# mx-strk/InformationBottleneckDecodingLDPC

Hardware: AMD Instinct MI355X
Metric: decoded codewords/sec + achieved HBM GB/s, DVB-S2 N=64800 i_max=50 (higher is better)
Workload: dtype u4

## Files before the change

include/ibldpc.h:

```cpp
#ifndef IBLDPC_H
#define IBLDPC_H

#include <stdint.h>

#ifdef __cplusplus
extern "C" {
#endif

#define IBL_VERSION 3

enum { IBL_OK = 0, IBL_EINVAL = -1, IBL_EHIP = -2, IBL_ENOMEM = -3, IBL_EUNSUPPORTED = -4 };
enum { IBL_U8 = 1, IBL_I32 = 2, IBL_F32 = 3, IBL_F64 = 4, IBL_I8 = 5 };
enum { IBL_MINSUM = 0, IBL_BP = 1 };
enum { IBL_PATH_AUTO = 0, IBL_PATH_PASSES = 1, IBL_PATH_FUSED = 2 };
enum { IBL_FLAG_FORCE_GENERIC = 1 };

typedef struct ibl_graph ibl_graph;
typedef struct ibl_ib ibl_ib;
typedef struct ibl_float ibl_float;

int ibl_version(void);
const char* ibl_last_error(void);
int ibl_device_count(int32_t* n);

int ibl_map_node_connections(int32_t n_v, int32_t n_c, const int32_t* csr_indptr, const int32_t* csr_cols,
                             int32_t* cn_start, int32_t* cn_deg, int32_t* tgt_cn,
                             int32_t* vn_start, int32_t* vn_deg, int32_t* tgt_vn);

int ibl_graph_create(int32_t n_v, int32_t n_c, const int32_t* csr_indptr, const int32_t* csr_cols,
                     int32_t device, ibl_graph** out);
int ibl_graph_info(const ibl_graph* g, int32_t* n_v, int32_t* n_c, int64_t* n_e, int32_t* d_c_max,
                   int32_t* d_v_max);
void ibl_graph_destroy(ibl_graph* g);

int ibl_ib_create(const ibl_graph* g, int32_t T_ch, int32_t T_dec, int32_t imax,
                  const int32_t* cn_lut, int64_t cn_len, const int32_t* vn_lut, int64_t vn_len,
                  const int32_t* match_cn, int64_t mc_len, const int32_t* match_vn, int64_t mv_len,
                  int32_t match, int32_t max_batch, int32_t flags, ibl_ib** out);
int ibl_ib_path(const ibl_ib* h);
int ibl_ib_set_path(ibl_ib* h, int32_t path);
int ibl_ib_path_in_use(const ibl_ib* h, int32_t* fused);
int ibl_ib_set_small_batch(ibl_ib* h, int32_t max_b);
int ibl_ib_small_batch(const ibl_ib* h, int32_t* max_b);
int ibl_ib_folded(const ibl_ib* h, int32_t* n_folded);
int ibl_ib_set_fold(ibl_ib* h, int32_t on);
int ibl_ib_fused_ncw(const ibl_ib* h, int32_t B, int32_t* ncw);
int ibl_ib_decode(ibl_ib* h, const void* d_ch, int32_t ch_dtype, int32_t B, void* d_out, int32_t out_dtype,
                  int32_t early_stop, int32_t* d_iters, void* stream);
void ibl_ib_destroy(ibl_ib* h);
int ibl_ib_timing(ibl_ib* h, int32_t enable);
int ibl_ib_timing_read(ibl_ib* h, double* cn_ms, int32_t* cn_launches, double* vn_ms, int32_t* vn_launches);

int ibl_float_create(const ibl_graph* g, int32_t kind, int32_t imax, double llr_max, int32_t precision,
                     int32_t max_batch, ibl_float** out);
int ibl_float_decode(ibl_float* h, const void* d_llr, int32_t llr_dtype, int32_t B, void* d_out,
                     int32_t out_dtype, int32_t early_stop, int32_t* d_iters, void* stream);
void ibl_float_destroy(ibl_float* h);
int ibl_float_set_path(ibl_float* h, int32_t path);
int ibl_float_path_in_use(const ibl_float* h, int32_t* fused);
int ibl_float_fused_geometry(const ibl_float* h, int32_t B, int32_t* ngroups, int32_t* grid);
int ibl_float_folded(const ibl_float* h, int32_t* n_folded);
int ibl_float_is_wide(const ibl_float* h, int32_t* wide);
int ibl_float_set_small_batch(ibl_float* h, int32_t max_b);
int ibl_float_small_batch(const ibl_float* h, int32_t* max_b);
int ibl_float_input_check(ibl_float* h, int32_t* violations, void* stream);
int ibl_float_timing(ibl_float* h, int32_t enable);
int ibl_float_timing_read(ibl_float* h, double* cn_ms, int32_t* cn_launches, double* vn_ms, int32_t* vn_launches);
int ibl_float_create_corrected(const ibl_graph* g, double alpha, double beta, int32_t imax, double llr_max,
                               int32_t precision, int32_t max_batch, ibl_float** out);
int ibl_float_correction(const ibl_float* h, double* alpha, double* beta);
int ibl_ib_decode_each(ibl_ib* h, const void* d_ch, int32_t ch_dtype, int32_t B, void* d_out, int32_t out_dtype,
                       int32_t* d_iters, void* stream);
int ibl_float_decode_each(ibl_float* h, const void* d_llr, int32_t llr_dtype, int32_t B, void* d_out,
                          int32_t out_dtype, int32_t* d_iters, void* stream);

typedef struct ibl_layered ibl_layered;
int ibl_layers_validate(int32_t n_v, int32_t n_c, const int32_t* csr_indptr, const int32_t* csr_cols,
                        int32_t n_layers, const int32_t* layer_ptr, const int32_t* layer_checks);
int ibl_layered_create(const ibl_graph* g, int32_t n_layers, const int32_t* layer_ptr, const int32_t* layer_checks,
                       int32_t imax, float alpha, float beta, float llr_max, int32_t precision, int32_t max_batch,
                       ibl_layered** out);
int ibl_layered_create_path(const ibl_graph* g, int32_t n_layers, const int32_t* layer_ptr,
                            const int32_t* layer_checks, int32_t imax, float alpha, float beta, float llr_max,
                            int32_t precision, int32_t max_batch, int32_t path, ibl_layered** out);
int ibl_layered_path_in_use(const ibl_layered* h, int32_t* fused);
int ibl_layered_is_wide(const ibl_layered* h, int32_t* wide);
int ibl_layered_decode(ibl_layered* h, const void* d_llr, int32_t llr_dtype, int32_t B, void* d_out,
                       int32_t out_dtype, int32_t early_stop, int32_t* d_iters, void* stream);
int ibl_layered_geometry(const ibl_layered* h, int32_t B, int32_t* cw_per_group, int32_t* ngroups, int32_t* grid);
int ibl_layered_set_compaction(ibl_layered* h, int32_t every, int32_t min_free_pct);
int ibl_layered_compaction_stats(const ibl_layered* h, void* stream, int32_t* compactions, int32_t* extent);
void ibl_layered_destroy(ibl_layered* h);

int ibl_layered_create_fixed(const ibl_graph* g, int32_t n_layers, const int32_t* layer_ptr,
                             const int32_t* layer_checks, int32_t imax, int32_t alpha16, int32_t beta_q, int32_t q_max,
                             float scale, int32_t max_batch, int32_t path, ibl_layered** out);
int ibl_layered_create_fixed_fused(const ibl_graph* g, int32_t n_layers, const int32_t* layer_ptr,
                                   const int32_t* layer_checks, int32_t imax, int32_t alpha16, int32_t beta_q,
                                   int32_t q_max, float scale, int32_t max_batch, ibl_layered** out);
int ibl_layered_is_fixed(const ibl_layered* h, int32_t* fixed);

int ibl_count_below(const void* d_x, int32_t dtype, int64_t rows, int32_t B, int64_t ld, double threshold,
                    int64_t* d_count, void* stream);

int ibl_channel_sample(const double* cdf, int32_t T, const double* llr, uint64_t seed, uint64_t offset, int32_t n,
                       int32_t B, const uint8_t* d_bits, void* d_out, int32_t out_dtype, int64_t ld, void* stream);

typedef struct ibl_encoder ibl_encoder;
int ibl_encoder_create(int32_t n_v, int32_t n_c, const int32_t* indptr, const int32_t* cols, int32_t max_batch,
                       int32_t device, ibl_encoder** out);
const char* ibl_encoder_algorithm(const ibl_encoder* h);
int ibl_encode(ibl_encoder* h, const uint8_t* d_info, int32_t B, uint8_t* d_code, void* stream);
void ibl_encoder_destroy(ibl_encoder* h);

int ibl_random_bits(uint64_t seed, uint64_t offset, int32_t n, int32_t B, uint8_t* d_out, void* stream);

int ibl_count_errors(const void* d_x, int32_t dtype, int64_t rows, int32_t B, int64_t ld, double threshold,
                     const uint8_t* d_bits, int64_t bits_ld, int64_t* d_count, void* stream);

int ibl_shard_range(int64_t total, int32_t rank, int32_t world, int64_t* start, int64_t* count);
#define IBL_COMM_ID_BYTES 128
typedef struct ibl_comm ibl_comm;
int ibl_comm_unique_id(uint8_t* id);
int ibl_comm_create(const uint8_t* id, int32_t nranks, int32_t rank, int32_t device, ibl_comm** out);
int ibl_comm_broadcast(ibl_comm* c, void* d_buf, int64_t bytes, int32_t root, void* stream);
int ibl_comm_allreduce_sum_i64(ibl_comm* c, int64_t* d_buf, int64_t count, void* stream);
void ibl_comm_destroy(ibl_comm* c);

// ... 6 lines not shown
```

informationbottleneckdecodingldpc_amd/_lib.py:

```python
from __future__ import annotations

import ctypes
import os

import numpy as np

_HERE = os.path.dirname(os.path.abspath(__file__))
LIB_PATH = os.environ.get("IBLDPC_LIB") or os.path.join(_HERE, "libibldpc.so")

IBL_OK, IBL_EINVAL, IBL_EHIP, IBL_ENOMEM, IBL_EUNSUPPORTED = 0, -1, -2, -3, -4
IBL_U8, IBL_I32, IBL_F32, IBL_F64, IBL_I8 = 1, 2, 3, 4, 5
IBL_MINSUM, IBL_BP = 0, 1
IBL_FLAG_FORCE_GENERIC = 1
IBL_PATH_AUTO, IBL_PATH_PASSES, IBL_PATH_FUSED = 0, 1, 2

EXPORTS = [
    "ibl_version", "ibl_last_error", "ibl_device_count", "ibl_map_node_connections",
    "ibl_graph_create", "ibl_graph_info", "ibl_graph_destroy",
    "ibl_ib_create", "ibl_ib_path", "ibl_ib_set_path", "ibl_ib_path_in_use", "ibl_ib_fused_ncw", "ibl_ib_decode",
    "ibl_ib_set_small_batch", "ibl_ib_small_batch", "ibl_ib_folded", "ibl_ib_set_fold",
    "ibl_ib_destroy",
    "ibl_float_create", "ibl_float_decode", "ibl_float_destroy", "ibl_count_below",
    "ibl_float_set_path", "ibl_float_path_in_use", "ibl_float_fused_geometry", "ibl_float_folded",
    "ibl_float_input_check", "ibl_float_is_wide",
    "ibl_float_set_small_batch", "ibl_float_small_batch",
    "ibl_float_create_corrected", "ibl_float_correction", "ibl_float_decode_each", "ibl_ib_decode_each",
    "ibl_ib_timing", "ibl_ib_timing_read", "ibl_float_timing", "ibl_float_timing_read",
    "ibl_channel_sample",
    "ibl_encoder_create",
    "ibl_encoder_algorithm",
    "ibl_encode",
    "ibl_encoder_destroy",
    "ibl_random_bits",
    "ibl_count_errors",
    "ibl_shard_range", "ibl_comm_unique_id", "ibl_comm_create", "ibl_comm_broadcast", "ibl_comm_allreduce_sum_i64",
    "ibl_comm_destroy",
    "ibl_layers_validate", "ibl_layered_create", "ibl_layered_decode", "ibl_layered_geometry", "ibl_layered_destroy",
    "ibl_layered_create_path", "ibl_layered_path_in_use", "ibl_layered_create_fixed", "ibl_layered_is_fixed",
    "ibl_layered_set_compaction", "ibl_layered_compaction_stats", "ibl_layered_is_wide",
    "ibl_layered_create_fixed_fused",
]
IBL_COMM_ID_BYTES = 128


class IBLError(RuntimeError):
    pass


_lib = None
_i32p = np.ctypeslib.ndpointer(dtype=np.int32, flags="C_CONTIGUOUS")
_vp = ctypes.c_void_p
_i32, _i64 = ctypes.c_int32, ctypes.c_int64


def load():
    global _lib
    if _lib is not None:
        return _lib
    if not os.path.exists(LIB_PATH):
        raise ImportError(f"{LIB_PATH} not found: build it with "
                          "`python -c 'import __graft_entry__ as g; g.build()'` (hipcc, gfx950)")
    L = ctypes.CDLL(LIB_PATH)
    L.ibl_version.restype = ctypes.c_int
    L.ibl_last_error.restype = ctypes.c_char_p
    L.ibl_device_count.argtypes = [ctypes.POINTER(_i32)]
    L.ibl_map_node_connections.argtypes = [_i32, _i32, _i32p, _i32p, _i32p, _i32p, _i32p, _i32p, _i32p, _i32p]
    L.ibl_graph_create.argtypes = [_i32, _i32, _i32p, _i32p, _i32, ctypes.POINTER(_vp)]
    L.ibl_graph_info.argtypes = [_vp, ctypes.POINTER(_i32), ctypes.POINTER(_i32), ctypes.POINTER(_i64),
                                 ctypes.POINTER(_i32), ctypes.POINTER(_i32)]
    L.ibl_graph_destroy.argtypes = [_vp]
    L.ibl_graph_destroy.restype = None
    L.ibl_ib_create.argtypes = [_vp, _i32, _i32, _i32, _i32p, _i64, _i32p, _i64, _i32p, _i64, _i32p, _i64,
                                _i32, _i32, _i32, ctypes.POINTER(_vp)]
    L.ibl_ib_path.argtypes = [_vp]
    L.ibl_ib_set_path.argtypes = [_vp, _i32]
    L.ibl_ib_path_in_use.argtypes = [_vp, ctypes.POINTER(_i32)]
    L.ibl_ib_fused_ncw.argtypes = [_vp, _i32, ctypes.POINTER(_i32)]
    L.ibl_ib_set_small_batch.argtypes = [_vp, _i32]
    L.ibl_ib_small_batch.argtypes = [_vp, ctypes.POINTER(_i32)]
    L.ibl_ib_folded.argtypes = [_vp, ctypes.POINTER(_i32)]
    L.ibl_ib_set_fold.argtypes = [_vp, _i32]
    L.ibl_ib_decode.argtypes = [_vp, _vp, _i32, _i32, _vp, _i32, _i32, _vp, _vp]
    L.ibl_ib_decode_each.argtypes = [_vp, _vp, _i32, _i32, _vp, _i32, _vp, _vp]
    L.ibl_ib_destroy.argtypes = [_vp]
    L.ibl_ib_destroy.restype = None
    L.ibl_float_create.argtypes = [_vp, _i32, _i32, ctypes.c_double, _i32, _i32, ctypes.POINTER(_vp)]
    L.ibl_float_decode.argtypes = [_vp, _vp, _i32, _i32, _vp, _i32, _i32, _vp, _vp]
    L.ibl_float_decode_each.argtypes = [_vp, _vp, _i32, _i32, _vp, _i32, _vp, _vp]
    L.ibl_float_destroy.argtypes = [_vp]
    L.ibl_float_destroy.restype = None
    L.ibl_float_set_path.argtypes = [_vp, _i32]
    L.ibl_float_path_in_use.argtypes = [_vp, ctypes.POINTER(_i32)]
    L.ibl_float_fused_geometry.argtypes = [_vp, _i32, ctypes.POINTER(_i32), ctypes.POINTER(_i32)]
    L.ibl_float_folded.argtypes = [_vp, ctypes.POINTER(_i32)]
    L.ibl_float_is_wide.argtypes = [_vp, ctypes.POINTER(_i32)]
    L.ibl_float_set_small_batch.argtypes = [_vp, _i32]
    L.ibl_float_small_batch.argtypes = [_vp, ctypes.POINTER(_i32)]
    L.ibl_float_input_check.argtypes = [_vp, ctypes.POINTER(_i32), _vp]
    L.ibl_float_create_corrected.argtypes = [_vp, ctypes.c_double, ctypes.c_double, _i32, ctypes.c_double, _i32, _i32,
                                             ctypes.POINTER(_vp)]
    L.ibl_float_correction.argtypes = [_vp, ctypes.POINTER(ctypes.c_double), ctypes.POINTER(ctypes.c_double)]
    for nm in ("ibl_ib_timing", "ibl_float_timing"):
        getattr(L, nm).argtypes = [_vp, _i32]
    for nm in ("ibl_ib_timing_read", "ibl_float_timing_read"):
        getattr(L, nm).argtypes = [_vp, ctypes.POINTER(ctypes.c_double), ctypes.POINTER(_i32),
                                   ctypes.POINTER(ctypes.c_double), ctypes.POINTER(_i32)]
    L.ibl_count_below.argtypes = [_vp, _i32, _i64, _i32, _i64, ctypes.c_double, _vp, _vp]
    _dp = np.ctypeslib.ndpointer(np.float64, flags="C_CONTIGUOUS")
    L.ibl_channel_sample.argtypes = [_dp, _i32, _vp, ctypes.c_uint64, ctypes.c_uint64, _i32, _i32, _vp, _vp,
                                     _i32, _i64, _vp]
    L.ibl_encoder_create.argtypes = [_i32, _i32, _i32p, _i32p, _i32, _i32, ctypes.POINTER(_vp)]
    L.ibl_encoder_algorithm.argtypes = [_vp]
    L.ibl_encoder_algorithm.restype = ctypes.c_char_p
    L.ibl_encode.argtypes = [_vp, _vp, _i32, _vp, _vp]
    L.ibl_encoder_destroy.argtypes = [_vp]
    L.ibl_encoder_destroy.restype = None
    L.ibl_random_bits.argtypes = [ctypes.c_uint64, ctypes.c_uint64, _i32, _i32, _vp, _vp]
    L.ibl_count_errors.argtypes = [_vp, _i32, _i64, _i32, _i64, ctypes.c_double, _vp, _i64, _vp, _vp]
    L.ibl_shard_range.argtypes = [_i64, _i32, _i32, ctypes.POINTER(_i64), ctypes.POINTER(_i64)]
    L.ibl_comm_unique_id.argtypes = [_vp]
    L.ibl_comm_create.argtypes = [_vp, _i32, _i32, _i32, ctypes.POINTER(_vp)]
    L.ibl_comm_broadcast.argtypes = [_vp, _vp, _i64, _i32, _vp]
    L.ibl_comm_allreduce_sum_i64.argtypes = [_vp, _vp, _i64, _vp]
    L.ibl_comm_destroy.argtypes = [_vp]
    L.ibl_comm_destroy.restype = None
    L.ibl_layers_validate.argtypes = [_i32, _i32, _i32p, _i32p, _i32, _i32p, _i32p]
    _f32 = ctypes.c_float
    L.ibl_layered_create.argtypes = [_vp, _i32, _i32p, _i32p, _i32, _f32, _f32, _f32, _i32, _i32, ctypes.POINTER(_vp)]
    L.ibl_layered_create_path.argtypes = [_vp, _i32, _i32p, _i32p, _i32, _f32, _f32, _f32, _i32, _i32, _i32,
                                          ctypes.POINTER(_vp)]
    L.ibl_layered_path_in_use.argtypes = [_vp, ctypes.POINTER(_i32)]
    L.ibl_layered_create_fixed.argtypes = [_vp, _i32, _i32p, _i32p, _i32, _i32, _i32, _i32, _f32, _i32, _i32,
                                           ctypes.POINTER(_vp)]
    L.ibl_layered_create_fixed_fused.argtypes = [_vp, _i32, _i32p, _i32p, _i32, _i32, _i32, _i32, _f32, _i32,
                                                 ctypes.POINTER(_vp)]
    L.ibl_layered_is_fixed.argtypes = [_vp, ctypes.POINTER(_i32)]
    L.ibl_layered_is_wide.argtypes = [_vp, ctypes.POINTER(_i32)]
    L.ibl_layered_decode.argtypes =[_vp, _vp, _i32, _i32, _vp, _i32, _i32, _vp, _vp]
    L.ibl_layered_geometry.argtypes = [_vp, _i32, ctypes.POINTER(_i32), ctypes.POINTER(_i32), ctypes.POINTER(_i32)]
    L.ibl_layered_set_compaction.argtypes = [_vp, _i32, _i32]
    L.ibl_layered_compaction_stats.argtypes = [_vp, _vp, ctypes.POINTER(_i32), ctypes.POINTER(_i32)]
    L.ibl_layered_destroy.argtypes = [_vp]
    L.ibl_layered_destroy.restype = None
    for name in EXPORTS:
        getattr(L, name)
    _lib = L
    return L


def check(rc: int, what: str = "") -> None:
    if rc != IBL_OK:
        msg = load().ibl_last_error().decode(errors="replace")
        raise IBLError(f"{what} failed (rc={rc}): {msg}")


def device_count() -> int:
    n = _i32(0)
    load().ibl_device_count(ctypes.byref(n))
    return int(n.value)


def map_node_connections(n_v: int, n_c: int, indptr: np.ndarray, cols: np.ndarray):
    L = load()
    indptr = np.ascontiguousarray(indptr, dtype=np.int32)
# ... 33 lines not shown
```

informationbottleneckdecodingldpc_amd/csrc/capi_ib.hip:

```cpp
#include <cstring>
#include <functional>

#include "host.h"

using namespace ibl;

struct ibl_ib {
  const ibl_graph* g = nullptr;
  int32_t Tc = 0, T = 0, imax = 0, CM = 0, VM = 0, match = 0, max_batch = 0, ldb = 0;
  bool fast = false;
  DevBuf<uint8_t> cin, vin, ch8;
  DevBuf<int32_t> flags, dL;
  DevBuf<uint32_t> cn_img, vn_img, dec_img;
  int cn_nt = 0, vn_nt = 0, dec_nt = 0;
  int32_t cn_fslot[kMaxD + 1] = {0}, vn_fslot[kMaxD + 1] = {0};
  KCfg kcn, kvn, kdec;
  KTimer timer;
  int32_t n_folded = 0, fold_slot = -1, n_rest = 0, rest_heavy = 0;
  bool fold_on = true;
  std::vector<int32_t> fold_rec, fold_cn_info, fold_vn_info;
  DevBuf<uint8_t> cin2;
  DevBuf<int32_t> fold, cn_info_f, vn_info_r;
  int32_t path = IBL_PATH_AUTO;
  bool fused_ok = false, f_half_ok = false;
  bool f_each_ok = false;
  int32_t f_ncw_forced = 0;
  int32_t small_b = 0;
  bool s_ok = false;
  size_t s_lds_cn = 0, s_lds_vn = 0, s_lds_dec = 0;
  ChainGraphs s_graphs;
  FusedTaskBufs ft;
  int32_t f_nreg = 0, f_dbuf = 0, f_cn_uni = 0, f_vn_uni = 0;
  size_t f_lds = 0;
  int f_grid = 0, f_block = 0;
  DevBuf<int32_t> cn_lut, vn_lut, mc, mv;
  int64_t cn_len = 0, vn_len = 0, mc_len = 0, mv_len = 0;
};

namespace {

using Table = std::vector<uint8_t>;

struct IbLuts {
  const int32_t *cn, *vn, *mc, *mv;
  int64_t cn_len, vn_len, mc_len, mv_len;
};
struct IbSlots {
  std::vector<int> cdeg, vdeg;
  int cn_nraw = 0, vn_nraw = 0;
  int cn_nt = 0, vn_nt = 0;
};
struct IbImages {
  std::vector<uint32_t> cn_img, vn_img, dec_img;
};

Table make_table(int T, const std::function<int(int, int)>& f) {
  Table tb(256, 0);
  for (int t = 0; t < T; ++t)
    for (int m = 0; m < T; ++m) tb[t * kTP + m] = (uint8_t)f(t, m);
  return tb;
}

void append_pass(std::vector<uint32_t>& img, const std::vector<Table>& tbs, int nreg) {
  for (int R = 0; R < nreg; ++R)
    for (int r = 0; r < 256; ++r) {
      uint32_t w = 0;
      for (int j = 0; j < 4; ++j) {
        const size_t k = (size_t)4 * R + j;
        if (k < tbs.size()) w |= (uint32_t)tbs[k][r] << (8 * j);
      }
      img.push_back(w);
    }
}

std::vector<int> present(const std::vector<int32_t>& deg) {
  std::vector<int> d(deg.begin(), deg.end());
  std::sort(d.begin(), d.end());
  d.erase(std::unique(d.begin(), d.end()), d.end());
  return d;
}

size_t fast_lds(int nt) { return lds_of_quads(regions_of(nt)) + 64; }

int pick_cfg(int which, int maxd, int nt, int num_cus, KCfg* k) {
  k->lds = fast_lds(nt);
  int best_waves = 0;
  for (int block : {1024, 768, 640, 512, 384, 256}) {
    int bpc = 0;
    if (ib_fast_occupancy(which, maxd, block, k->lds, &bpc) != hipSuccess) continue;
    const int waves = bpc * block / 64;
    if (bpc > 0 && waves > best_waves) {
      best_waves = waves;
      k->block = block;
      k->grid = bpc * num_cus;
    }
  }
  return best_waves > 0 ? IBL_OK : fail(IBL_EHIP, "no occupancy for IB kernel (LDS too large?)");
}

int ib_validate(const ibl_graph* g, int32_t Tc, int32_t T, int32_t imax, const IbLuts& lu, int32_t match,
                int32_t max_batch) {
  if (Tc < 2 || T < 2 || Tc > 256 || T > 256) return fail(IBL_EUNSUPPORTED, "cardinalities must lie in [2, 256]");
  if (imax < 1) return fail(IBL_EINVAL, "imax must be >= 1");
  if (max_batch < 1) return fail(IBL_EINVAL, "max_batch must be >= 1");
  const int CM = g->dcm, VM = g->dvm;
  if (CM < 3) return fail(IBL_EUNSUPPORTED, "IB decoding needs a check-node degree >= 3");
  const int64_t need_cn = (int64_t)Tc * Tc + (int64_t)(CM - 3) * Tc * T + (int64_t)(imax - 1) * (CM - 2) * T * T;
  const int64_t need_vn = (int64_t)imax * ((int64_t)Tc * T + (int64_t)(VM - 1) * T * T);
  if (!lu.cn || lu.cn_len < need_cn) return fail(IBL_EINVAL, "CN LUT vector shorter than the reference layout");
  if (!lu.vn || lu.vn_len < need_vn) return fail(IBL_EINVAL, "VN LUT vector shorter than the reference layout");
  auto in_T = [T](const int32_t* p, int64_t n) { return std::all_of(p, p + n, [T](int32_t x) { return x >= 0 && x < T; }); };
  if (!in_T(lu.cn, lu.cn_len)) return fail(IBL_EINVAL, "CN LUT entries must lie in [0, T_dec)");
  if (!in_T(lu.vn, lu.vn_len)) return fail(IBL_EINVAL, "VN LUT entries must lie in [0, T_dec)");
  if (match) {
    if (!lu.mc || lu.mc_len < (int64_t)imax * CM * T || !lu.mv || lu.mv_len < (int64_t)imax * VM * T)
      return fail(IBL_EINVAL, "matching vectors shorter than (imax, d_max, T_dec)");
    if (!in_T(lu.mc, lu.mc_len) || !in_T(lu.mv, lu.mv_len))
      return fail(IBL_EINVAL, "matching entries must lie in [0, T_dec)");
  }
  return IBL_OK;
}

IbSlots ib_plan_slots(ibl_ib* h, int32_t flags) {
  const ibl_graph* g = h->g;
  const int CM = h->CM, VM = h->VM;
  IbSlots sl;
  sl.cdeg = present(g->h_cn_deg);
  sl.vdeg = present(g->h_vn_deg);
  const bool deg_ok = CM <= kMaxD && VM <= kMaxD;
  sl.cn_nt = sl.cn_nraw = h->match ? CM - 3 : CM - 2;
  sl.vn_nt = sl.vn_nraw = h->match ? std::max(VM - 2, 0) : VM - 1;
  if (h->match) {
    sl.cn_nt += (int)sl.cdeg.size();
    for (int d : sl.vdeg) sl.vn_nt += (d >= 2);
  }
  const int max_nt = (kLdsBytes / kSuper) * 8;
  int slot = sl.cn_nraw;
  for (int d : sl.cdeg) {
    const int fs = h->match ? slot++ : (d >= 3 ? d - 3 : 0);
    if (deg_ok) h->cn_fslot[d] = fs;
  }
  slot = sl.vn_nraw;
  for (int d : sl.vdeg) {
    if (d < 2) continue;
    const int fs = h->match ? slot++ : d - 2;
    if (deg_ok) h->vn_fslot[d] = fs;
  }
  const bool lds_ok = fast_lds(sl.cn_nt) <= (size_t)kLdsBytes && fast_lds(std::max(sl.vn_nt, 1)) <= (size_t)kLdsBytes;
  h->fast = !(flags & IBL_FLAG_FORCE_GENERIC) && h->Tc == h->T && h->T <= kTP && deg_ok && sl.cn_nt <= max_nt &&
            sl.vn_nt <= max_nt && VM <= max_nt && sl.cn_nt > 0 && lds_ok;
  if (h->fast && CM <= 8) {
    std::vector<int32_t> rec, rest;
    const int32_t n = plan_ib_fold(*g, &rec, &rest);
    if (n > 0 && sl.cn_nt + 1 <= max_nt && fast_lds(sl.cn_nt + 1) <= (size_t)kLdsBytes) {
      h->n_folded = n;
      h->fold_slot = sl.cn_nt++;
      std::vector<int32_t> cls((size_t)g->n_c), all((size_t)g->n_c);
      for (int32_t c = 0; c < g->n_c; ++c) {
        cls[c] = rec[(size_t)kIbFoldRec * c];
        all[c] = c;
      }
      int32_t heavy = 0;
      h->fold_cn_info = work_order_keyed(all, g->h_cn_start, g->h_cn_deg, &cls, &heavy);
      h->fold_vn_info = work_order_keyed(rest, g->h_vn_start, g->h_vn_deg, nullptr, &h->rest_heavy);
      h->n_rest = (int32_t)rest.size();
      h->fold_rec.swap(rec);
    }
  }
  return sl;
}

IbImages ib_build_images(ibl_ib* h, const IbLuts& lu, const IbSlots& sl) {
  const int Tc = h->Tc, T = h->T, imax = h->imax, CM = h->CM, VM = h->VM;
  IbImages im;
  const int64_t T2 = (int64_t)T * T;
  auto cn_raw = [&](int p, int l, int t, int m) -> int {
    int64_t idx;
    if (p == 0) idx = (l == 0) ? (int64_t)t * Tc + m : (int64_t)Tc * Tc + (int64_t)(l - 1) * Tc * T + (int64_t)t * T + m;
    else idx = (int64_t)Tc * Tc + (int64_t)(CM - 3) * Tc * T + (int64_t)(p - 1) * (CM - 2) * T2 + l * T2 + (int64_t)t * T + m;
    return lu.cn[idx];
  };
  auto vn_raw = [&](int k, int l, int t, int m) -> int {
    const int64_t off = (int64_t)k * ((int64_t)Tc * T + (int64_t)(VM - 1) * T2);
    const int64_t idx = off + (l == 0 ? (int64_t)t * T + m : (int64_t)Tc * T + (int64_t)(l - 1) * T2 + (int64_t)t * T + m);
    return lu.vn[idx];
  };
  for (int p = 0; p < imax; ++p) {
    std::vector<Table> tbs;
    for (int l = 0; l < sl.cn_nraw; ++l) tbs.push_back(make_table(T, [&](int t, int m) { return cn_raw(p, l, t, m); }));
    if (h->match)
      for (int d : sl.cdeg) {
        const int64_t mrow = (int64_t)p * T * CM + (int64_t)(d - 1) * T;
        if (d == 2) tbs.push_back(make_table(T, [&](int t, int) { return lu.mc[mrow + t]; }));
        else tbs.push_back(make_table(T, [&](int t, int m) { return lu.mc[mrow + cn_raw(p, d - 3, t, m)]; }));
      }
    if (h->fold_slot >= 0) {
      const int64_t mrow = (int64_t)p * T * VM + (int64_t)T;
      tbs.resize((size_t)h->fold_slot, Table(256, 0));
      tbs.push_back(make_table(T, [&](int t, int m) {
        const int r = vn_raw(p, 0, m, t);
        return h->match ? lu.mv[mrow + r] : r;
      }));
    }
    append_pass(im.cn_img, tbs, regions_of(sl.cn_nt));
  }
  h->cn_nt = regions_of(sl.cn_nt);
  for (int k = 0; k < std::max(imax - 1, 1); ++k) {
    std::vector<Table> tbs;
    for (int l = 0; l < sl.vn_nraw; ++l) tbs.push_back(make_table(T, [&](int t, int m) { return vn_raw(k, l, t, m); }));
    for (int d : sl.vdeg) {
      if (!h->match || d < 2) continue;
      const int64_t mrow = (int64_t)k * T * VM + (int64_t)(d - 1) * T;
      tbs.push_back(make_table(T, [&](int t, int m) { return lu.mv[mrow + vn_raw(k, d - 2, t, m)]; }));
    }
    append_pass(im.vn_img, tbs, regions_of(std::max(sl.vn_nt, 1)));
  }
  h->vn_nt = regions_of(std::max(sl.vn_nt, 1));
  for (int k = 0; k < imax; ++k) {
    std::vector<Table> tbs;
    for (int l = 0; l < VM; ++l) tbs.push_back(make_table(T, [&](int t, int m) { return vn_raw(k, l, t, m); }));
    append_pass(im.dec_img, tbs, regions_of(VM));
  }
  h->dec_nt = regions_of(VM);
  return im;
}

int ib_fused_setup(ibl_ib* h) {
  const ibl_graph* g = h->g;
  if (!h->fast || g->n_e == 0 || g->dc_min < 2) return IBL_OK;
  const int nreg = std::max(h->cn_nt, std::max(h->vn_nt, h->dec_nt));
  const size_t lds1 = lds_of_quads(nreg) + (size_t)nreg * 1024 + (size_t)g->n_e * 4 + 16;
  const size_t lds2 = lds_of_quads(2 * nreg) + (size_t)g->n_e * 4 + 16;
  const bool dbuf = nreg <= 2 && lds2 <= (size_t)kLdsBytes && env_on("IBL_FUSED_DBUF");
  const size_t lds = dbuf ? lds2 : lds1;
  if (lds > (size_t)kLdsBytes) return IBL_OK;
  int bpc = 0, block = 0;
  size_t priv = 0;
  if (ib_fused_occupancy(h->CM, h->VM, 8, lds, &bpc, &block, &priv) != hipSuccess || bpc < 1 || priv != 0) {
    (void)hipGetLastError();
    return IBL_OK;
  }
  {
    int bpc4 = 0, block4 = 0;
    size_t priv4 = 0;
    h->f_half_ok = ib_fused_occupancy(h->CM, h->VM, 4, lds, &bpc4, &block4, &priv4) == hipSuccess && bpc4 == bpc &&
                   block4 == block && priv4 == 0;
    (void)hipGetLastError();
  }
  {
    int bpe = 0, blocke = 0;
    size_t prive = 0;
    h->f_each_ok = ib_fused_occupancy(h->CM, h->VM, 8, lds, &bpe, &blocke, &prive, true) == hipSuccess && bpe == bpc &&
                   blocke == block && prive == 0;
    if (h->f_each_ok && h->f_half_ok)
      h->f_each_ok = ib_fused_occupancy(h->CM, h->VM, 4, lds, &bpe, &blocke, &prive, true) == hipSuccess &&
                     bpe == bpc && blocke == block && prive == 0;
    (void)hipGetLastError();
  }
  FusedTasks ft;
  build_fused_tasks(*g, &ft, env_on("IBL_FUSED_VORDER"), fused_vwin());
  if (int rc = h->ft.upload(ft)) return rc;
  if (env_on("IBL_FUSED_UNIFORM")) {
    auto uniform = [](const std::vector<int32_t>& task, int32_t n, bool vn) {
      if (task.empty()) return 0;
      const int32_t d = task[2];
      for (size_t t = 0; t < task.size() / 4; ++t) {
        const int32_t p = (int32_t)(64 * t), cnt = std::min<int32_t>(64, n - p);
        const int32_t* r = &task[4 * t];
        if (r[1] != cnt || r[2] != d || (vn ? (r[0] != p || r[3] != p * d) : r[0] != p * d)) return 0;
      }
      return (int)d;
    };
    h->f_cn_uni = uniform(ft.cn_task, g->n_c, false);
    h->f_vn_uni = uniform(ft.vn_task, g->n_v, true);
  }
  if (const char* ne = getenv("IBL_FUSED_NCW")) h->f_ncw_forced = atoi(ne);
  h->f_nreg = nreg;
  h->f_dbuf = dbuf ? 1 : 0;
  h->f_lds = lds;
  h->f_block = block;
  h->f_grid = bpc * g->num_cus;
  h->fused_ok = true;
  return IBL_OK;
}

int ib_configure_fast(ibl_ib* h, const IbImages& im) {
  const ibl_graph* g = h->g;
  const int CM = h->CM, VM = h->VM;
  int rc;
  if ((rc = h->cn_img.upload(im.cn_img)) || (rc = h->vn_img.upload(im.vn_img)) || (rc = h->dec_img.upload(im.dec_img)))
    return rc;
  if ((rc = pick_cfg(0, CM, 4 * h->cn_nt, g->num_cus, &h->kcn)) ||
      (rc = pick_cfg(1, VM, 4 * h->vn_nt, g->num_cus, &h->kvn)) ||
      (rc = pick_cfg(2, VM, 4 * h->dec_nt, g->num_cus, &h->kdec)))
    return rc;
  size_t priv = 0;
  const char* kname = "";
  HIPCHK(ib_fast_private_bytes(CM, VM, &priv, &kname));
#if IBL_DIAG
  const bool allow_scratch = getenv("IBL_ALLOW_SCRATCH") != nullptr;
#else
  const bool allow_scratch = false;
#endif
  if (!allow_scratch && (rc = refuse_private(priv, std::string("fast-path kernel ") + kname + " has a ",
                                             "-byte private segment (register spill / scratch item): rebuild required")))
    return rc;
  if ((rc = ib_fused_setup(h))) return rc;
  HIPCHK(ib_small_private_bytes(CM, VM, &priv, &kname));
  h->s_ok = priv == 0;
  small_batch_env(h->s_ok, kSmallBatchDefault, &h->small_b, &h->s_graphs);
  h->s_lds_cn = lds_of_quads(h->cn_nt);
  h->s_lds_vn = lds_of_quads(h->vn_nt);
  h->s_lds_dec = lds_of_quads(h->dec_nt);
  return IBL_OK;
}

int ib_upload_generic(ibl_ib* h, const IbLuts& lu) {
  int rc;
  h->cn_len = lu.cn_len; h->vn_len = lu.vn_len;
  if ((rc = h->cn_lut.upload(lu.cn, lu.cn_len)) || (rc = h->vn_lut.upload(lu.vn, lu.vn_len))) return rc;
  if (h->match) {
    h->mc_len = lu.mc_len; h->mv_len = lu.mv_len;
    if ((rc = h->mc.upload(lu.mc, lu.mc_len)) || (rc = h->mv.upload(lu.mv, lu.mv_len))) return rc;
  }
  return IBL_OK;
}

bool ib_fused_in_use(const ibl_ib* h) { return h->fused_ok && h->path != IBL_PATH_PASSES; }

int ib_fused_ncw(const ibl_ib* h, int B) {
  const int ngroups = (B + 7) / 8;
  const int forced = h->f_ncw_forced;
  if (!h->f_half_ok || forced == 8) return 8;
  return (forced == 4 || 2 * ngroups <= h->f_grid) ? 4 : 8;
}

int ib_fold_alloc(ibl_ib* h) {
  if (h->n_folded == 0 || h->cin2) return IBL_OK;
  DevBuf<uint8_t> c2;
  DevBuf<int32_t> fold, cf, vr;
  int rc;
  if ((rc = c2.alloc_zero((size_t)h->g->n_e * h->ldb)) || (rc = fold.upload(h->fold_rec)) ||
      (rc = cf.upload(h->fold_cn_info)) || (rc = vr.upload(h->fold_vn_info)))
    return rc;
  h->fold = std::move(fold);
  h->cn_info_f = std::move(cf);
  h->vn_info_r = std::move(vr);
  h->cin2 = std::move(c2);
  return IBL_OK;
}


void ib_pass_args(const ibl_ib* h, int B, int ldbb, IbFastArgs* cn, IbFastArgs* vn) {
  const ibl_graph* g = h->g;
  cn->ch8 = vn->ch8 = h->ch8;
  cn->info = g->cn_info; cn->tgt = g->tgt_cn; cn->out = h->vin;
  vn->info = g->vn_info; vn->tgt = g->tgt_vn; vn->out = h->cin; vn->in = h->vin;
  cn->n_nodes = g->n_c; vn->n_nodes = g->n_v;
  cn->ldb = vn->ldb = ldbb;
  cn->B = vn->B = B;
  cn->half = vn->half = h->T / 2;
  cn->match = vn->match = h->match;
  cn->nt = h->cn_nt; vn->nt = h->vn_nt;
  std::memcpy(cn->fslot, h->cn_fslot, sizeof(cn->fslot));
  std::memcpy(vn->fslot, h->vn_fslot, sizeof(vn->fslot));
}

IbFusedArgs ib_fused_args(const ibl_ib* h, uint32_t* chT, int32_t B, void* d_out, int32_t out_dtype, int* grid) {
  const ibl_graph* g = h->g;
  IbFusedArgs f{};
  f.cn_img = h->cn_img; f.vn_img = h->vn_img; f.dec_img = h->dec_img; f.chT = chT;
  f.cn_task = h->ft.cn_task; f.vn_task = h->ft.vn_task; f.vn_node = h->ft.vn_node; f.vn_slot = h->ft.vn_slot;
  f.out = d_out;
  std::memcpy(f.cn_fslot, h->cn_fslot, sizeof(f.cn_fslot));
  std::memcpy(f.vn_fslot, h->vn_fslot, sizeof(f.vn_fslot));
  f.cn_nt = h->cn_nt; f.vn_nt = h->vn_nt; f.dec_nt = h->dec_nt; f.nreg = h->f_nreg; f.dbuf = h->f_dbuf;
  f.n_cn_nodes = g->n_c; f.cn_uni = h->f_cn_uni; f.vn_uni = h->f_vn_uni;
  f.n_e = (int32_t)g->n_e; f.n_v = g->n_v; f.n_cn_tasks = h->ft.n_cn; f.n_vn_tasks = h->ft.n_vn;
// ... 60 lines not shown
    const int wpb = small_block(nwords) / 64;
    const int need = (ntask * nwords + wpb - 1) / wpb;
    return std::max(1, std::min(need, per_cu * g->num_cus));
  };
  IbFastArgs cn{}, vn{};
  ib_pass_args(h, B, ldbb, &cn, &vn);
  cn.task = g->cn_task; cn.n_tasks = g->n_cn_task;
  vn.task = g->vn_task; vn.n_tasks = g->n_vn_task;
  cn.nwords = vn.nwords = nwords;
  const int gcn = grid_of(g->n_cn_task, h->s_lds_cn), gvn = grid_of(g->n_vn_task, h->s_lds_vn);
  auto chain = [&](hipStream_t st) -> hipError_t {
    IbFastArgs c0 = cn, v = vn;
    c0.in = nullptr; c0.gather = g->csr_cols; c0.img = h->cn_img; c0.gate = nullptr; c0.unsat = nullptr;
    hipError_t e = h->timer.timed(0, st, [&] { return launch_ib_cn_small(c0, h->CM, gcn, h->s_lds_cn, st); });
    if (e != hipSuccess) return e;
    IbFastArgs c = c0;
    c.gather = nullptr;
    c.in = h->cin;
    for (int j = 1; j < I; ++j) {
      const int32_t* gate = flag_row(h->flags, early && j >= 2, j - 1);
      v.img = h->vn_img + (size_t)(j - 1) * h->vn_nt * 256;
      v.gate = gate;
      if ((e = h->timer.timed(1, st, [&] { return launch_ib_vn_small(v, h->VM, gvn, h->s_lds_vn, st); })) != hipSuccess)
        return e;
      c.img = h->cn_img + (size_t)j * h->cn_nt * 256;
      c.gate = gate;
      c.unsat = flag_row(h->flags, early, j);
      if ((e = h->timer.timed(0, st, [&] { return launch_ib_cn_small(c, h->CM, gcn, h->s_lds_cn, st); })) != hipSuccess)
        return e;
    }
    return hipSuccess;
  };
  if (h->s_graphs.on && !h->timer.on) HIPCHK(h->s_graphs.run(B, early ? 1 : 0, s, chain));
  else HIPCHK(chain(s));
  HIPCHK(launch_finalize(h->flags, I, early ? 1 : 0, h->dL, d_iters, s));
  IbDecArgs dc{};
  dc.vin = h->vin; dc.ch8 = h->ch8; dc.img = h->dec_img; dc.iters = h->dL; dc.out = d_out; dc.out_dtype = out_dtype;
  dc.nt = h->dec_nt; dc.n_nodes = g->n_v; dc.ldb = ldbb; dc.B = B;
  dc.info = g->vn_info; dc.task = g->vn_task; dc.n_tasks = g->n_vn_task; dc.nwords = nwords;
  dc.aligned = out_aligned(B, d_out, 4, out_dtype == kU8 ? 1 : 4);
  HIPCHK(launch_ib_dec_small(dc, grid_of(g->n_vn_task, h->s_lds_dec), h->s_lds_dec, s));
  return IBL_OK;
}

int ib_decode_fast(ibl_ib* h, const void* d_ch, int32_t ch_dtype, int32_t B, void* d_out, int32_t out_dtype,
                   bool early, int32_t* d_iters, hipStream_t s) {
  const ibl_graph* g = h->g;
  const int I = h->imax;
  const int ccn = ib_fast_chunk(h->CM), cvn = ib_fast_chunk(h->VM);
  const int ldbb = h->ldb / 2;
  HIPCHK(launch_ib_stage4(d_ch, ch_dtype, g->n_v, B, h->ch8, ldbb, s));
  IbFastArgs cn{}, vn{};
  ib_pass_args(h, B, ldbb, &cn, &vn);
  cn.n_heavy = g->cn_heavy; vn.n_heavy = g->vn_heavy;
  const bool fold = h->fold_on && h->n_folded > 0 && I > 1;
  int rc;
  if (fold) {
    if ((rc = ib_fold_alloc(h))) return rc;
    vn.info = h->vn_info_r; vn.n_nodes = h->n_rest; vn.n_heavy = h->rest_heavy;
    cn.fold = h->fold; cn.fold_slot = h->fold_slot;
  }
  uint8_t* cb[2] = {h->cin, fold ? h->cin2 : h->cin};
  auto cn_fold = [&](int j) {
    const bool f = fold && j < I - 1;
    cn.info = f ? h->cn_info_f.get() : g->cn_info.get();
    cn.fold_mode = f ? ((early && j >= 1) ? 2 : 1) : 0;
    cn.fout = f ? cb[(j + 1) & 1] : nullptr;
  };
#if IBL_DIAG
  if (const char* vp = getenv("IBL_VN_PART")) {
    if (vp[0] == 'h') {
      vn.n_nodes = g->vn_heavy;
    } else if (vp[0] == 'l') {
      vn.info = g->vn_info + 4 * (size_t)g->vn_heavy;
      vn.n_nodes = g->n_v - g->vn_heavy;
      vn.n_heavy = 0;
    }
  }
#endif
  cn.nchunks = (B + ccn - 1) / ccn;
  vn.nchunks = (B + cvn - 1) / cvn;
  cn.in = nullptr; cn.gather = g->csr_cols; cn.img = h->cn_img; cn.gate = nullptr; cn.unsat = nullptr;
  cn_fold(0);
  auto launch_cn = [&]() { return launch_ib_cn_fast(cn, h->CM, h->kcn.grid, h->kcn.block, h->kcn.lds, s); };
  HIPCHK(h->timer.timed(0, s, launch_cn));
  cn.gather = nullptr;
  uint64_t* trace = nullptr;
  size_t nwv = 0;
#if IBL_DIAG
  const char* trace_path = getenv("IBL_TRACE_WAVES");
  TraceBuf tr;
  nwv = (size_t)h->kvn.grid * (h->kvn.block / 64);
  const size_t nwc = (size_t)h->kcn.grid * (h->kcn.block / 64);
  if (trace_path && I > 1) {
    if ((rc = tr.open(3 * (nwv + nwc), s))) return rc;
    trace = tr.d;
  }
#endif
  for (int j = 1; j < I; ++j) {
    const int32_t* gate = flag_row(h->flags, early && j >= 2, j - 1);
    vn.img = h->vn_img + (size_t)(j - 1) * h->vn_nt * 256;
    vn.gate = gate;
    vn.trace = (trace && j == I / 2) ? trace : nullptr;
    vn.out = cb[j & 1];
    HIPCHK(h->timer.timed(1, s, [&] { return launch_ib_vn_fast(vn, h->VM, h->kvn.grid, h->kvn.block, h->kvn.lds, s); }));
    cn.img = h->cn_img + (size_t)j * h->cn_nt * 256;
    cn.gate = gate;
    cn.unsat = flag_row(h->flags, early, j);
    cn.trace = (trace && j == I / 2) ? trace + 3 * nwv : nullptr;
    cn.in = cb[j & 1];
    cn_fold(j);
    HIPCHK(h->timer.timed(0, s, launch_cn));
  }
#if IBL_DIAG
  if (trace && ((rc = tr.save(s, std::string(trace_path) + "_vn.bin", 0, 3 * nwv)) ||
                (rc = tr.save(s, std::string(trace_path) + "_cn.bin", 3 * nwv, 3 * nwc))))
    return rc;
#endif
  HIPCHK(launch_finalize(h->flags, I, early ? 1 : 0, h->dL, d_iters, s));
  IbDecArgs dc{};
  dc.vin = h->vin; dc.ch8 = h->ch8; dc.start = g->vn_start; dc.deg = g->vn_deg; dc.img = h->dec_img;
  dc.iters = h->dL; dc.out = d_out; dc.out_dtype = out_dtype; dc.nt = h->dec_nt; dc.n_nodes = g->n_v;
  dc.nchunks = (B + kChunkDec - 1) / kChunkDec; dc.ldb = ldbb; dc.B = B;
  dc.aligned = out_aligned(B, d_out, 4, out_dtype == kU8 ? 1 : 4);
  HIPCHK(launch_ib_dec_fast(dc, h->kdec.grid, h->kdec.block, h->kdec.lds, s));
  return IBL_OK;
}

int ib_decode_generic(ibl_ib* h, const void* d_ch, int32_t ch_dtype, int32_t B, void* d_out, int32_t out_dtype,
                      bool early, int32_t* d_iters, hipStream_t s) {
  const ibl_graph* g = h->g;
  const int I = h->imax;
  HIPCHK(launch_ib_stage(d_ch, ch_dtype, g->n_v, B, h->ch8, h->ldb, s));
  IbGenArgs cn{}, vn{};
  cn.ch8 = vn.ch8 = h->ch8;
  cn.start = g->cn_start; cn.deg = g->cn_deg; cn.tgt = g->tgt_cn; cn.out = h->vin; cn.lut = h->cn_lut;
  cn.lut_len = h->cn_len; cn.mt = h->mc; cn.mt_len = h->mc_len;
  vn.start = g->vn_start; vn.deg = g->vn_deg; vn.tgt = g->tgt_vn; vn.out = h->cin; vn.in = h->vin; vn.lut = h->vn_lut;
  vn.lut_len = h->vn_len; vn.mt = h->mv; vn.mt_len = h->mv_len;
  cn.Tc = vn.Tc = h->Tc; cn.T = vn.T = h->T; cn.CM = vn.CM = h->CM; cn.VM = vn.VM = h->VM;
  cn.match = vn.match = h->match;
  cn.n_nodes = g->n_c; vn.n_nodes = g->n_v;
  cn.ldb = vn.ldb = h->ldb; cn.B = vn.B = B; cn.half = vn.half = h->T / 2;
  cn.pass = 0; cn.in = nullptr; cn.gather = g->csr_cols;
  HIPCHK(h->timer.timed(0, s, [&] { return launch_ib_cn_gen(cn, s); }));
  cn.in = h->cin; cn.gather = nullptr;
  for (int j = 1; j < I; ++j) {
    const int32_t* gate = flag_row(h->flags, early && j >= 2, j - 1);
    vn.pass = j - 1; vn.gate = gate;
    HIPCHK(h->timer.timed(1, s, [&] { return launch_ib_vn_gen(vn, s); }));
    cn.pass = j; cn.gate = gate; cn.unsat = flag_row(h->flags, early, j);
    HIPCHK(h->timer.timed(0, s, [&] { return launch_ib_cn_gen(cn, s); }));
  }
  HIPCHK(launch_finalize(h->flags, I, early ? 1 : 0, h->dL, d_iters, s));
  IbGenDecArgs dc{};
  dc.vin = h->vin; dc.ch8 = h->ch8; dc.start = g->vn_start; dc.deg = g->vn_deg; dc.lut = h->vn_lut;
  dc.lut_len = h->vn_len; dc.iters = h->dL; dc.out = d_out; dc.out_dtype = out_dtype; dc.Tc = h->Tc; dc.T = h->T;
  dc.VM = h->VM; dc.n_nodes = g->n_v; dc.ldb = h->ldb; dc.B = B;
  HIPCHK(launch_ib_dec_gen(dc, s));
  return IBL_OK;
}
}

extern "C" {

int ibl_ib_create(const ibl_graph* g, int32_t Tc, int32_t T, int32_t imax, const int32_t* cn_lut, int64_t cn_len,
                  const int32_t* vn_lut, int64_t vn_len, const int32_t* match_cn, int64_t mc_len,
                  const int32_t* match_vn, int64_t mv_len, int32_t match, int32_t max_batch, int32_t flags,
                  ibl_ib** out) {
  if (!out) return fail(IBL_EINVAL, "out is NULL");
  *out = nullptr;
  if (!g) return fail(IBL_EINVAL, "graph is NULL");
  const IbLuts lu{cn_lut, vn_lut, match_cn, match_vn, cn_len, vn_len, mc_len, mv_len};
  int rc = ib_validate(g, Tc, T, imax, lu, match, max_batch);
  if (rc) return rc;
  HIPCHK(hipSetDevice(g->device));
  std::unique_ptr<ibl_ib> h(new ibl_ib());
  h->g = g;
  h->Tc = Tc; h->T = T; h->imax = imax; h->CM = g->dcm; h->VM = g->dvm; h->match = match ? 1 : 0;
  h->max_batch = max_batch;
  h->ldb = (max_batch + kRowPad - 1) / kRowPad * kRowPad;
  const size_t inbox = (size_t)g->n_e * h->ldb;
  if ((rc = h->cin.alloc_zero(inbox)) || (rc = h->vin.alloc_zero(inbox)) ||
      (rc = h->ch8.alloc_zero((size_t)g->n_v * h->ldb)) || (rc = h->flags.alloc_zero((size_t)imax * kShards)) ||
      (rc = h->dL.alloc(1)))
    return rc;
  const IbSlots sl = ib_plan_slots(h.get(), flags);
  if (h->fast) rc = ib_configure_fast(h.get(), ib_build_images(h.get(), lu, sl));
  else rc = ib_upload_generic(h.get(), lu);
  if (rc) return rc;
  *out = h.release();
  return IBL_OK;
}

int ibl_ib_path(const ibl_ib* h) { return h && h->fast ? 1 : 0; }

int ibl_ib_set_small_batch(ibl_ib* h, int32_t max_b) {
  if (!h) return fail(IBL_EINVAL, "decoder is NULL");
  if (max_b < 0) return fail(IBL_EINVAL, "max_b must be >= 0");
  if (max_b > 0 && !(h->fast && h->s_lds_cn > 0))
    return fail(IBL_EUNSUPPORTED, "the small-batch kernels need the fast path (T_ch = T_dec <= 16, degrees <= 16)");
  if (max_b > 0 && !h->s_ok)
    return fail(IBL_EUNSUPPORTED, "the small-batch kernels of this build have a private segment: rebuild required");
  h->small_b = max_b;
  return IBL_OK;
}

int ibl_ib_small_batch(const ibl_ib* h, int32_t* max_b) {
  if (!h || !max_b) return fail(IBL_EINVAL, "NULL argument");
  *max_b = h->small_b;
  return IBL_OK;
}

int ibl_ib_set_path(ibl_ib* h, int32_t path) {
  if (!h) return fail(IBL_EINVAL, "decoder is NULL");
  if (int rc = check_path(path)) return rc;
  if (path == IBL_PATH_FUSED && !h->fused_ok)
    return fail(IBL_EUNSUPPORTED, "code does not fit the fused IB kernel (fast path, E * 4 B of messages plus the "
                                  "largest pass's tables within 160 KiB, check degrees >= 2)");
  h->path = path;
  return IBL_OK;
}

int ibl_ib_fused_ncw(const ibl_ib* h, int32_t B, int32_t* ncw) {
  if (!h || !ncw) return fail(IBL_EINVAL, "NULL argument");
  if (B < 1 || B > h->max_batch) return fail(IBL_EINVAL, "B must lie in [1, max_batch]");
  *ncw = ib_fused_in_use(h) ? ib_fused_ncw(h, B) : 0;
  return IBL_OK;
}

int ibl_ib_path_in_use(const ibl_ib* h, int32_t* fused) {
  if (!h || !fused) return fail(IBL_EINVAL, "NULL argument");
  *fused = ib_fused_in_use(h) ? 1 : 0;
  return IBL_OK;
}

int ibl_ib_folded(const ibl_ib* h, int32_t* n_folded) {
  if (!h || !n_folded) return fail(IBL_EINVAL, "NULL argument");
  *n_folded = h->n_folded;
  return IBL_OK;
}

int ibl_ib_set_fold(ibl_ib* h, int32_t on) {
  if (!h) return fail(IBL_EINVAL, "decoder is NULL");
  h->fold_on = on != 0;
  return IBL_OK;
}

int ibl_ib_timing(ibl_ib* h, int32_t enable) { return timing_enable(h, enable); }
int ibl_ib_timing_read(ibl_ib* h, double* cn_ms, int32_t* cn_n, double* vn_ms, int32_t* vn_n) {
  return timing_read(h, cn_ms, cn_n, vn_ms, vn_n);
}

void ibl_ib_destroy(ibl_ib* h) {
  if (h) (void)hipSetDevice(h->g->device);
  delete h;
}

static int ib_decode_check(const ibl_ib* h, const void* d_ch, int32_t ch_dtype, int32_t B, const void* d_out,
                           int32_t out_dtype) {
  if (!h) return fail(IBL_EINVAL, "decoder is NULL");
  if (B < 1 || B > h->max_batch) return fail(IBL_EINVAL, "B must lie in [1, max_batch]");
  if (ch_dtype != kU8 && ch_dtype != kI32) return fail(IBL_EINVAL, "channel dtype must be IBL_U8 or IBL_I32");
  if (out_dtype != kU8 && out_dtype != kI32) return fail(IBL_EINVAL, "output dtype must be IBL_U8 or IBL_I32");
  if (!d_ch || !d_out) return fail(IBL_EINVAL, "NULL buffer");
  return IBL_OK;
}

int
ibl_ib_decode_each(ibl_ib* h, const void* d_ch, int32_t ch_dtype, int32_t B, void* d_out, int32_t out_dtype,
                   int32_t* d_iters, void* stream) {
  if (int rc = ib_decode_check(h, d_ch, ch_dtype, B, d_out, out_dtype)) return rc;
  if (!ib_fused_in_use(h))
    return fail(IBL_EUNSUPPORTED, "the per-codeword stop runs on the fused kernel only (path \"passes\", the generic "
                                  "path, or the code does not fit it)");
  if (!h->f_each_ok)
    return fail(IBL_EUNSUPPORTED, "the per-codeword-stop kernels of this build have a private segment or another "
                                  "occupancy than the fused kernel: rebuild required");
  HIPCHK(hipSetDevice(h->g->device));
  return ib_each_fused(h, d_ch, ch_dtype, B, d_out, out_dtype, d_iters, (hipStream_t)stream);
}

int ibl_ib_decode(ibl_ib* h, const void* d_ch, int32_t ch_dtype, int32_t B, void* d_out, int32_t out_dtype,
                  int32_t early_stop, int32_t* d_iters, void* stream) {
  if (int rc = ib_decode_check(h, d_ch, ch_dtype, B, d_out, out_dtype)) return rc;
  hipStream_t s = (hipStream_t)stream;
  HIPCHK(hipSetDevice(h->g->device));
  const bool early = early_stop != 0 && h->imax > 1;
  if (early) HIPCHK(hipMemsetAsync(h->flags, 0, sizeof(int32_t) * (size_t)h->imax * kShards, s));
  if (ib_fused_in_use(h)) return ib_decode_fused(h, d_ch, ch_dtype, B, d_out, out_dtype, early, d_iters, s);
  if (!h->fast) return ib_decode_generic(h, d_ch, ch_dtype, B, d_out, out_dtype, early, d_iters, s);
  if (B <= h->small_b) return ib_decode_small(h, d_ch, ch_dtype, B, d_out, out_dtype, early, d_iters, s);
  return ib_decode_fast(h, d_ch, ch_dtype, B, d_out, out_dtype, early, d_iters, s);
}

}
```

informationbottleneckdecodingldpc_amd/csrc/common.h:

```cpp
#pragma once
#include <hip/hip_runtime.h>
#pragma clang diagnostic ignored "-Wunused-result"
#include <stddef.h>
#include <stdint.h>

#include "plan.h"

namespace ibl {

constexpr int kWave = 64;
constexpr int kChunk = 256;
#ifndef IBL_W
#define IBL_W 2
#endif
constexpr int kW = IBL_W;
constexpr int kChunkIB = 512 * kW;
#ifndef IBL_LIGHT_W
#define IBL_LIGHT_W 4
#endif
constexpr int kRowPad = 512 * (IBL_LIGHT_W > IBL_W ? IBL_LIGHT_W : IBL_W);
constexpr int kChunkDec = 512;
constexpr int kTbl = 8192;
constexpr int kSuper = 65536;
constexpr int kRowSh = 12, kColSh = 8;
__host__ __device__ constexpr uint32_t quad_off(int q) { return (uint32_t)(q >> 1) * kSuper + (uint32_t)(q & 1) * 128u; }
__host__ __device__ constexpr uint32_t slot_off(int s) { return quad_off(s >> 2) + (uint32_t)(s & 3); }
constexpr int regions_of(int nt) { return (nt + 3) >> 2; }
__host__ __device__ constexpr size_t lds_of_quads(int nq) { return (size_t)((nq + 1) >> 1) * kSuper; }
constexpr int kTP = 16;
constexpr int kShards = 64;
constexpr int kLdsBytes = 160 * 1024;

enum Dtype : int32_t { kU8 = 1, kI32 = 2, kF32 = 3, kF64 = 4, kI8 = 5 };

int set_error(int code, const char* msg);

typedef __attribute__((address_space(4))) const int32_t cint32;
__device__ __forceinline__ int32_t sload(const int32_t* p, int i) { return ((cint32*)p)[i]; }

__device__ __forceinline__ int take_ticket(int* ctr, int lane) {
  int t = 0;
  if (lane == 0) t = __hip_atomic_fetch_add(ctr, 1, __ATOMIC_RELAXED, __HIP_MEMORY_SCOPE_WORKGROUP);
  return __builtin_amdgcn_readfirstlane(t);
}

struct IbFastArgs {
  const uint8_t* in;
  uint8_t* out;
  const uint8_t* ch8;
  const int32_t* info;
  const int32_t* tgt;
  const int32_t* gather;
  const uint32_t* img;
  const int32_t* gate;
  int32_t* unsat;
  int32_t fslot[kMaxD + 1];
  int32_t nt;
  int32_t n_nodes, nchunks, ldb, B, half, match;
  int32_t n_heavy;
  uint64_t* trace;
  const int32_t* task;
  int32_t n_tasks, nwords;
  const int32_t* fold;
  uint8_t* fout;
  int32_t fold_mode, fold_slot;
};

struct IbDecArgs {
  const uint8_t* vin;
  const uint8_t* ch8;
  const int32_t* start;
  const int32_t* deg;
  const uint32_t* img;
  const int32_t* iters;
  void* out;
  int32_t out_dtype, nt, n_nodes, nchunks, ldb, B, aligned;
  const int32_t* info;
  const int32_t* task;
  int32_t n_tasks, nwords;
};

struct IbFusedArgs {
  const uint32_t* cn_img;
  const uint32_t* vn_img;
  const uint32_t* dec_img;
  const uint32_t* chT;
  const int32_t* cn_task;
  const int32_t* vn_task;
  const int32_t* vn_node;
  const int32_t* vn_slot;
  void* out;
  int32_t* unsat;
  const int32_t* dL;
  int32_t cn_fslot[kMaxD + 1], vn_fslot[kMaxD + 1];
  int32_t cn_nt, vn_nt, dec_nt, nreg;
  int32_t dbuf;
  int32_t n_cn_nodes;
  int32_t cn_uni, vn_uni;
  int32_t n_e, n_v, n_cn_tasks, n_vn_tasks, B, imax, half, match, out_dtype, aligned, ngroups;
  int32_t ncw;
  uint64_t* trace;
  int32_t* iters;
};

struct IbGenArgs {
  const uint8_t* in;
  uint8_t* out;
  const uint8_t* ch8;
  const int32_t* start;
  const int32_t* deg;
  const int32_t* tgt;
  const int32_t* gather;
  const int32_t* lut;
  const int32_t* mt;
  const int32_t* gate;
  int32_t* unsat;
  int64_t lut_len, mt_len;
  int32_t pass, Tc, T, CM, VM, match, n_nodes, ldb, B, half;
};

struct IbGenDecArgs {
  const uint8_t* vin;
  const uint8_t* ch8;
  const int32_t* start;
  const int32_t* deg;
  const int32_t* lut;
  const int32_t* iters;
  void* out;
  int64_t lut_len;
  int32_t out_dtype, Tc, T, VM, n_nodes, ldb, B;
};

enum FlFamily : int { kFlPerPass = 0, kFlSmall = 1, kFlFused = 2 };
enum FlPass : int { kFlCheck = 0, kFlVariable = 1, kFlDecision = 2, kFlSend = 3 };
constexpr int kFlWideD = 32;
constexpr int fl_cw_per_lane(int prec) { return prec == kF32 ? 4 : 2; }
constexpr size_t fl_elem_size(int dtype) { return dtype == kF32 ? 4 : 8; }
constexpr int fl_vn_chunk(int prec) { return 64 * fl_cw_per_lane(prec); }
struct FlArgs {
  const void* in;
  void* out;
  const void* ch;
  const int32_t* start;
  const int32_t* deg;
  const int32_t* tgt;
  const int32_t* gate;
  int32_t* unsat;
  double llr_max;
  int32_t n_nodes, nchunks, ldb, B;
  const int32_t* fold;
  void* fout;
  int32_t fold_mode;
  const int32_t* nodes;
  const int32_t* info;
  const int32_t* task;
  int32_t n_tasks, nwords;
  double cor_a, cor_b;
};

constexpr int kFlTraceWords = 65;
struct FlFusedArgs {
  const void* ch;
  const int32_t* cn_task;
  const int32_t* vn_task;
  const int32_t* vn_node;
  const int32_t* vn_slot;
  void* out;
  int32_t* unsat;
  const int32_t* dL;
  double llr_max;
  int32_t n_e, n_v, n_cn_tasks, n_vn_tasks, ldb, B, imax, out_dtype, aligned, ngroups;
  int32_t n_vs;
  uint64_t* trace;
  double cor_a, cor_b;
  int32_t* iters;
};

struct FlDecArgs {
  const void* vin0;
  const void* vin1;
  const void* ch;
  const int32_t* start;
  const int32_t* deg;
  const int32_t* iters;
  void* out;
  int32_t out_dtype, n_nodes, nchunks, ldb, B, aligned;
  const int32_t* info;
  const int32_t* task;
  int32_t n_tasks, nwords;
};

hipError_t launch_ib_stage(const void* ch, int dtype, int n, int B, uint8_t* ch8, int ldb, hipStream_t s);
hipError_t launch_ib_stage4(const void* ch, int dtype, int n, int B, uint8_t* ch4, int ldb_bytes, hipStream_t s);
hipError_t launch_ib_cn_fast(const IbFastArgs& a, int maxd, int grid, int block, size_t lds, hipStream_t s);
hipError_t launch_ib_vn_fast(const IbFastArgs& a, int maxd, int grid, int block, size_t lds, hipStream_t s);
int ib_fast_chunk(int maxd);
hipError_t launch_ib_dec_fast(const IbDecArgs& a, int grid, int block, size_t lds, hipStream_t s);
constexpr int kSmallBlock = 1024;
__host__ __device__ constexpr int small_block(int nwords) { return nwords <= 1 ? 256 : (nwords <= 8 ? 512 : 1024); }
constexpr int kFlSmallBlock = 256;
constexpr int kSmallBatchDefault = 224;
constexpr int kFlSmallBatchDefault = 64;
hipError_t launch_ib_cn_small(const IbFastArgs& a, int maxd, int grid, size_t lds, hipStream_t s);
hipError_t launch_ib_vn_small(const IbFastArgs& a, int maxd, int grid, size_t lds, hipStream_t s);
hipError_t launch_ib_dec_small(const IbDecArgs& a, int grid, size_t lds, hipStream_t s);
hipError_t ib_small_private_bytes(int cn_maxd, int vn_maxd, size_t* bytes, const char** name);
hipError_t ib_fast_occupancy(int which, int maxd, int block, size_t lds, int* blocks_per_cu);
hipError_t ib_fast_private_bytes(int cn_maxd, int vn_maxd, size_t* bytes, const char** name);
hipError_t launch_ib_stage_t(const void* ch, int dtype, int n, int B, const int32_t* perm, uint32_t* chT,
                             hipStream_t s);
hipError_t launch_ib_fused(const IbFusedArgs& a, int cmax, int vmax, int grid, int block, size_t lds, hipStream_t s,
                           bool each = false);
hipError_t ib_fused_occupancy(int cmax, int vmax, int ncw, size_t lds, int* blocks_per_cu, int* block,
                              size_t* private_bytes, bool each = false);
hipError_t launch_ib_cn_gen(const IbGenArgs& a, hipStream_t s);
hipError_t launch_ib_vn_gen(const IbGenArgs& a, hipStream_t s);
hipError_t launch_ib_dec_gen(const IbGenDecArgs& a, hipStream_t s);
hipError_t launch_finalize(const int32_t* flags, int imax, int early, int32_t* dL, int32_t* user, hipStream_t s);
constexpr int kMaxT = 64;
constexpr int kChBinSh = 43, kChBins = 1 << (53 - kChBinSh);
struct ChArgs {
  uint64_t kthr[kMaxT + 1];
  double llr[kMaxT];
  uint64_t ctr[4];
  uint64_t key[2];
  const uint8_t* bits;
  void* out;
  int64_t total, ld;
  int32_t B, T, dtype;
  int32_t sorted;
  uint16_t bin[kChBins];
};
hipError_t launch_ch_sample(const ChArgs& a, hipStream_t s);

hipError_t launch_enc_pack(const uint8_t* in, int rows, int B, int Bw, uint32_t* out, hipStream_t s);
hipError_t launch_enc_ax(const uint32_t* x, const int32_t* indptr, const int32_t* cols, int M, int Bw, uint32_t* r,
                         hipStream_t s);
hipError_t launch_enc_subst(const uint32_t* in, uint32_t* out, const int32_t* indptr, const int32_t* cols, int M,
                            int Bw, int dir, hipStream_t s);
hipError_t launch_enc_scan(const uint32_t* r, uint32_t* tot, int M, int Bw, int dir, uint32_t* p, hipStream_t s);
int enc_scan_segments();
hipError_t launch_enc_gather(const uint32_t* in, const int32_t* order, int M, int Bw, uint32_t* out, hipStream_t s);
hipError_t launch_enc_unpack(const uint8_t* info, const uint32_t* p, int K, int M, int B, int Bw, uint8_t* code,
                             hipStream_t s);
hipError_t launch_random_bits(uint64_t seed, uint64_t offset, int64_t total, uint8_t* out, hipStream_t s);
hipError_t launch_count_errors(const void* x, int dtype, int64_t rows, int B, int64_t ld, double thr,
                               const uint8_t* bits, int64_t bits_ld, unsigned long long* cnt, hipStream_t s);

hipError_t launch_count_below(const void* x, int dtype, int64_t rows, int B, int64_t ld, double thr,
                              unsigned long long* cnt, hipStream_t s);

hipError_t launch_fl_send(const FlArgs& a, int prec, hipStream_t s);
hipError_t launch_fl_stage(const void* x, int in_dtype, int n, int B, void* dst, int prec, int ldb, int rule,
                           int32_t* bad, hipStream_t s);
hipError_t launch_fl_stage_t(const void* x, int in_dtype, int n, int B, const int32_t* perm, void* dst, int prec,
                             int rule, int32_t* bad, hipStream_t s);
hipError_t launch_fl_pass(FlFamily fam, FlPass pass, const FlArgs& a, int kind, int prec, int maxd, int grid,
                          hipStream_t s);
hipError_t launch_fl_dec(FlFamily fam, const FlDecArgs& a, int prec, int grid, hipStream_t s);
hipError_t launch_fl_fused(const FlFusedArgs& a, int kind, int prec, int cmax, int vmax, int grid, size_t lds,
                           hipStream_t s, bool each = false);
hipError_t fl_occupancy(FlFamily fam, FlPass pass, int kind, int prec, int cmax, int vmax, size_t lds,
                        int* blocks_per_cu, int* block, bool each = false);
hipError_t fl_private_bytes(FlFamily fam, int kind, int prec, int cn_maxd, int vn_maxd, bool fused, size_t* bytes,
                            const char** name);

struct LayeredArgs {
  float* buf;
  const int32_t* task;
  const int32_t* idx;
  int32_t* iters;
  float alpha, beta, llr_max;
  int32_t n_v, n_c, n_tasks, B, imax, early, ngroups, cw_per_group, cw_bytes;
  uint64_t* trace;
};
hipError_t lay_fused_occupancy(bool wide, int cw_per_group, size_t lds, int* blocks_per_cu, size_t* private_bytes);
hipError_t launch_lay_fused(const LayeredArgs& a, bool wide, int grid, size_t lds, hipStream_t s);
// ... 76 lines not shown
```

informationbottleneckdecodingldpc_amd/csrc/ib_kernels.hip:

```cpp
#include <algorithm>
#include <type_traits>

#include "common.h"

namespace ibl {


typedef __attribute__((address_space(3))) const uint8_t lds8_t;
__device__ __forceinline__ uint32_t lu(uint32_t x, uint32_t c) {
  asm("" : "+v"(x));
  return *(lds8_t*)(size_t)(x + c);
}
__device__ __forceinline__ uint32_t luc(uint32_t t, uint32_t q, uint32_t c) {
  uint32_t x;
  static_assert(kRowSh == 12, "luc's shift is the row shift of the table layout");
  asm("v_lshl_or_b32 %0, %1, 12, %2" : "=v"(x) : "v"(t), "v"(q));
  return *(lds8_t*)(size_t)(x + c);
}
__device__ __forceinline__ uint32_t lds_base(const uint8_t* p) { return (uint32_t)(size_t)(lds8_t*)p; }
__device__ __forceinline__ void lds_at_zero(const uint8_t* lds) {
  if (lds_base(lds) != 0u) __builtin_trap();
}

__device__ __forceinline__ uint32_t qidx(uint32_t m, uint32_t lane4) { return (m << kColSh) | lane4; }

__device__ __forceinline__ uint32_t valid_mask4(int remaining) {
  return remaining >= 4 ? 0xFu : (remaining <= 0 ? 0u : ((1u << remaining) - 1u));
}

__device__ __forceinline__ bool gate_open(const int32_t* gate, int lane) {
  if (!gate) return true;
  return __ballot(gate[lane] != 0) != 0ull;
}

constexpr int kStageR = 4;
__device__ __forceinline__ void stage_tables(uint8_t* lds, const uint32_t* img, int nreg) {
  const int nraw = nreg * 256, lane = threadIdx.x & 63;
  const int wv = threadIdx.x >> 6, nwv = blockDim.x >> 6, nchunk = (nraw + 63) >> 6;
  for (int c0 = 0; c0 < nchunk; c0 += kStageR * nwv) {
    uint32_t v[kStageR];
#pragma unroll
    for (int k = 0; k < kStageR; ++k) {
      const int r = (c0 + wv + k * nwv) * 64 + lane;
      v[k] = r < nraw ? img[r] : 0u;
    }
#pragma unroll
    for (int k = 0; k < kStageR; ++k) {
      const int c = c0 + wv + k * nwv;
      if (c >= nchunk) break;
#pragma unroll
      for (int p = 0; p < 8; ++p) {
        const int src = 8 * p + (lane >> 3), r = c * 64 + src;
        const uint32_t w = __shfl(v[k], src, 64);
        if (r < nraw)
          *reinterpret_cast<uint4*>(lds + quad_off(r >> 8) + (uint32_t)(r & 255) * 256u + 16u * (uint32_t)(lane & 7)) =
              make_uint4(w, w, w, w);
      }
    }
  }
}

__device__ __forceinline__ uint32_t nib(uint32_t w, int k) { return __builtin_amdgcn_ubfe(w, 4 * k, 4); }
__device__ __forceinline__ uint32_t colq(uint32_t w, int k, uint32_t lane4) {
  static_assert(kColSh == 8, "colq places the column in byte 1");
  const uint32_t src = (k & 1) ? ((w >> 4) & 0x0F0F0F0Fu) : (w & 0x0F0F0F0Fu);
  return __builtin_amdgcn_perm(src, lane4, 0x03020000u | ((4u + (uint32_t)(k >> 1)) << 8));
}

template <int P>
__device__ __forceinline__ uint32_t rowcol(uint32_t x, uint32_t y) {
  if constexpr (P == 0) return ((x << 4) & 0xF0F0F0F0u) | (y & 0x0F0F0F0Fu);
  else return (x & 0xF0F0F0F0u) | ((y >> 4) & 0x0F0F0F0Fu);
}
__device__ __forceinline__ uint32_t colb(uint32_t e, int k, uint32_t lane4) {
  return __builtin_amdgcn_perm(e, lane4, 0x03020000u | ((4u + (uint32_t)(k >> 1)) << 8));
}
template <int K>
__device__ __forceinline__ uint32_t pk(uint32_t acc, uint32_t t) {
  static_assert(K >= 0 && K < 8, "nibble of a dword");
  if constexpr (K == 0) {
    return t;
  } else {
    uint32_t r;
    asm("v_lshl_or_b32 %0, %1, %2, %3" : "=v"(r) : "v"(t), "n"(4 * K), "v"(acc));
    return r;
  }
}

__device__ __forceinline__ void step_fence() { __builtin_amdgcn_sched_barrier(0); }
#define IBL_E(e, x, y) const uint32_t e##_0 = rowcol<0>(x, y), e##_1 = rowcol<1>(x, y)
#define IBL_EP(e, s) ((ST == 2 ? (K0 & 1) : ((s) & 1)) ? e##_1 : e##_0)
#define IBL_X2(M, ...) M(0, __VA_ARGS__), M(1, __VA_ARGS__)
#define IBL_X4(M, ...) IBL_X2(M, __VA_ARGS__), M(2, __VA_ARGS__), M(3, __VA_ARGS__)
#define IBL_Q_(s, q, w, base) q##_##s = colq(w, K0 + ST * s, base)
#define IBL_QC_(s, q, on, w) q##_##s = (on) ? colq(w, K0 + ST * s, lane4c) : 0u
#define IBL_LUC_(s, n, p, q, c) n##_##s = luc(p##_##s, q##_##s, c)
#define IBL_LU1_(s, n, e, base, c) n##_##s = lu(colb(IBL_EP(e, s), K0 + ST * s, base), c)
#define IBL_LINK_(s, n, on, p, q) n##_##s = (on) ? luc(p##_##s, q##_##s, 0u) : p##_##s
#define IBL_PK_(s, o, v) o = pk<K0 + ST * s>(o, v##_##s)
#define IBL_Q2(...) const uint32_t IBL_X2(IBL_Q_, __VA_ARGS__)
#define IBL_Q4(...) const uint32_t IBL_X4(IBL_Q_, __VA_ARGS__)
#define IBL_QC2(...) const uint32_t IBL_X2(IBL_QC_, __VA_ARGS__)
#define IBL_QC4(...) const uint32_t IBL_X4(IBL_QC_, __VA_ARGS__)
#define IBL_LUC2(...) const uint32_t IBL_X2(IBL_LUC_, __VA_ARGS__)
#define IBL_LUC4(...) const uint32_t IBL_X4(IBL_LUC_, __VA_ARGS__)
#define IBL_LU12(...) const uint32_t IBL_X2(IBL_LU1_, __VA_ARGS__)
#define IBL_LU14(...) const uint32_t IBL_X4(IBL_LU1_, __VA_ARGS__)
#define IBL_LINK2(...) const uint32_t IBL_X2(IBL_LINK_, __VA_ARGS__)
#define IBL_LINK4(...) const uint32_t IBL_X4(IBL_LINK_, __VA_ARGS__)
#define IBL_PK2(...) IBL_X2(IBL_PK_, __VA_ARGS__)
#define IBL_PK4(...) IBL_X4(IBL_PK_, __VA_ARGS__)

__device__ __forceinline__ uint32_t valid_nib8(int remaining) {
  return remaining >= 8 ? 0xFFFFFFFFu : (remaining <= 0 ? 0u : ((1u << (4 * remaining)) - 1u));
}

template <int W> struct RowVec;
template <> struct RowVec<1> { typedef uint32_t T; };
template <> struct RowVec<2> { typedef uint2 T; };
template <> struct RowVec<4> { typedef uint4 T; };

#ifndef IBL_NT_CN
#define IBL_NT_CN 1
#endif
#ifndef IBL_NT
#define IBL_NT 1
#endif
typedef uint32_t u32x2_t __attribute__((ext_vector_type(2)));
typedef uint32_t u32x4_t __attribute__((ext_vector_type(4)));
template <int W> struct RowNV;
template <> struct RowNV<1> { typedef uint32_t T; };
template <> struct RowNV<2> { typedef u32x2_t T; };
template <> struct RowNV<4> { typedef u32x4_t T; };

template <int W, bool NT = false>
__device__ __forceinline__ void load_row(const uint8_t* p, uint32_t (&r)[W]) {
  if constexpr (NT) {
    using T = typename RowNV<W>::T;
    const T v = __builtin_nontemporal_load(reinterpret_cast<const T*>(p));
    if constexpr (W == 1) {
      r[0] = v;
    } else {
#pragma unroll
      for (int i = 0; i < W; ++i) r[i] = v[i];
    }
  } else {
    const auto v = *reinterpret_cast<const typename RowVec<W>::T*>(p);
    if constexpr (W == 1) {
      r[0] = v;
    } else if constexpr (W == 2) {
      r[0] = v.x; r[1] = v.y;
    } else {
      r[0] = v.x; r[1] = v.y; r[2] = v.z; r[3] = v.w;
    }
  }
}

template <int W, bool NT = false>
__device__ __forceinline__ void store_row(uint8_t* p, const uint32_t (&r)[W]) {
  if constexpr (NT) {
    using T = typename RowNV<W>::T;
    T v;
    if constexpr (W == 1) {
      v = r[0];
    } else {
#pragma unroll
      for (int i = 0; i < W; ++i) v[i] = r[i];
    }
    __builtin_nontemporal_store(v, reinterpret_cast<T*>(p));
  } else if constexpr (W == 1) {
    *reinterpret_cast<uint32_t*>(p) = r[0];
  } else if constexpr (W == 2) {
    *reinterpret_cast<uint2*>(p) = make_uint2(r[0], r[1]);
  } else {
    *reinterpret_cast<uint4*>(p) = make_uint4(r[0], r[1], r[2], r[3]);
  }
}


template <int MAXD>
constexpr int rowW() { return MAXD <= 8 ? kW : 1; }
template <int MAXD>
constexpr int chunkOf() { return 512 * rowW<MAXD>(); }
static_assert(kLightD <= 8, "light item buffers must fit the MAXD=8 bodies");

template <int MAXD, int W_ = rowW<MAXD>()>
struct ItemBuf {
  static constexpr int kMax = MAXD, W = W_;
  uint32_t row[MAXD][W];
  uint32_t tgv;
  uint32_t chw[W];
  int d, st, node;
  uint32_t off;
  int cwb;
  int fc, fv0, fv1, fd0, fd1;
};

struct PhaseItems {
  int first, pos0, nch;
};

template <class Buf, bool VN, bool GATHER, int FOLD = 0>
__device__ __forceinline__ void fetch_item(const IbFastArgs& a, int item, int lane, Buf& b, const PhaseItems& pi) {
  constexpr int W = Buf::W, MAXD = Buf::kMax;
  const int rel = item - pi.first;
  const int q = __builtin_amdgcn_readfirstlane(rel / pi.nch);
  const int chunk = __builtin_amdgcn_readfirstlane(rel - q * pi.nch);
  const int pos = pi.pos0 + q;
  const int node = sload(a.info, 4 * pos);
  b.node = node;
  b.st = sload(a.info, 4 * pos + 1);
  b.d = sload(a.info, 4 * pos + 2);
  if constexpr (FOLD != 0) {
    const int32_t* rec = a.fold + (size_t)kIbFoldRec * node;
    b.fc = sload(rec, 0);
    b.fv0 = sload(rec, 1);
    b.fv1 = sload(rec, 2);
    b.fd0 = sload(rec, 3);
    b.fd1 = sload(rec, 4);
  }
  b.off = (uint32_t)(chunk * (256 * W) + lane * 4 * W);
  b.cwb = chunk * (512 * W) + lane * 8 * W;
#pragma unroll
  for (int j = 0; j < MAXD; ++j) {
    const int e = b.st + min(j, b.d - 1);
    const uint8_t* row = GATHER ? a.ch8 + (size_t)sload(a.gather, e) * a.ldb : a.in + (size_t)e * a.ldb;
    load_row<W, VN ? (bool)IBL_NT : ((bool)IBL_NT_CN && !GATHER)>(row + b.off, b.row[j]);
  }
  if (VN) {
    load_row<W, IBL_NT>(a.ch8 + (size_t)node * a.ldb + b.off, b.chw);
  } else {
#pragma unroll
    for (int i = 0; i < W; ++i) b.chw[i] = 0;
  }
  b.tgv = (uint32_t)a.tgt[b.st + min(lane, b.d - 1)];
}

template <bool VN, class Buf>
__device__ __forceinline__ void settle(const Buf& b) {
  constexpr int W = Buf::W;
#pragma unroll
  for (int j = 0; j < Buf::kMax; ++j)
#pragma unroll
    for (int i = 0; i < W; ++i) asm volatile("" ::"v"(b.row[j][i]));
  if constexpr (VN) {
#pragma unroll
    for (int i = 0; i < W; ++i) asm volatile("" ::"v"(b.chw[i]));
  }
  asm volatile("" ::"v"(b.tgv));
}

__device__ __forceinline__ uint32_t pack4n(uint32_t acc, const uint32_t (&t)[4], int g) {
  return g == 0 ? pk<3>(pk<2>(pk<1>(pk<0>(acc, t[0]), t[1]), t[2]), t[3])
                : pk<7>(pk<6>(pk<5>(pk<4>(acc, t[0]), t[1]), t[2]), t[3]);
}

#ifndef IBL_SCHED_FILE
#define IBL_SCHED_FILE "ib_sched.inc"
#endif
#include IBL_SCHED_FILE
#ifndef IBL_UNROLLED_FILE
#define IBL_UNROLLED_FILE "ib_unrolled.inc"
#endif
template <int D, int MAXD = 8> constexpr bool kWordCT = D <= 8 && MAXD <= 8;
#include IBL_UNROLLED_FILE
template <int D, int K0, int ST>
__device__ __forceinline__ void cn_group_ct(uint32_t lane4, const uint32_t (&in)[D], uint32_t fbase, uint32_t (&o)[D]) {
  cn_group_fold_ct<D, 0, K0, ST>(lane4, in, fbase, 0u, 0u, 0u, o);
}

template <int NCW> constexpr int kWordST = NCW == 8 ? 2 : 1;
template <int S, int NCW>
__host__ __device__ constexpr int word_k0(int gi) {
  if (kWordST<NCW> == 1) return gi * S;
  const int npp = 4 / S;
  return gi / npp + (gi % npp) * 2 * S;
}
template <int D, int GI, int NCW>
__device__ __forceinline__ void cn_word_ct(uint32_t lane4, const uint32_t (&in)[D], uint32_t fbase,
                                           uint32_t (&outw)[D]) {
  constexpr int S = cn_sched_s(D);
  static_assert(S == 2 || S == 4, "parity groups of 2 or 4 codewords");
  cn_group_ct<D, word_k0<S, NCW>(GI), kWordST<NCW>>(lane4, in, fbase, outw);
  if constexpr ((GI + 1) * S < NCW) {
    __builtin_amdgcn_sched_barrier(0);
    cn_word_ct<D, GI + 1, NCW>(lane4, in, fbase, outw);
  }
}
template <int D, int NCW = 8, bool CT = false>
__device__ __forceinline__ void cn_word(uint32_t lane4, const uint32_t (&in)[D], uint32_t fbase,
                                        uint32_t (&outw)[D]) {
  if constexpr (CT) {
    cn_word_ct<D, 0, NCW>(lane4, in, fbase, outw);
  } else {
#pragma unroll 1
    for (int k0 = 0; k0 < NCW; k0 += cn_sched_s(D)) cn_group<D>(lane4, in, fbase, outw, k0);
  }
}

template <int D, int FC, int GI = 0>
__device__ __forceinline__ void cn_word_fold(uint32_t lane4, const uint32_t (&in)[D], uint32_t fbase,
                                             uint32_t lane4c, uint32_t ch0, uint32_t ch1, uint32_t (&outw)[D]) {
  constexpr int S = cn_sched_s(D);
  static_assert(S == 2 || S == 4, "parity groups of 2 or 4 codewords");
  cn_group_fold_ct<D, FC, word_k0<S, 8>(GI), kWordST<8>>(lane4, in, fbase, lane4c, ch0, ch1, outw);
  if constexpr ((GI + 1) * S < 8) {
    __builtin_amdgcn_sched_barrier(0);
    cn_word_fold<D, FC, GI + 1>(lane4, in, fbase, lane4c, ch0, ch1, outw);
  }
}
__device__ __forceinline__ uint32_t fold_word(uint32_t w, uint32_t ch, uint32_t lane4c) {
  uint32_t r = 0;
#pragma unroll
  for (int g = 0; g < 2; ++g) {
    uint32_t t[4];
#pragma unroll
    for (int s = 0; s < 4; ++s) t[s] = luc(nib(w, 4 * g + s), colq(ch, 4 * g + s, lane4c), 0u);
    r = pack4n(r, t, g);
  }
  return r;
}

template <int D, bool GATHER, class Buf, int FC = 0, bool KEEP = false>
__device__ __forceinline__ void cn_compute(const IbFastArgs& a, uint32_t lane4, const Buf& b,
                                           int fslot, bool do_par, bool& unsat, uint8_t* fout = nullptr) {
  constexpr int W = Buf::W;
  uint32_t outw[D][W], trow[D];
  uint32_t chf[2][W] = {};
  if constexpr (FC != 0 && !GATHER) {
    if constexpr ((FC & 1) != 0) load_row<W>(a.ch8 + (size_t)b.fv0 * (uint32_t)a.ldb + b.off, chf[0]);
    if constexpr ((FC & 2) != 0) load_row<W>(a.ch8 + (size_t)b.fv1 * (uint32_t)a.ldb + b.off, chf[1]);
  }
#pragma unroll
  for (int w = 0; w < D; ++w) trow[w] = __builtin_amdgcn_readlane(b.tgv, w);
  const uint32_t fbase = slot_off(fslot);
  if (do_par) {
    const uint32_t bias = (uint32_t)(8 - a.half) * 0x11111111u;
    uint32_t any = 0;
#pragma unroll
    for (int i = 0; i < W; ++i) {
      uint32_t x = (D & 1) ? 0x88888888u : 0u;
#pragma unroll
      for (int j = 0; j < D; ++j) x ^= b.row[j][i] + bias;
      any |= x & 0x88888888u & valid_nib8(a.B - b.cwb - 8 * i);
    }
    if (__ballot(any != 0) != 0ull) unsat = true;
  }
#pragma unroll
  for (int i = 0; i < W; ++i) {
    uint32_t in[D], o[D];
    if constexpr (kWordCT<D, Buf::kMax>) {
      if (i) __builtin_amdgcn_sched_barrier(0);
    }
#pragma unroll
    for (int j = 0; j < D; ++j) {
      in[j] = b.row[j][i];
      o[j] = 0;
    }
    if constexpr (D == 2) {
      if (a.match) {
#pragma unroll
        for (int g = 0; g < 2; ++g) {
          uint32_t t0[4], t1[4];
#pragma unroll
          for (int s = 0; s < 4; ++s) {
            t0[s] = lu((nib(in[1], 4 * g + s) << kRowSh) + lane4, fbase);
            t1[s] = lu((nib(in[0], 4 * g + s) << kRowSh) + lane4, fbase);
          }
          o[0] = pack4n(o[0], t0, g);
          o[1] = pack4n(o[1], t1, g);
        }
      } else {
        o[0] = in[1];
        o[1] = in[0];
      }
    } else if constexpr (FC != 0 && !KEEP) {
      const uint32_t c0 = GATHER ? in[D - 2] : chf[0][i], c1 = GATHER ? in[D - 1] : chf[1][i];
      cn_word_fold<D, FC>(lane4, in, fbase, lane4 + slot_off(a.fold_slot), c0, c1, o);
    } else {
      cn_word<D, 8, kWordCT<D, Buf::kMax>>(lane4, in, fbase, o);
    }
#pragma unroll
    for (int w = 0; w < D; ++w) outw[w][i] = o[w];
  }
  if constexpr (FC == 0 || KEEP) {
#pragma unroll
    for (int w = 0; w < D; ++w) store_row<W, (bool)IBL_NT_CN>(a.out + (size_t)trow[w] * (uint32_t)a.ldb + b.off, outw[w]);
  }
  if constexpr (FC != 0 && KEEP) {
    const uint32_t lane4c = lane4 + slot_off(a.fold_slot);
#pragma unroll
    for (int fa = 0; fa < 2; ++fa) {
      if (!((FC >> fa) & 1)) continue;
      uint32_t fw[W];
#pragma unroll
      for (int i = 0; i < W; ++i) fw[i] = fold_word(outw[D - 2 + fa][i], GATHER ? b.row[D - 2 + fa][i] : chf[fa][i], lane4c);
      store_row<W, (bool)IBL_NT_CN>(fout + (size_t)(uint32_t)(fa ? b.fd1 : b.fd0) * (uint32_t)a.ldb + b.off, fw);
    }
  } else if constexpr (FC != 0) {
#pragma unroll
    for (int w = 0; w < D - 2; ++w) store_row<W, (bool)IBL_NT_CN>(a.out + (size_t)trow[w] * (uint32_t)a.ldb + b.off, outw[w]);
    if constexpr ((FC & 1) != 0) {
      store_row<W, (bool)IBL_NT_CN>(fout + (size_t)(uint32_t)b.fd0 * (uint32_t)a.ldb + b.off, outw[D - 2]);
    } else {
      store_row<W, (bool)IBL_NT_CN>(a.out + (size_t)trow[D - 2] * (uint32_t)a.ldb + b.off, outw[D - 2]);
    }
    if constexpr ((FC & 2) != 0) {
      store_row<W, (bool)IBL_NT_CN>(fout + (size_t)(uint32_t)b.fd1 * (uint32_t)a.ldb + b.off, outw[D - 1]);
    } else {
      store_row<W, (bool)IBL_NT_CN>(a.out + (size_t)trow[D - 1] * (uint32_t)a.ldb + b.off, outw[D - 1]);
    }
  }
}

template <int D, bool GATHER, bool KEEP, class Buf>
__device__ __forceinline__ void cn_compute_fold(const IbFastArgs& a, uint32_t lane4, const Buf& b,
                                                int fslot, bool do_par, bool& unsat) {
  if constexpr (D >= 3 && D <= 8) {
    uint8_t* fout = a.fout;
    asm volatile("" : "+s"(fout));
    switch (b.fc) {
      case 1: cn_compute<D, GATHER, Buf, 1, KEEP>(a, lane4, b, fslot, do_par, unsat, fout); return;
      case 2: cn_compute<D, GATHER, Buf, 2, KEEP>(a, lane4, b, fslot, do_par, unsat, fout); return;
      case 3: cn_compute<D, GATHER, Buf, 3, KEEP>(a, lane4, b, fslot, do_par, unsat, fout); return;
      default: break;
    }
  }
  cn_compute<D, GATHER>(a, lane4, b, fslot, do_par, unsat);
}

template <int D, int GI, int NCW>
__device__ __forceinline__ void vn_word_ct(uint32_t lane4, const uint32_t (&in)[D], uint32_t chw,
                                           uint32_t fbase, uint32_t (&outw)[D]) {
  constexpr int S = vn_sched_s(D);
  static_assert(S == 2 || S == 4, "parity groups of 2 or 4 codewords");
  vn_group_ct<D, word_k0<S, NCW>(GI), kWordST<NCW>>(lane4, in, fbase, chw, outw);
  if constexpr ((GI + 1) * S < NCW) {
    __builtin_amdgcn_sched_barrier(0);
    vn_word_ct<D, GI + 1, NCW>(lane4, in, chw, fbase, outw);
  }
}
template <int D, int NCW = 8, bool CT = false>
__device__ __forceinline__ void vn_word(uint32_t lane4, const uint32_t (&in)[D], uint32_t chw,
                                        uint32_t fbase, uint32_t (&outw)[D]) {
  if constexpr (CT) {
    vn_word_ct<D, 0, NCW>(lane4, in, chw, fbase, outw);
  } else {
#pragma unroll 1
    for (int k0 = 0; k0 < NCW; k0 += vn_sched_s(D)) vn_group<D>(lane4, in, chw, fbase, outw, k0);
  }
}

template <int D, class Buf>
__device__ __forceinline__ void vn_compute(const IbFastArgs& a, uint32_t lane4, const Buf& b,
                                           int fslot) {
  constexpr int W = Buf::W;
  uint32_t outw[D][W], trow[D];
#pragma unroll
  for (int w = 0; w < D; ++w) trow[w] = __builtin_amdgcn_readlane(b.tgv, w);
  const uint32_t fbase = slot_off(fslot);
#pragma unroll
  for (int i = 0; i < W; ++i) {
    if constexpr (D == 1) {
      outw[0][i] = b.chw[i];
    } else {
      uint32_t in[D], o[D];
#pragma unroll
      for (int j = 0; j < D; ++j) {
        in[j] = b.row[j][i];
        o[j] = 0;
      }
      vn_word<D>(lane4, in, b.chw[i], fbase, o);
#pragma unroll
      for (int w = 0; w < D; ++w) outw[w][i] = o[w];
    }
  }
#pragma unroll
  for (int w = 0; w < D; ++w) store_row<W, IBL_NT>(a.out + (size_t)trow[w] * (uint32_t)a.ldb + b.off, outw[w]);
}

__device__ __forceinline__ void store4(void* out, int dtype, size_t row_off, int cw0, int B, bool aligned,
                                       uint32_t packed) {
  if (dtype == kU8) {
    uint8_t* p = reinterpret_cast<uint8_t*>(out) + row_off + cw0;
    if (aligned && cw0 + 4 <= B) {
      *reinterpret_cast<uint32_t*>(p) = packed;
    } else {
#pragma unroll
      for (int s = 0; s < 4; ++s)
        if (cw0 + s < B) p[s] = (uint8_t)(packed >> (8 * s));
    }
  } else {
    int32_t* p = reinterpret_cast<int32_t*>(out) + row_off + cw0;
    if (aligned && cw0 + 4 <= B) {
      int4 v = make_int4(packed & 0xff, (packed >> 8) & 0xff, (packed >> 16) & 0xff, packed >> 24);
      *reinterpret_cast<int4*>(p) = v;
    } else {
#pragma unroll
      for (int s = 0; s < 4; ++s)
        if (cw0 + s < B) p[s] = (int32_t)((packed >> (8 * s)) & 0xff);
    }
  }
}

template <int D>
__device__ __forceinline__ void dec_item(const IbDecArgs& a, uint32_t lane4, int node,
                                         int st, uint32_t off, int cwb) {
  uint32_t inw[D];
#pragma unroll
  for (int j = 0; j < D; ++j) inw[j] = *reinterpret_cast<const uint32_t*>(a.vin + (size_t)(st + j) * a.ldb + off);
  const uint32_t cw = *reinterpret_cast<const uint32_t*>(a.ch8 + (size_t)node * a.ldb + off);
#pragma unroll
  for (int g = 0; g < 2; ++g) {
    if (cwb + 4 * g >= a.B) break;
    uint32_t packed = 0;
#pragma unroll
    for (int s = 0; s < 4; ++s) {
      const int k = 4 * g + s;
      uint32_t Q = lu((nib(cw, k) << kRowSh) + qidx(nib(inw[0], k), lane4), 0);
#pragma unroll
      for (int l = 1; l < D; ++l) Q = luc(Q, qidx(nib(inw[l], k), lane4), slot_off(l));
      packed |= Q << (8 * s);
    }
    store4(a.out, a.out_dtype, (size_t)node * a.B, cwb + 4 * g, a.B, a.aligned != 0, packed);
  }
}

#define IBL_DEG_CASES(X) X(2) X(3) X(4) X(5) X(6) X(7) X(8) X(9) X(10) X(11) X(12) X(13) X(14) X(15) X(16)
#define IBL_DEG_CASES8(X) X(2) X(3) X(4) X(5) X(6) X(7) X(8)

__device__ __forceinline__ int* lds_counters(const uint8_t* lds, const IbFastArgs& a) {
  return reinterpret_cast<int*>(const_cast<uint8_t*>(lds) + lds_of_quads(a.nt));
}
__device__ __forceinline__ void stage_pass(uint8_t* lds, const IbFastArgs& a) {
  if (threadIdx.x < 2) lds_counters(lds, a)[threadIdx.x] = 0;
  stage_tables(lds, a.img, a.nt);
}

#ifndef IBL_LIGHT_DEPTH
#define IBL_LIGHT_DEPTH 2
#endif
template <class Buf, bool VN, bool GATHER, int DLO, int DEPTH = 2, int FOLD = 0>
__device__ __forceinline__ void ib_phase(const IbFastArgs& a, uint32_t lane4, int lane, int first,
                                         int end, int nw, int wpb, int* ctr, bool do_par, bool& unsat,
                                         uint64_t* trace_items, const PhaseItems pi) {
  auto compute = [&](const Buf& cur) __attribute__((always_inline)) {
    settle<VN>(cur);
    if constexpr (VN) {
      switch (cur.d) {
        case 1: if constexpr (DLO < 1) vn_compute<1>(a, lane4, cur, 0); break;
#define X(D) case D: if constexpr (D > DLO && D <= Buf::kMax) vn_compute<D>(a, lane4, cur, a.fslot[D]); break;
        IBL_DEG_CASES(X)
#undef X
        default: break;
      }
    } else {
      switch (cur.d) {
#define X(D) case D: if constexpr (D > DLO && D <= Buf::kMax) { \
          if constexpr (FOLD != 0) cn_compute_fold<D, GATHER, FOLD == 2>(a, lane4, cur, a.fslot[D], do_par, unsat); \
          else cn_compute<D, GATHER>(a, lane4, cur, a.fslot[D], do_par, unsat); } break;
        IBL_DEG_CASES(X)
#undef X
        default: break;
      }
    }
  };
  const int base = first + (int)blockIdx.x * wpb;
  auto item_of = [&](int k) { return base + (k % wpb) + nw * (k / wpb); };
  int done = 0;
  if constexpr (DEPTH == 3) {
    Buf A, Bb, Cc;
    int ia = item_of(take_ticket(ctr, lane));
    if (ia >= end) return;
    fetch_item<Buf, VN, GATHER, FOLD>(a, ia, lane, A, pi);
    int ib = item_of(take_ticket(ctr, lane));
    fetch_item<Buf, VN, GATHER, FOLD>(a, min(ib, end - 1), lane, Bb, pi);
    int kn = take_ticket(ctr, lane);
    for (;;) {
      int ic = item_of(kn);
      fetch_item<Buf, VN, GATHER, FOLD>(a, min(ic, end - 1), lane, Cc, pi);
      kn = take_ticket(ctr, lane);
      compute(A);
      ++done;
      if (ib >= end) break;
      ia = item_of(kn);
      fetch_item<Buf, VN, GATHER, FOLD>(a, min(ia, end - 1), lane, A, pi);
      kn = take_ticket(ctr, lane);
      compute(Bb);
      ++done;
      if (ic >= end) break;
      ib = item_of(kn);
      fetch_item<Buf, VN, GATHER, FOLD>(a, min(ib, end - 1), lane, Bb, pi);
      kn = take_ticket(ctr, lane);
      compute(Cc);
      ++done;
      if (ia >= end) break;
    }
  } else {
    Buf A, Bb;
    int item = item_of(take_ticket(ctr, lane));
    if (item >= end) return;
    fetch_item<Buf, VN, GATHER, FOLD>(a, item, lane, A, pi);
    int kn = take_ticket(ctr, lane);
    for (;;) {
      int next = item_of(kn);
      fetch_item<Buf, VN, GATHER, FOLD>(a, min(next, end - 1), lane, Bb, pi);
      kn = take_ticket(ctr, lane);
      compute(A);
      ++done;
      if (next >= end) break;
      item = next;
      next = item_of(kn);
      fetch_item<Buf, VN, GATHER, FOLD>(a, min(next, end - 1), lane, A, pi);
      kn = take_ticket(ctr, lane);
      compute(Bb);
      ++done;
      if (next >= end) break;
      item = next;
    }
  }
  if (trace_items && lane == 0) *trace_items += (uint64_t)done;
}

template <int MAXD, bool VN, bool GATHER, int FOLD = 0>
__device__ __forceinline__ void ib_pass(const IbFastArgs& a, const uint8_t* lds) {
  const int lane = threadIdx.x & 63;
  const uint32_t lane4 = (uint32_t)(lane & 31) << 2;
  const int wpb = blockDim.x >> 6;
  const int gw = __builtin_amdgcn_readfirstlane(blockIdx.x * wpb + (threadIdx.x >> 6)), nw = gridDim.x * wpb;
  constexpr int W = rowW<MAXD>();
  constexpr int LW = (VN && MAXD <= 8) ? IBL_LIGHT_W : W;
  const int nch_l = LW == W ? a.nchunks : (a.B + 512 * LW - 1) / (512 * LW);
  const int heavy_end = a.n_heavy * a.nchunks, nitems = heavy_end + (a.n_nodes - a.n_heavy) * nch_l;
  const bool do_par = !VN && !GATHER && a.unsat != nullptr;
  bool unsat = false;
  uint64_t* trace_items = a.trace ? a.trace + 3 * gw + 2 : nullptr;
  if (a.trace && lane == 0) {
    a.trace[3 * gw] = __builtin_readcyclecounter();
    *trace_items = (uint64_t)__smid() << 32;
  }
  int* ctr = lds_counters(lds, a);
#ifndef IBL_MIX16
#define IBL_MIX16 6
#endif
  const bool light_first = VN && (int)(threadIdx.x >> 6) * 16 < wpb * IBL_MIX16;
#pragma unroll 1
  for (int r = 0; r < 2; ++r) {
    if ((r == 0) != light_first)
      ib_phase<ItemBuf<MAXD, W>, VN, GATHER, kLightD, 2, FOLD>(a, lane4, lane, 0, heavy_end, nw, wpb, ctr, do_par, unsat,
                                                      trace_items, PhaseItems{0, 0, a.nchunks});
    else
      ib_phase<ItemBuf<kLightD, LW>, VN, GATHER, 0, (VN ? IBL_LIGHT_DEPTH : 2), FOLD>(a, lane4, lane, heavy_end, nitems, nw, wpb, ctr + 1, do_par,
                                                   unsat, trace_items, PhaseItems{heavy_end, a.n_heavy, nch_l});
  }
  if (a.trace && lane == 0) {
    a.trace[3 * gw + 1] = __builtin_readcyclecounter();
  }
  if (do_par && unsat && lane == 0) atomicOr(&a.unsat[gw & (kShards - 1)], 1);
}

#ifndef IBL_LB8
#define IBL_LB8 1024
#endif
#ifndef IBL_LB16
#define IBL_LB16 512
#endif
#ifndef IBL_WPE8
#define IBL_WPE8 1
#endif
#ifndef IBL_LB8C
#define IBL_LB8C IBL_LB8
#endif
#ifndef IBL_WPE8C
#define IBL_WPE8C IBL_WPE8
#endif
template <int MAXD, bool GATHER, int FOLD = 0>
__global__ __launch_bounds__(MAXD <= 8 ? IBL_LB8C : IBL_LB16, MAXD <= 8 ? IBL_WPE8C : 1) void ib_cn_fast(IbFastArgs a) {
  static_assert(FOLD == 0 || MAXD <= 8, "the max-degree-16 bodies do not fold");
  extern __shared__ __attribute__((aligned(16))) uint8_t lds[];
  if (!gate_open(a.gate, threadIdx.x & 63)) return;
  lds_at_zero(lds);
  stage_pass(lds, a);
  __syncthreads();
  ib_pass<MAXD, false, GATHER, FOLD>(a, lds);
}

template <int MAXD>
__global__ __launch_bounds__(MAXD <= 8 ? IBL_LB8 : IBL_LB16, MAXD <= 8 ? IBL_WPE8 : 1) void ib_vn_fast(IbFastArgs a) {
  extern __shared__ __attribute__((aligned(16))) uint8_t lds[];
  if (!gate_open(a.gate, threadIdx.x & 63)) return;
  lds_at_zero(lds);
  stage_pass(lds, a);
  __syncthreads();
  ib_pass<MAXD, true, false>(a, lds);
}

__global__ __launch_bounds__(1024) void ib_dec_fast(IbDecArgs a) {
  extern __shared__ __attribute__((aligned(16))) uint8_t lds[];
  const int lane = threadIdx.x & 63;
  const int L = __builtin_amdgcn_readfirstlane(*a.iters);
  lds_at_zero(lds);
  stage_tables(lds, a.img + (size_t)L * a.nt * 256, a.nt);
  __syncthreads();
  const uint32_t lane4 = (uint32_t)(lane & 31) << 2;
  const int wpb = blockDim.x >> 6;
  const int gw = blockIdx.x * wpb + (threadIdx.x >> 6), nw = gridDim.x * wpb;
  const int nitems = a.n_nodes * a.nchunks;
  for (int item = gw; item < nitems; item += nw) {
    const int node = __builtin_amdgcn_readfirstlane(item / a.nchunks);
    const int chunk = __builtin_amdgcn_readfirstlane(item - node * a.nchunks);
    const int d = a.deg[node], st = a.start[node];
    const uint32_t off = (uint32_t)(chunk * (kChunkDec / 2) + lane * 4);
    const int cwb = chunk * kChunkDec + lane * 8;
    if (cwb >= a.B) continue;
    switch (d) {
      case 1: dec_item<1>(a, lane4, node, st, off, cwb); break;
#define X(D) case D: dec_item<D>(a, lane4, node, st, off, cwb); break;
      IBL_DEG_CASES(X)
#undef X
      default: break;
    }
  }
}

template <int D, bool GATHER>
__device__ __forceinline__ void cn_small_item(const IbFastArgs& a, uint32_t lane4, int st, int c, bool do_par,
                                              bool& unsat) {
  uint32_t in[D], o[D];
  int tg[D];
  const uint32_t off = 4u * (uint32_t)c;
#pragma unroll
  for (int j = 0; j < D; ++j) {
    const int e = st + j;
    const uint8_t* row = GATHER ? a.ch8 + (size_t)a.gather[e] * a.ldb : a.in + (size_t)e * a.ldb;
    in[j] = *reinterpret_cast<const uint32_t*>(row + off);
    tg[j] = a.tgt[e];
    o[j] = 0;
  }
  if (do_par) {
    const uint32_t bias = (uint32_t)(8 - a.half) * 0x11111111u;
    uint32_t x = (D & 1) ? 0x88888888u : 0u;
#pragma unroll
    for (int j = 0; j < D; ++j) x ^= in[j] + bias;
    if (x & 0x88888888u & valid_nib8(a.B - 8 * c)) unsat = true;
  }
  const uint32_t fbase = slot_off(a.fslot[D]);
  if constexpr (D == 2) {
    if (a.match) {
#pragma unroll
      for (int g = 0; g < 2; ++g) {
        uint32_t t0[4], t1[4];
#pragma unroll
        for (int s = 0; s < 4; ++s) {
          t0[s] = lu((nib(in[1], 4 * g + s) << kRowSh) + lane4, fbase);
          t1[s] = lu((nib(in[0], 4 * g + s) << kRowSh) + lane4, fbase);
        }
        o[0] = pack4n(o[0], t0, g);
        o[1] = pack4n(o[1], t1, g);
      }
    } else {
      o[0] = in[1];
      o[1] = in[0];
    }
  } else {
    if (a.B - 8 * c <= 4) cn_word<D, 4>(lane4, in, fbase, o);
    else cn_word<D>(lane4, in, fbase, o);
  }
// ... 797 lines not shown
    if (d == 1) {
      a.out[(size_t)a.tgt[st] * a.ldb + b] = (uint8_t)c;
      continue;
    }
    for (int w = 0; w < d; ++w) {
      auto other = [&](int pos) -> int64_t { return a.in[(size_t)(st + (pos < w ? pos : pos + 1)) * a.ldb + b]; };
      int64_t x = lut_at(a.lut, a.lut_len, off + c * T + other(0));
      for (int l = 1; l <= d - 2; ++l)
        x = lut_at(a.lut, a.lut_len, off + x * T + other(l) + Tc * T + (int64_t)(l - 1) * T * T);
      if (a.match) x = lut_at(a.mt, a.mt_len, (int64_t)a.pass * T * a.VM + (int64_t)(d - 1) * T + x);
      a.out[(size_t)a.tgt[st + w] * a.ldb + b] = (uint8_t)x;
    }
  }
}

__global__ void ib_dec_gen(IbGenDecArgs a) {
  const int nb = (a.B + blockDim.x - 1) / blockDim.x;
  const int L = *a.iters;
  const int64_t T = a.T, Tc = a.Tc;
  const int64_t off = (int64_t)L * (Tc * T + (int64_t)(a.VM - 1) * T * T);
  for (int it = blockIdx.x; it < a.n_nodes * nb; it += gridDim.x) {
    const int n = it / nb;
    const int b = (it - n * nb) * blockDim.x + threadIdx.x;
    if (b >= a.B) continue;
    const int d = a.deg[n], st = a.start[n];
    const int64_t c = a.ch8[(size_t)n * a.ldb + b];
    int64_t x = lut_at(a.lut, a.lut_len, off + c * T + a.vin[(size_t)st * a.ldb + b]);
    for (int l = 1; l < d; ++l)
      x = lut_at(a.lut, a.lut_len, off + x * T + a.vin[(size_t)(st + l) * a.ldb + b] + Tc * T + (int64_t)(l - 1) * T * T);
    if (a.out_dtype == kU8) reinterpret_cast<uint8_t*>(a.out)[(size_t)n * a.B + b] = (uint8_t)x;
    else reinterpret_cast<int32_t*>(a.out)[(size_t)n * a.B + b] = (int32_t)x;
  }
}

__global__ void finalize_iters(const int32_t* flags, int imax, int early, int32_t* dL, int32_t* user) {
  const int lane = threadIdx.x & 63;
  int L = imax - 1;
  if (early) {
    for (int j = 1; j <= imax - 1; ++j) {
      if (__ballot(flags[(size_t)j * kShards + lane] != 0) == 0ull) {
        L = j;
        break;
      }
    }
  }
  if (lane == 0) {
    *dL = L;
    if (user) *user = L;
  }
}

hipError_t launch_ib_stage(const void* ch, int dtype, int n, int B, uint8_t* ch8, int ldb, hipStream_t s) {
  const size_t total = (size_t)n * (ldb / 4);
  const int grid = (int)std::min<size_t>((total + 255) / 256, 8192);
  hipLaunchKernelGGL(ib_stage, dim3(grid), dim3(256), 0, s, ch, dtype, n, B, ch8, ldb);
  return hipGetLastError();
}
hipError_t launch_ib_stage4(const void* ch, int dtype, int n, int B, uint8_t* ch4, int ldb_bytes, hipStream_t s) {
  const int words = std::min(ldb_bytes / 4, (B + 7) / 8);
  if (words <= 32 && (int64_t)n * words < (1ll << 31)) {
    const int grid = (int)std::max<int64_t>(1, std::min<int64_t>(((int64_t)n * words + 255) / 256, 8192));
    if (dtype == kU8)
      hipLaunchKernelGGL(ib_stage4_words<kU8>, dim3(grid), dim3(256), 0, s, ch, n, B, ch4, ldb_bytes, words);
    else
      hipLaunchKernelGGL(ib_stage4_words<kI32>, dim3(grid), dim3(256), 0, s, ch, n, B, ch4, ldb_bytes, words);
    return hipGetLastError();
  }
  const int64_t nseg = (words + 1023) / 1024, items = (int64_t)n * nseg;
  const int grid = (int)std::max<int64_t>(1, std::min<int64_t>(items, 8192));
  const size_t align = dtype == kU8 ? 8 : 16;
  int vec = (B % 8) == 0 && (reinterpret_cast<uintptr_t>(ch) % align) == 0;
  if (vec && dtype == kU8 && (B % 16) == 0 && (reinterpret_cast<uintptr_t>(ch) % 16) == 0 && (ldb_bytes % 16) == 0)
    vec = 2;
  if (dtype == kU8)
    hipLaunchKernelGGL(ib_stage4<kU8>, dim3(grid), dim3(256), 0, s, ch, n, B, ch4, ldb_bytes, words, nseg, vec);
  else
    hipLaunchKernelGGL(ib_stage4<kI32>, dim3(grid), dim3(256), 0, s, ch, n, B, ch4, ldb_bytes, words, nseg, vec);
  return hipGetLastError();
}
static bool ib_fold_args_ok(const IbFastArgs& a, int maxd) {
  return maxd <= 8 && a.fold && a.fout && a.fold_slot >= 0 && a.fold_slot < 8 * (int)(kLdsBytes / kSuper) &&
         !(a.gather && a.fold_mode == 2);
}
hipError_t launch_ib_cn_fast(const IbFastArgs& a, int maxd, int grid, int block, size_t lds, hipStream_t s) {
  if (a.fold_mode != 0) {
    if (!ib_fold_args_ok(a, maxd)) return hipErrorInvalidValue;
    if (a.gather) hipLaunchKernelGGL((ib_cn_fast<8, true, 1>), dim3(grid), dim3(block), lds, s, a);
    else if (a.fold_mode == 2) hipLaunchKernelGGL((ib_cn_fast<8, false, 2>), dim3(grid), dim3(block), lds, s, a);
    else hipLaunchKernelGGL((ib_cn_fast<8, false, 1>), dim3(grid), dim3(block), lds, s, a);
    return hipGetLastError();
  }
  if (a.gather) {
    if (maxd <= 8) hipLaunchKernelGGL((ib_cn_fast<8, true>), dim3(grid), dim3(block), lds, s, a);
    else hipLaunchKernelGGL((ib_cn_fast<16, true>), dim3(grid), dim3(block), lds, s, a);
  } else {
    if (maxd <= 8) hipLaunchKernelGGL((ib_cn_fast<8, false>), dim3(grid), dim3(block), lds, s, a);
    else hipLaunchKernelGGL((ib_cn_fast<16, false>), dim3(grid), dim3(block), lds, s, a);
  }
  return hipGetLastError();
}
hipError_t launch_ib_vn_fast(const IbFastArgs& a, int maxd, int grid, int block, size_t lds, hipStream_t s) {
  if (maxd <= 8) hipLaunchKernelGGL(ib_vn_fast<8>, dim3(grid), dim3(block), lds, s, a);
  else hipLaunchKernelGGL(ib_vn_fast<16>, dim3(grid), dim3(block), lds, s, a);
  return hipGetLastError();
}
int ib_fast_chunk(int maxd) { return maxd <= 8 ? chunkOf<8>() : chunkOf<16>(); }
static bool ib_small_args_ok(const IbFastArgs& a, bool vn) {
  return a.task && a.info && a.tgt && a.out && a.img && a.ch8 && (a.in || (!vn && a.gather)) && a.n_tasks >= 0 &&
         a.nwords >= 1 && 4 * a.nwords <= a.ldb;
}
hipError_t launch_ib_cn_small(const IbFastArgs& a, int maxd, int grid, size_t lds, hipStream_t s) {
  if (!ib_small_args_ok(a, false)) return hipErrorInvalidValue;
  if (a.gather) {
    if (maxd <= 8) hipLaunchKernelGGL((ib_cn_small<8, true>), dim3(grid), dim3(small_block(a.nwords)), lds, s, a);
    else hipLaunchKernelGGL((ib_cn_small<16, true>), dim3(grid), dim3(small_block(a.nwords)), lds, s, a);
  } else {
    if (maxd <= 8) hipLaunchKernelGGL((ib_cn_small<8, false>), dim3(grid), dim3(small_block(a.nwords)), lds, s, a);
    else hipLaunchKernelGGL((ib_cn_small<16, false>), dim3(grid), dim3(small_block(a.nwords)), lds, s, a);
  }
  return hipGetLastError();
}
hipError_t launch_ib_vn_small(const IbFastArgs& a, int maxd, int grid, size_t lds, hipStream_t s) {
  if (!ib_small_args_ok(a, true)) return hipErrorInvalidValue;
  if (maxd <= 8) hipLaunchKernelGGL(ib_vn_small<8>, dim3(grid), dim3(small_block(a.nwords)), lds, s, a);
  else hipLaunchKernelGGL(ib_vn_small<16>, dim3(grid), dim3(small_block(a.nwords)), lds, s, a);
  return hipGetLastError();
}
hipError_t launch_ib_dec_small(const IbDecArgs& a, int grid, size_t lds, hipStream_t s) {
  if (!a.task || !a.info || !a.vin || !a.img || !a.out || a.nwords < 1 || 4 * a.nwords > a.ldb)
    return hipErrorInvalidValue;
  hipLaunchKernelGGL(ib_dec_small, dim3(grid), dim3(small_block(a.nwords)), lds, s, a);
  return hipGetLastError();
}
hipError_t ib_small_private_bytes(int cn_maxd, int vn_maxd, size_t* bytes, const char** name) {
  const bool c8 = cn_maxd <= 8, v8 = vn_maxd <= 8;
  const struct { const void* f; const char* n; } ks[] = {
      {c8 ? (const void*)ib_cn_small<8, true> : (const void*)ib_cn_small<16, true>, "ib_cn_small<gather>"},
      {c8 ? (const void*)ib_cn_small<8, false> : (const void*)ib_cn_small<16, false>, "ib_cn_small"},
      {v8 ? (const void*)ib_vn_small<8> : (const void*)ib_vn_small<16>, "ib_vn_small"},
      {(const void*)ib_dec_small, "ib_dec_small"}};
  *bytes = 0;
  *name = "";
  for (const auto& k : ks) {
    hipError_t e = hipFuncSetAttribute(k.f, hipFuncAttributeMaxDynamicSharedMemorySize, kLdsBytes);
    if (e != hipSuccess) return e;
    hipFuncAttributes fa;
    e = hipFuncGetAttributes(&fa, k.f);
    if (e != hipSuccess) return e;
    if (fa.localSizeBytes > *bytes) {
      *bytes = fa.localSizeBytes;
      *name = k.n;
    }
  }
  return hipSuccess;
}
hipError_t launch_ib_dec_fast(const IbDecArgs& a, int grid, int block, size_t lds, hipStream_t s) {
  hipLaunchKernelGGL(ib_dec_fast, dim3(grid), dim3(block), lds, s, a);
  return hipGetLastError();
}
hipError_t ib_fast_occupancy(int which, int maxd, int block, size_t lds, int* blocks_per_cu) {
  if (which == 0) {
    for (const void* g : {(const void*)ib_cn_fast<8, true>, (const void*)ib_cn_fast<16, true>,
                          (const void*)ib_cn_fast<8, true, 1>, (const void*)ib_cn_fast<8, false, 1>,
                          (const void*)ib_cn_fast<8, false, 2>}) {
      hipError_t e = hipFuncSetAttribute(g, hipFuncAttributeMaxDynamicSharedMemorySize, kLdsBytes);
      if (e != hipSuccess) return e;
    }
  }
  const void* f = which == 0 ? (maxd <= 8 ? (const void*)ib_cn_fast<8, false> : (const void*)ib_cn_fast<16, false>)
                : which == 1 ? (maxd <= 8 ? (const void*)ib_vn_fast<8> : (const void*)ib_vn_fast<16>)
                             : (const void*)ib_dec_fast;
  hipError_t e = hipFuncSetAttribute(f, hipFuncAttributeMaxDynamicSharedMemorySize, kLdsBytes);
  if (e != hipSuccess) return e;
  hipFuncAttributes fa;
  e = hipFuncGetAttributes(&fa, f);
  if (e != hipSuccess) return e;
  if (block > fa.maxThreadsPerBlock) return hipErrorInvalidValue;
  return hipOccupancyMaxActiveBlocksPerMultiprocessor(blocks_per_cu, f, block, lds);
}
hipError_t ib_fast_private_bytes(int cn_maxd, int vn_maxd, size_t* bytes, const char** name) {
// ... 89 lines not shown
```

informationbottleneckdecodingldpc_amd/csrc/ib_unrolled.inc:

```
static_assert(cn_sched_s(8) == 4 && vn_sched_s(8) == 2,
              "the unrolled bodies were generated for another schedule (IBL_UNROLLED_FILE)");
template <int D, int FC, int K0, int ST> __device__ __forceinline__ void cn_group_fold_ct(uint32_t lane4, const uint32_t (&in)[D], uint32_t fbase, uint32_t lane4c, uint32_t ch0, uint32_t ch1,
    uint32_t (&o)[D]) {
  static_assert(D >= 3 && D <= 8 && K0 >= 0 && (ST == 1 || ST == 2), "unrolled bodies: degrees 3..8");
  if constexpr (D == 3) {
    const uint32_t lane4f = lane4 + fbase;
    IBL_E(E0_1, in[0], in[1]);
    IBL_E(E0_2, in[0], in[2]);
    IBL_E(E1_2, in[1], in[2]);
    IBL_LU14(v_P_0, E0_1, lane4f, 0u);
    IBL_LU14(v_o0_0, E1_2, lane4f, 0u);
    step_fence();
    IBL_QC4(qc1, FC & 2, ch1);
    IBL_LINK4(f_P, FC & 2, v_P_0, qc1);
    IBL_LU14(v_c1_0, E0_2, lane4f, 0u);
    IBL_PK4(o[0], v_o0_0);
    step_fence();
    IBL_QC4(qc0, FC & 1, ch0);
    IBL_LINK4(f_c1, FC & 1, v_c1_0, qc0);
    IBL_PK4(o[2], f_P);
    step_fence();
    IBL_PK4(o[1], f_c1);
    step_fence();
  }
// ... 170 lines not shown
    step_fence();
    IBL_QC4(qc0, FC & 1, ch0);
    IBL_LINK4(f_c5, FC & 1, v_c5_0, qc0);
    step_fence();
    IBL_PK4(o[5], f_c5);
    step_fence();
  }
  if constexpr (D == 8) {
    const uint32_t lane4f = lane4 + fbase;
    IBL_E(E0_1, in[0], in[1]);
    IBL_E(E0_2, in[0], in[2]);
    IBL_E(E1_2, in[1], in[2]);
    IBL_LU14(v_P_0, E0_1, lane4, 0u);
    IBL_LU14(v_o0_0, E1_2, lane4, 0u);
    step_fence();
    IBL_Q4(q2, in[2], lane4);
    IBL_Q4(q3, in[3], lane4);
    IBL_LUC4(v_P_1, v_P_0, q2, 1u);
    IBL_LUC4(v_o0_1, v_o0_0, q3, 1u);
    step_fence();
    IBL_Q4(q4, in[4], lane4);
    IBL_LUC4(v_P_2, v_P_1, q3, 2u);
    IBL_LUC4(v_o0_2, v_o0_1, q4, 2u);
    step_fence();
    IBL_Q4(q5, in[5], lane4);
    IBL_LUC4(v_P_3, v_P_2, q4, 3u);
    IBL_LUC4(v_o0_3, v_o0_2, q5, 3u);
    step_fence();
    IBL_Q4(q6, in[6], lane4);
    IBL_LUC4(v_P_4, v_P_3, q5, 128u);
    IBL_LUC4(v_o0_4, v_o0_3, q6, 128u);
    step_fence();
    IBL_Q4(q7, in[7], lane4f);
    IBL_LUC4(v_P_5, v_P_4, q6, fbase);
    IBL_LUC4(v_o0_5, v_o0_4, q7, 0u);
    step_fence();
    IBL_QC4(qc1, FC & 2, ch1);
    IBL_LINK4(f_P, FC & 2, v_P_5, qc1);
    IBL_LU14(v_c1_0, E0_2, lane4, 0u);
    IBL_LUC4(v_c2_0, v_P_0, q3, 1u);
    IBL_PK4(o[0], v_o0_5);
    step_fence();
    IBL_LUC4(v_c1_1, v_c1_0, q3, 1u);
    IBL_LUC4(v_c2_1, v_c2_0, q4, 2u);
    IBL_PK4(o[7], f_P);
    step_fence();
    IBL_LUC4(v_c1_2, v_c1_1, q4, 2u);
    IBL_LUC4(v_c2_2, v_c2_1, q5, 3u);
    step_fence();
    IBL_LUC4(v_c1_3, v_c1_2, q5, 3u);
    IBL_LUC4(v_c2_3, v_c2_2, q6, 128u);
    step_fence();
    IBL_LUC4(v_c1_4, v_c1_3, q6, 128u);
    IBL_LUC4(v_c2_4, v_c2_3, q7, 0u);
    step_fence();
    IBL_LUC4(v_c1_5, v_c1_4, q7, 0u);
    IBL_LUC4(v_c3_0, v_P_1, q4, 2u);
    IBL_PK4(o[2], v_c2_4);
    step_fence();
    IBL_LUC4(v_c3_1, v_c3_0, q5, 3u);
    IBL_LUC4(v_c4_0, v_P_2, q5, 3u);
    IBL_PK4(o[1], v_c1_5);
    step_fence();
    IBL_LUC4(v_c3_2, v_c3_1, q6, 128u);
    IBL_LUC4(v_c4_1, v_c4_0, q6, 128u);
    step_fence();
    IBL_LUC4(v_c3_3, v_c3_2, q7, 0u);
    IBL_LUC4(v_c4_2, v_c4_1, q7, 0u);
    step_fence();
    IBL_LUC4(v_c5_0, v_P_3, q6, 128u);
    IBL_LUC4(v_c6_0, v_P_4, q7, 0u);
    IBL_PK4(o[3], v_c3_3);
    IBL_PK4(o[4], v_c4_2);
    step_fence();
    IBL_QC4(qc0, FC & 1, ch0);
    IBL_LINK4(f_c6, FC & 1, v_c6_0, qc0);
    IBL_LUC4(v_c5_1, v_c5_0, q7, 0u);
    step_fence();
    IBL_PK4(o[6], f_c6);
    IBL_PK4(o[5], v_c5_1);
    step_fence();
  }
}
template <int D, int K0, int ST> __device__ __forceinline__ void vn_group_ct(uint32_t lane4, const uint32_t (&in)[D], uint32_t fbase, uint32_t chw,
    uint32_t (&o)[D]) {
  static_assert(D >= 2 && D <= 4 && K0 >= 0 && (ST == 1 || ST == 2), "unrolled bodies: degrees 2..4");
  if constexpr (D == 2) {
    const uint32_t lane4f = lane4 + fbase;
    IBL_E(Ec_0, chw, in[0]);
    IBL_E(Ec_1, chw, in[1]);
    IBL_LU12(v_Q_0, Ec_0, lane4f, 0u);
    IBL_LU12(v_o0_0, Ec_1, lane4f, 0u);
    step_fence();
    IBL_PK2(o[1], v_Q_0);
    IBL_PK2(o[0], v_o0_0);
    step_fence();
  }
  if constexpr (D == 3) {
    const uint32_t lane4f = lane4 + fbase;
    IBL_E(Ec_0, chw, in[0]);
    IBL_E(Ec_1, chw, in[1]);
    IBL_LU12(v_Q_0, Ec_0, lane4, 0u);
    IBL_LU12(v_o0_0, Ec_1, lane4, 0u);
    step_fence();
    IBL_Q2(q1, in[1], lane4f);
    IBL_Q2(q2, in[2], lane4f);
    IBL_LUC2(v_Q_1, v_Q_0, q1, 0u);
    IBL_LUC2(v_o0_1, v_o0_0, q2, 0u);
    IBL_LUC2(v_c1_0, v_Q_0, q2, 0u);
    step_fence();
    IBL_PK2(o[2], v_Q_1);
    IBL_PK2(o[0], v_o0_1);
    IBL_PK2(o[1], v_c1_0);
    step_fence();
  }
  if constexpr (D == 4) {
    const uint32_t lane4f = lane4 + fbase;
    IBL_E(Ec_0, chw, in[0]);
    IBL_E(Ec_1, chw, in[1]);
    IBL_LU12(v_Q_0, Ec_0, lane4, 0u);
    IBL_LU12(v_o0_0, Ec_1, lane4, 0u);
    step_fence();
    IBL_Q2(q1, in[1], lane4);
    IBL_Q2(q2, in[2], lane4);
    IBL_LUC2(v_Q_1, v_Q_0, q1, 1u);
    IBL_LUC2(v_o0_1, v_o0_0, q2, 1u);
    IBL_LUC2(v_c1_0, v_Q_0, q2, 1u);
    step_fence();
    IBL_Q2(q3, in[3], lane4f);
    IBL_LUC2(v_Q_2, v_Q_1, q2, fbase);
    IBL_LUC2(v_o0_2, v_o0_1, q3, 0u);
    IBL_LUC2(v_c1_1, v_c1_0, q3, 0u);
    IBL_LUC2(v_c2_0, v_Q_1, q3, 0u);
    step_fence();
    IBL_PK2(o[3], v_Q_2);
    IBL_PK2(o[0], v_o0_2);
    IBL_PK2(o[1], v_c1_1);
    IBL_PK2(o[2], v_c2_0);
    step_fence();
  }
}
```

informationbottleneckdecodingldpc_amd/csrc/plan.h:

```cpp
#pragma once
#include <stddef.h>
#include <stdint.h>

#include <algorithm>
#include <string>
#include <vector>

namespace ibl {

constexpr int kMaxD = 16;
constexpr int kLightD = 4;
constexpr int kFoldRec = 8;

struct HostGraph {
  int32_t n_v = 0, n_c = 0;
  int64_t n_e = 0;
  std::vector<int32_t> h_cn_deg, h_vn_deg;
  std::vector<int32_t> h_cn_start, h_cols, h_vn_start, h_tgt_vn;
};

inline bool map_node_connections(int32_t n_v, int32_t n_c, const int32_t* indptr, const int32_t* cols,
                                 int32_t* cn_start, int32_t* cn_deg, int32_t* tgt_cn, int32_t* vn_start,
                                 int32_t* vn_deg, int32_t* tgt_vn, std::string* err) {
  if (n_v <= 0 || n_c <= 0 || !indptr || !cols) return *err = "empty graph", false;
// ... 76 lines not shown
    const int32_t e1 = g.h_tgt_vn[(size_t)g.h_vn_start[v]], e2 = g.h_tgt_vn[(size_t)g.h_vn_start[v] + 1];
    const int32_t c1 = chk_of[(size_t)e1], c2 = chk_of[(size_t)e2];
    if (used[c1] >= 2 || used[c2] >= 2) continue;
    auto put = [&](int32_t c, int32_t e, int32_t other) {
      int32_t* r = &(*rec)[(size_t)kFoldRec * c];
      const int k = used[c]++;
      r[k] = e - g.h_cn_start[c];
      r[2 + k] = other;
      r[4 + k] = v;
    };
    put(c1, e1, e2);
    put(c2, e2, e1);
    folded[v] = 1;
    ++n;
  }
  rest->clear();
  for (int32_t v = 0; v < nv; ++v)
    if (!folded[v]) rest->push_back(v);
  return n;
}

constexpr int kIbFoldRec = 8;
inline int32_t plan_ib_fold(const HostGraph& g, std::vector<int32_t>* rec, std::vector<int32_t>* rest) {
  const int32_t nc = g.n_c, nv = g.n_v;
  rec->assign((size_t)nc * kIbFoldRec, 0);
  std::vector<int32_t> chk_of(g.h_cols.size());
  for (int32_t c = 0; c < nc; ++c) {
    int32_t* r = &(*rec)[(size_t)kIbFoldRec * c];
    const int32_t d = g.h_cn_deg[c], st = g.h_cn_start[c];
    for (int32_t k = 0; k < d; ++k) chk_of[(size_t)st + k] = c;
    for (int a = 0; a < 2; ++a) {
      r[1 + a] = d >= 2 ? g.h_cols[(size_t)st + d - 2 + a] : 0;
      r[3 + a] = -1;
    }
  }
  auto tail_pos = [&](int32_t e) {
    const int32_t c = chk_of[(size_t)e], d = g.h_cn_deg[c], k = e - g.h_cn_start[c];
    return d >= 3 && k >= d - 2 ? k - (d - 2) : -1;
  };
  rest->clear();
  int32_t n = 0;
  for (int32_t v = 0; v < nv; ++v) {
    int32_t a1 = -1, a2 = -1, e1 = 0, e2 = 0;
    if (g.h_vn_deg[v] == 2) {
      e1 = g.h_tgt_vn[(size_t)g.h_vn_start[v]];
      e2 = g.h_tgt_vn[(size_t)g.h_vn_start[v] + 1];
      a1 = tail_pos(e1);
      a2 = tail_pos(e2);
    }
    if (a1 < 0 || a2 < 0) {
      rest->push_back(v);
      continue;
    }
    int32_t* r1 = &(*rec)[(size_t)kIbFoldRec * chk_of[(size_t)e1]];
    int32_t* r2 = &(*rec)[(size_t)kIbFoldRec * chk_of[(size_t)e2]];
    r1[0] |= 1 << a1;
    r1[3 + a1] = e2;
    r2[0] |= 1 << a2;
    r2[3 + a2] = e1;
    ++n;
  }
  return n;
}

inline std::vector<int32_t> work_order_keyed(const std::vector<int32_t>& nodes, const std::vector<int32_t>& start,
                                             const std::vector<int32_t>& deg, const std::vector<int32_t>* key,
                                             int32_t* heavy) {
  std::vector<int32_t> idx(nodes);
  auto kof = [&](int32_t x) { return key ? (*key)[(size_t)x] : 0; };
  std::stable_sort(idx.begin(), idx.end(), [&](int32_t x, int32_t y) {
    return deg[x] != deg[y] ? deg[x] > deg[y] : kof(x) < kof(y);
  });
  std::vector<int32_t> info(idx.size() * 4);
  *heavy = 0;
  for (size_t p = 0; p < idx.size(); ++p) {
    const int32_t v = idx[p];
    info[4 * p] = v;
    info[4 * p + 1] = start[v];
    info[4 * p + 2] = deg[v];
    info[4 * p + 3] = kof(v);
    if (deg[v] > kLightD) ++*heavy;
  }
  return info;
}

struct FusedTasks {
  std::vector<int32_t> cn_task, vn_task, vn_node, vn_slot;
};

inline void build_fused_tasks(const HostGraph& g, FusedTasks* ft, bool bank_order, size_t vwin) {
  const int64_t E = g.n_e;
  vwin = std::max<size_t>(1, vwin);
  const std::vector<int32_t>& tgt_vn = g.h_tgt_vn;
  auto starts = [](const std::vector<int32_t>& deg) {
    std::vector<int64_t> st(deg.size() + 1, 0);
    for (size_t i = 0; i < deg.size(); ++i) st[i + 1] = st[i] + deg[i];
    return st;
  };
  auto sorted = [](const std::vector<int32_t>& deg) {
    std::vector<int32_t> idx(deg.size());
    for (size_t i = 0; i < idx.size(); ++i) idx[i] = (int32_t)i;
    std::stable_sort(idx.begin(), idx.end(), [&](int32_t x, int32_t y) { return deg[x] > deg[y]; });
    return idx;
  };
  const std::vector<int64_t> cst = starts(g.h_cn_deg), vst = starts(g.h_vn_deg);
  std::vector<int32_t> slot_of((size_t)E);
  {
    const std::vector<int32_t> ord = sorted(g.h_cn_deg);
    int32_t slot = 0;
    for (size_t i = 0; i < ord.size();) {
      const int32_t d = g.h_cn_deg[ord[i]];
      int32_t cnt = 0;
      while (i + cnt < ord.size() && cnt < 64 && g.h_cn_deg[ord[i + cnt]] == d) ++cnt;
      ft->cn_task.insert(ft->cn_task.end(), {slot, cnt, d, 0});
      for (int32_t l = 0; l < cnt; ++l)
        for (int32_t k = 0; k < d; ++k) slot_of[(size_t)cst[ord[i + l]] + k] = slot + k * cnt + l;
      slot += cnt * d;
      i += cnt;
    }
  }
  {
    std::vector<int32_t> ord = sorted(g.h_vn_deg);
    for (size_t i0 = 0; bank_order && i0 < ord.size();) {
      const int32_t d = g.h_vn_deg[ord[i0]];
      size_t i1 = i0;
      while (i1 < ord.size() && g.h_vn_deg[ord[i1]] == d) ++i1;
      std::vector<int32_t> pool(ord.begin() + (long)i0, ord.begin() + (long)i1), res;
      res.reserve(pool.size());
      auto bank = [&](int32_t v, int k) { return (uint32_t)slot_of[(size_t)tgt_vn[(size_t)vst[v] + k]] & 31u; };
      while (!pool.empty()) {
        uint32_t used[kMaxD + 1] = {0};
        for (int lane = 0; lane < 32 && !pool.empty(); ++lane) {
          size_t best = 0;
          int bestc = 1 << 30;
          const size_t win = std::min<size_t>(pool.size(), vwin);
          for (size_t c = 0; c < win && bestc > 0; ++c) {
            int col = 0;
            for (int k = 0; k < d && k <= kMaxD; ++k) col += (used[k] >> bank(pool[c], k)) & 1u;
            if (col < bestc) { bestc = col; best = c; }
          }
          const int32_t v = pool[best];
          for (int k = 0; k < d && k <= kMaxD; ++k) used[k] |= 1u << bank(v, k);
          res.push_back(v);
          pool.erase(pool.begin() + (long)best);
        }
      }
      std::copy(res.begin(), res.end(), ord.begin() + (long)i0);
      i0 = i1;
    }
    int32_t sidx = 0;
    for (size_t i = 0; i < ord.size();) {
      const int32_t d = g.h_vn_deg[ord[i]];
      int32_t cnt = 0;
      while (i + cnt < ord.size() && cnt < 64 && g.h_vn_deg[ord[i + cnt]] == d) ++cnt;
      ft->vn_task.insert(ft->vn_task.end(), {(int32_t)i, cnt, d, sidx});
      ft->vn_slot.resize((size_t)sidx + (size_t)cnt * d);
      for (int32_t l = 0; l < cnt; ++l) {
        const int32_t v = ord[i + l];
        ft->vn_node.push_back(v);
        for (int32_t k = 0; k < d; ++k) ft->vn_slot[(size_t)sidx + k * cnt + l] = slot_of[(size_t)tgt_vn[(size_t)vst[v] + k]];
      }
      sidx += cnt * d;
      i += cnt;
    }
  }
}
// ... 135 lines not shown
```

informationbottleneckdecodingldpc_amd/engine.py:

```python
from __future__ import annotations

import ctypes
from typing import Optional

import numpy as np
import torch

from . import _lib
from .graph import EdgeGraph, build_graph
from .tables import IBTables

_DT_IB = {torch.uint8: _lib.IBL_U8, torch.int32: _lib.IBL_I32}
_DT_FL = {torch.float32: _lib.IBL_F32, torch.float64: _lib.IBL_F64}
_DT_ANY = {torch.uint8: _lib.IBL_U8, torch.int32: _lib.IBL_I32, torch.float32: _lib.IBL_F32,
           torch.float64: _lib.IBL_F64}


def _require_gpu(device) -> torch.device:
    if not torch.cuda.is_available():
        raise RuntimeError("no HIP device visible: the LDPC decoders run only on the GPU (no CPU fallback)")
    dev = torch.device("cuda", torch.cuda.current_device()) if device is None else torch.device(device)
    if dev.type != "cuda":
        raise ValueError(f"decoder device must be a HIP (cuda) device, got {dev}")
    if dev.index is None:
        dev = torch.device("cuda", torch.cuda.current_device())
    return dev


def _stream_ptr(dev: torch.device) -> int:
    return torch.cuda.current_stream(dev).cuda_stream


def _check_tensor(t: torch.Tensor, dev: torch.device, n_rows: int, name: str) -> None:
    if not isinstance(t, torch.Tensor) or t.device != dev:
        raise ValueError(f"{name} must be a tensor on {dev}")
    if t.dim() != 2 or t.shape[0] != n_rows or not t.is_contiguous():
        raise ValueError(f"{name} must be a contiguous [{n_rows}][B] tensor, got {tuple(t.shape)}")


class Graph:

    def __init__(self, H_or_graph, device=None):
        self.device = _require_gpu(device)
        self.edges: EdgeGraph = H_or_graph if isinstance(H_or_graph, EdgeGraph) else build_graph(H_or_graph)
        g = self.edges
        L = _lib.load()
        h = ctypes.c_void_p()
        _lib.check(L.ibl_graph_create(g.n_v, g.n_c, np.ascontiguousarray(g.csr_indptr, np.int32),
                                      np.ascontiguousarray(g.csr_cols, np.int32), self.device.index,
                                      ctypes.byref(h)), "ibl_graph_create")
        self._h = h

    @property
    def handle(self):
        return self._h

    def __del__(self):
        h = getattr(self, "_h", None)
        if h is not None and h.value:
            try:
                _lib.load().ibl_graph_destroy(h)
            except Exception:
                pass
            self._h = None


class IBDecoder:

    _PATHS = {"auto": _lib.IBL_PATH_AUTO, "passes": _lib.IBL_PATH_PASSES, "fused": _lib.IBL_PATH_FUSED}

    def __init__(self, graph: Graph, tables: IBTables, match: bool, max_batch: int, force_generic: bool = False,
                 path: str = "auto", fold: bool = True):
        self.graph = graph
        self.tables = tables
        self.match = bool(match)
        self.max_batch = int(max_batch)
        self.device = graph.device
        tb = tables
        cn = np.ascontiguousarray(tb.cn, np.int32)
        vn = np.ascontiguousarray(tb.vn, np.int32)
        mc = np.ascontiguousarray(tb.match_cn if tb.match_cn is not None else np.zeros(1), np.int32)
        mv = np.ascontiguousarray(tb.match_vn if tb.match_vn is not None else np.zeros(1), np.int32)
        h = ctypes.c_void_p()
        L = _lib.load()
        _lib.check(L.ibl_ib_create(graph.handle, tb.Tc, tb.T, tb.imax, cn, cn.size, vn, vn.size, mc, mc.size,
                                   mv, mv.size, int(self.match), self.max_batch,
                                   _lib.IBL_FLAG_FORCE_GENERIC if force_generic else 0, ctypes.byref(h)),
                   "ibl_ib_create")
        self._h = h
        self.fast_path = bool(L.ibl_ib_path(h))
        if path not in self._PATHS:
            raise ValueError(f"path must be one of {sorted(self._PATHS)}")
        _lib.check(L.ibl_ib_set_path(h, self._PATHS[path]), "ibl_ib_set_path")
        if not fold:
            self.fold = False

    @property
    def fused(self) -> bool:
        f = ctypes.c_int32()
        _lib.check(_lib.load().ibl_ib_path_in_use(self._h, ctypes.byref(f)), "ibl_ib_path_in_use")
        return bool(f.value)

    @property
    def small_batch(self) -> int:
        n = ctypes.c_int32()
        _lib.check(_lib.load().ibl_ib_small_batch(self._h, ctypes.byref(n)), "ibl_ib_small_batch")
        return int(n.value)

    @small_batch.setter
    def small_batch(self, max_b: int) -> None:
        _lib.check(_lib.load().ibl_ib_set_small_batch(self._h, int(max_b)), "ibl_ib_set_small_batch")

    @property
    def folded(self) -> int:
        f = ctypes.c_int32()
        _lib.check(_lib.load().ibl_ib_folded(self._h, ctypes.byref(f)), "ibl_ib_folded")
        return int(f.value)

    @property
    def fold(self) -> bool:
        return getattr(self, "_fold", True)

    @fold.setter
    def fold(self, on: bool) -> None:
        _lib.check(_lib.load().ibl_ib_set_fold(self._h, int(bool(on))), "ibl_ib_set_fold")
        self._fold = bool(on)

    def fused_ncw(self, B: int) -> int:
        n = ctypes.c_int32()
        _lib.check(_lib.load().ibl_ib_fused_ncw(self._h, int(B), ctypes.byref(n)), "ibl_ib_fused_ncw")
        return int(n.value)

    def decode(self, ch: torch.Tensor, out: Optional[torch.Tensor] = None, out_dtype=torch.int32,
               early_stop=True, iters: Optional[torch.Tensor] = None) -> torch.Tensor:
        each = isinstance(early_stop, str)
        if each and early_stop != "codeword":
            raise ValueError('early_stop must be True, False or "codeword"')
        n = self.graph.edges.n_v
        _check_tensor(ch, self.device, n, "channel values")
        if ch.dtype not in _DT_IB:
            raise ValueError("channel values must be uint8 or int32")
        B = ch.shape[1]
        if out is None:
            out = torch.empty((n, B), dtype=out_dtype, device=self.device)
        _check_tensor(out, self.device, n, "output")
        if out.dtype not in _DT_IB or out.shape[1] != B:
            raise ValueError("output must be uint8/int32 [N][B]")
        it_ptr = None
        if iters is not None:
            if iters.dtype != torch.int32 or iters.device != self.device or iters.numel() < 1:
                raise ValueError("iters must be an int32 device tensor")
            if each and (iters.numel() < B or not iters.is_contiguous()):
                raise ValueError("iters must be a contiguous int32 device tensor of at least B entries")
            it_ptr = iters.data_ptr()
        if each:
            _lib.check(_lib.load().ibl_ib_decode_each(self._h, ch.data_ptr(), _DT_IB[ch.dtype], B, out.data_ptr(),
                                                      _DT_IB[out.dtype], it_ptr, _stream_ptr(self.device)),
                       "ibl_ib_decode_each")
            return out
        _lib.check(_lib.load().ibl_ib_decode(self._h, ch.data_ptr(), _DT_IB[ch.dtype], B, out.data_ptr(),
                                             _DT_IB[out.dtype], int(bool(early_stop)), it_ptr,
                                             _stream_ptr(self.device)), "ibl_ib_decode")
        return out

    def __del__(self):
        h = getattr(self, "_h", None)
        if h is not None and h.value:
            try:
                _lib.load().ibl_ib_destroy(h)
            except Exception:
                pass
            self._h = None


class FloatDecoder:

    _PATHS = {"auto": _lib.IBL_PATH_AUTO, "passes": _lib.IBL_PATH_PASSES, "fused": _lib.IBL_PATH_FUSED}

    def __init__(self, graph: Graph, kind: int, imax: int, max_batch: int, precision=torch.float32,
                 llr_max: float = 150.0, path: str = "auto", alpha: float = 1.0, beta: float = 0.0):
        self.graph = graph
        self.kind = int(kind)
        self.imax = int(imax)
        self.max_batch = int(max_batch)
        self.precision = precision
        self.device = graph.device
        corrected = not (float(alpha) == 1.0 and float(beta) == 0.0)
        if corrected and self.kind != _lib.IBL_MINSUM:
            raise ValueError("alpha / beta correct min-sum (kind=0) only")
        h = ctypes.c_void_p()
        if corrected:
            _lib.check(_lib.load().ibl_float_create_corrected(graph.handle, float(alpha), float(beta), self.imax,
                                                              float(llr_max), _DT_FL[precision], self.max_batch,
                                                              ctypes.byref(h)), "ibl_float_create_corrected")
        else:
            _lib.check(_lib.load().ibl_float_create(graph.handle, self.kind, self.imax, float(llr_max),
                                                    _DT_FL[precision], self.max_batch, ctypes.byref(h)),
                       "ibl_float_create")
        self._h = h
        if path not in self._PATHS:
            raise ValueError(f"path must be one of {sorted(self._PATHS)}")
        _lib.check(_lib.load().ibl_float_set_path(h, self._PATHS[path]), "ibl_float_set_path")

    @property
    def correction(self):
        a, b = ctypes.c_double(), ctypes.c_double()
        _lib.check(_lib.load().ibl_float_correction(self._h, ctypes.byref(a), ctypes.byref(b)), "ibl_float_correction")
        return float(a.value), float(b.value)

# ... 366 lines not shown
```

Baseline: 201,500.

## Add composite two-step CN lookup table for dominant check degree

Precomputes, per iteration, a composite table that folds the last two CN lookup steps into one 32-bit LDS word indexed by two input nibbles. The unrolled check-node bodies for degrees 5 to 8 then do one word lookup plus a nibble extract where they previously chained two byte lookups. This shortens the serial LDS dependency chain in the CN pass. In exchange it costs an extra 64 KiB of LDS per block, and it is enabled only when that LDS budget leaves the block and grid configuration unchanged.

```diff
diff --git a/include/ibldpc.h b/include/ibldpc.h
--- a/include/ibldpc.h
+++ b/include/ibldpc.h
@@ -44,6 +44,8 @@
 int ibl_ib_small_batch(const ibl_ib* h, int32_t* max_b);
 int ibl_ib_folded(const ibl_ib* h, int32_t* n_folded);
 int ibl_ib_set_fold(ibl_ib* h, int32_t on);
+int ibl_ib_composite(const ibl_ib* h, int32_t* degree);
+int ibl_ib_set_composite(ibl_ib* h, int32_t on);
 int ibl_ib_fused_ncw(const ibl_ib* h, int32_t B, int32_t* ncw);
 int ibl_ib_decode(ibl_ib* h, const void* d_ch, int32_t ch_dtype, int32_t B, void* d_out, int32_t out_dtype,
                   int32_t early_stop, int32_t* d_iters, void* stream);
diff --git a/informationbottleneckdecodingldpc_amd/_lib.py b/informationbottleneckdecodingldpc_amd/_lib.py
--- a/informationbottleneckdecodingldpc_amd/_lib.py
+++ b/informationbottleneckdecodingldpc_amd/_lib.py
@@ -19,6 +19,7 @@
     "ibl_graph_create", "ibl_graph_info", "ibl_graph_destroy",
     "ibl_ib_create", "ibl_ib_path", "ibl_ib_set_path", "ibl_ib_path_in_use", "ibl_ib_fused_ncw", "ibl_ib_decode",
     "ibl_ib_set_small_batch", "ibl_ib_small_batch", "ibl_ib_folded", "ibl_ib_set_fold",
+    "ibl_ib_composite", "ibl_ib_set_composite",
     "ibl_ib_destroy",
     "ibl_float_create", "ibl_float_decode", "ibl_float_destroy", "ibl_count_below",
     "ibl_float_set_path", "ibl_float_path_in_use", "ibl_float_fused_geometry", "ibl_float_folded",
@@ -80,6 +81,8 @@
     L.ibl_ib_small_batch.argtypes = [_vp, ctypes.POINTER(_i32)]
     L.ibl_ib_folded.argtypes = [_vp, ctypes.POINTER(_i32)]
     L.ibl_ib_set_fold.argtypes = [_vp, _i32]
+    L.ibl_ib_composite.argtypes = [_vp, ctypes.POINTER(_i32)]
+    L.ibl_ib_set_composite.argtypes = [_vp, _i32]
     L.ibl_ib_decode.argtypes = [_vp, _vp, _i32, _i32, _vp, _i32, _i32, _vp, _vp]
     L.ibl_ib_decode_each.argtypes = [_vp, _vp, _i32, _i32, _vp, _i32, _vp, _vp]
     L.ibl_ib_destroy.argtypes = [_vp]
diff --git a/informationbottleneckdecodingldpc_amd/csrc/capi_ib.hip b/informationbottleneckdecodingldpc_amd/csrc/capi_ib.hip
--- a/informationbottleneckdecodingldpc_amd/csrc/capi_ib.hip
+++ b/informationbottleneckdecodingldpc_amd/csrc/capi_ib.hip
@@ -21,6 +21,9 @@
   std::vector<int32_t> fold_rec, fold_cn_info, fold_vn_info;
   DevBuf<uint8_t> cin2;
   DevBuf<int32_t> fold, cn_info_f, vn_info_r;
+  int32_t comp_deg = 0;
+  bool comp_on = true;
+  DevBuf<uint32_t> cn_comp;
   int32_t path = IBL_PATH_AUTO;
   bool fused_ok = false, f_half_ok = false;
   bool f_each_ok = false;
@@ -51,7 +54,7 @@
   int cn_nt = 0, vn_nt = 0;
 };
 struct IbImages {
-  std::vector<uint32_t> cn_img, vn_img, dec_img;
+  std::vector<uint32_t> cn_img, vn_img, dec_img, cn_comp;
 };
 
 Table make_table(int T, const std::function<int(int, int)>& f) {
@@ -82,8 +85,8 @@
 
 size_t fast_lds(int nt) { return lds_of_quads(regions_of(nt)) + 64; }
 
-int pick_cfg(int which, int maxd, int nt, int num_cus, KCfg* k) {
-  k->lds = fast_lds(nt);
+int pick_cfg(int which, int maxd, int nt, int num_cus, KCfg* k, size_t extra = 0) {
+  k->lds = fast_lds(nt) + extra;
   int best_waves = 0;
   for (int block : {1024, 768, 640, 512, 384, 256}) {
     int bpc = 0;
@@ -167,6 +170,7 @@
       h->fold_rec.swap(rec);
     }
   }
+  if (h->fast) h->comp_deg = ib_composite_degree(g->h_cn_deg, CM, sl.cn_nt);
   return sl;
 }
 
@@ -174,12 +178,7 @@
   const int Tc = h->Tc, T = h->T, imax = h->imax, CM = h->CM, VM = h->VM;
   IbImages im;
   const int64_t T2 = (int64_t)T * T;
-  auto cn_raw = [&](int p, int l, int t, int m) -> int {
-    int64_t idx;
-    if (p == 0) idx = (l == 0) ? (int64_t)t * Tc + m : (int64_t)Tc * Tc + (int64_t)(l - 1) * Tc * T + (int64_t)t * T + m;
-    else idx = (int64_t)Tc * Tc + (int64_t)(CM - 3) * Tc * T + (int64_t)(p - 1) * (CM - 2) * T2 + l * T2 + (int64_t)t * T + m;
-    return lu.cn[idx];
-  };
+  auto cn_raw = [&](int p, int l, int t, int m) -> int { return lu.cn[ib_cn_raw_index(Tc, T, CM, p, l, t, m)]; };
   auto vn_raw = [&](int k, int l, int t, int m) -> int {
     const int64_t off = (int64_t)k * ((int64_t)Tc * T + (int64_t)(VM - 1) * T2);
     const int64_t idx = off + (l == 0 ? (int64_t)t * T + m : (int64_t)Tc * T + (int64_t)(l - 1) * T2 + (int64_t)t * T + m);
@@ -203,6 +202,10 @@
       }));
     }
     append_pass(im.cn_img, tbs, regions_of(sl.cn_nt));
+    if (h->comp_deg) {
+      im.cn_comp.resize((size_t)(p + 1) * 512);
+      ib_composite_pass(lu.cn, lu.mc, h->match != 0, T, CM, p, h->comp_deg, &im.cn_comp[(size_t)p * 512]);
+    }
   }
   h->cn_nt = regions_of(sl.cn_nt);
   for (int k = 0; k < std::max(imax - 1, 1); ++k) {
@@ -294,6 +297,14 @@
       (rc = pick_cfg(1, VM, 4 * h->vn_nt, g->num_cus, &h->kvn)) ||
       (rc = pick_cfg(2, VM, 4 * h->dec_nt, g->num_cus, &h->kdec)))
     return rc;
+  if (h->comp_deg) {
+    KCfg kc;
+    if (pick_cfg(0, CM, 4 * h->cn_nt, g->num_cus, &kc, kIbCompBytes) != IBL_OK || kc.block != h->kcn.block ||
+        kc.grid != h->kcn.grid)
+      h->comp_deg = 0;
+    else if ((rc = h->cn_comp.upload(im.cn_comp)))
+      return rc;
+  }
   size_t priv = 0;
   const char* kname = "";
   HIPCHK(ib_fast_private_bytes(CM, VM, &priv, &kname));
@@ -520,7 +531,11 @@
   vn.nchunks = (B + cvn - 1) / cvn;
   cn.in = nullptr; cn.gather = g->csr_cols; cn.img = h->cn_img; cn.gate = nullptr; cn.unsat = nullptr;
   cn_fold(0);
-  auto launch_cn = [&]() { return launch_ib_cn_fast(cn, h->CM, h->kcn.grid, h->kcn.block, h->kcn.lds, s); };
+  const int comp = h->comp_on ? h->comp_deg : 0;
+  const uint32_t* cimg = comp ? h->cn_comp.get() : nullptr;
+  auto launch_cn = [&]() {
+    return launch_ib_cn_fast(cn, h->CM, h->kcn.grid, h->kcn.block, h->kcn.lds + (comp ? kIbCompBytes : 0), s, cimg, comp);
+  };
   HIPCHK(h->timer.timed(0, s, launch_cn));
   cn.gather = nullptr;
   uint64_t* trace = nullptr;
@@ -543,6 +558,7 @@
     vn.out = cb[j & 1];
     HIPCHK(h->timer.timed(1, s, [&] { return launch_ib_vn_fast(vn, h->VM, h->kvn.grid, h->kvn.block, h->kvn.lds, s); }));
     cn.img = h->cn_img + (size_t)j * h->cn_nt * 256;
+    if (comp) cimg = h->cn_comp + (size_t)j * 512;
     cn.gate = gate;
     cn.unsat = flag_row(h->flags, early, j);
     cn.trace = (trace && j == I / 2) ? trace + 3 * nwv : nullptr;
@@ -685,6 +701,18 @@
   return IBL_OK;
 }
 
+int ibl_ib_composite(const ibl_ib* h, int32_t* degree) {
+  if (!h || !degree) return fail(IBL_EINVAL, "NULL argument");
+  *degree = h->comp_on ? h->comp_deg : 0;
+  return IBL_OK;
+}
+
+int ibl_ib_set_composite(ibl_ib* h, int32_t on) {
+  if (!h) return fail(IBL_EINVAL, "decoder is NULL");
+  h->comp_on = on != 0;
+  return IBL_OK;
+}
+
 int ibl_ib_timing(ibl_ib* h, int32_t enable) { return timing_enable(h, enable); }
 int ibl_ib_timing_read(ibl_ib* h, double* cn_ms, int32_t* cn_n, double* vn_ms, int32_t* vn_n) {
   return timing_read(h, cn_ms, cn_n, vn_ms, vn_n);
diff --git a/informationbottleneckdecodingldpc_amd/csrc/common.h b/informationbottleneckdecodingldpc_amd/csrc/common.h
--- a/informationbottleneckdecodingldpc_amd/csrc/common.h
+++ b/informationbottleneckdecodingldpc_amd/csrc/common.h
@@ -22,6 +22,7 @@
 constexpr int kChunkDec = 512;
 constexpr int kTbl = 8192;
 constexpr int kSuper = 65536;
+static_assert(kIbCompBytes == (size_t)kSuper, "the composite table is one super-region of the quad layout");
 constexpr int kRowSh = 12, kColSh = 8;
 __host__ __device__ constexpr uint32_t quad_off(int q) { return (uint32_t)(q >> 1) * kSuper + (uint32_t)(q & 1) * 128u; }
 __host__ __device__ constexpr uint32_t slot_off(int s) { return quad_off(s >> 2) + (uint32_t)(s & 3); }
@@ -30,6 +31,10 @@
 constexpr int kTP = 16;
 constexpr int kShards = 64;
 constexpr int kLdsBytes = 160 * 1024;
+static_assert(kIbLdsBytes == (size_t)kLdsBytes && ib_table_lds(1) == lds_of_quads(regions_of(1)) &&
+                  ib_table_lds(7) == lds_of_quads(regions_of(7)) && ib_table_lds(9) == lds_of_quads(regions_of(9)) &&
+                  ib_table_lds(16) == lds_of_quads(regions_of(16)),
+              "plan.h restates the table layout's LDS size for ib_composite_degree");
 
 enum Dtype : int32_t { kU8 = 1, kI32 = 2, kF32 = 3, kF64 = 4, kI8 = 5 };
 
@@ -192,7 +197,8 @@
 
 hipError_t launch_ib_stage(const void* ch, int dtype, int n, int B, uint8_t* ch8, int ldb, hipStream_t s);
 hipError_t launch_ib_stage4(const void* ch, int dtype, int n, int B, uint8_t* ch4, int ldb_bytes, hipStream_t s);
-hipError_t launch_ib_cn_fast(const IbFastArgs& a, int maxd, int grid, int block, size_t lds, hipStream_t s);
+hipError_t launch_ib_cn_fast(const IbFastArgs& a, int maxd, int grid, int block, size_t lds, hipStream_t s,
+                             const uint32_t* cimg = nullptr, int comp = 0);
 hipError_t launch_ib_vn_fast(const IbFastArgs& a, int maxd, int grid, int block, size_t lds, hipStream_t s);
 int ib_fast_chunk(int maxd);
 hipError_t launch_ib_dec_fast(const IbDecArgs& a, int grid, int block, size_t lds, hipStream_t s);
diff --git a/informationbottleneckdecodingldpc_amd/csrc/ib_kernels.hip b/informationbottleneckdecodingldpc_amd/csrc/ib_kernels.hip
--- a/informationbottleneckdecodingldpc_amd/csrc/ib_kernels.hip
+++ b/informationbottleneckdecodingldpc_amd/csrc/ib_kernels.hip
@@ -16,6 +16,17 @@
   static_assert(kRowSh == 12, "luc's shift is the row shift of the table layout");
   asm("v_lshl_or_b32 %0, %1, 12, %2" : "=v"(x) : "v"(t), "v"(q));
   return *(lds8_t*)(size_t)(x + c);
+}
+typedef __attribute__((address_space(3))) const uint32_t lds32_t;
+__device__ __forceinline__ uint32_t lucw(uint32_t t, uint32_t q) {
+  uint32_t x;
+  asm("v_lshl_or_b32 %0, %1, 12, %2" : "=v"(x) : "v"(t), "v"(q));
+  return *(lds32_t*)(size_t)x;
+}
+__device__ __forceinline__ uint32_t cnib(uint32_t w, uint32_t sh) {
+  uint32_t r;
+  asm("v_bfe_u32 %0, %1, %2, 4" : "=v"(r) : "v"(w), "v"(sh));
+  return r;
 }
 __device__ __forceinline__ uint32_t lds_base(const uint8_t* p) { return (uint32_t)(size_t)(lds8_t*)p; }
 __device__ __forceinline__ void lds_at_zero(const uint8_t* lds) {
@@ -74,6 +85,16 @@
 }
 __device__ __forceinline__ uint32_t colb(uint32_t e, int k, uint32_t lane4) {
   return __builtin_amdgcn_perm(e, lane4, 0x03020000u | ((4u + (uint32_t)(k >> 1)) << 8));
+}
+__device__ __forceinline__ uint32_t colk(uint32_t w, uint32_t y, int k, uint32_t lane4k) {
+  const uint32_t src = (k & 1) ? ((w >> 4) & 0x0F0F0F0Fu) : (w & 0x0F0F0F0Fu);
+  const uint32_t hy = (k & 1) ? (y & 0x80808080u) : ((y << 4) & 0x80808080u);
+  const uint32_t b = (uint32_t)(k >> 1);
+  return __builtin_amdgcn_perm(src, hy, 0x0C0C0000u | ((4u + b) << 8) | b) | lane4k;
+}
+__device__ __forceinline__ uint32_t shk(uint32_t y, int k) {
+  const uint32_t s = (k & 1) ? ((y >> 2) & 0x1C1C1C1Cu) : ((y << 2) & 0x1C1C1C1Cu);
+  return s >> (8 * (k >> 1));
 }
 template <int K>
 __device__ __forceinline__ uint32_t pk(uint32_t acc, uint32_t t) {
@@ -98,6 +119,10 @@
 #define IBL_LU1_(s, n, e, base, c) n##_##s = lu(colb(IBL_EP(e, s), K0 + ST * s, base), c)
 #define IBL_LINK_(s, n, on, p, q) n##_##s = (on) ? luc(p##_##s, q##_##s, 0u) : p##_##s
 #define IBL_PK_(s, o, v) o = pk<K0 + ST * s>(o, v##_##s)
+#define IBL_QK_(s, q, w, y, base) q##_##s = colk(w, y, K0 + ST * s, base)
+#define IBL_SH_(s, h, y) h##_##s = shk(y, LS ? ((K0 + ST * s) & 1) : K0 + ST * s)
+#define IBL_LUK_(s, n, p, q) n##_##s = lucw(p##_##s, q##_##s)
+#define IBL_PKK_(s, o, v, h) o = pk<K0 + ST * s>(o, cnib(v##_##s, LS ? h##_##s >> (8 * ((K0 + ST * s) >> 1)) : h##_##s))
 #define IBL_Q2(...) const uint32_t IBL_X2(IBL_Q_, __VA_ARGS__)
 #define IBL_Q4(...) const uint32_t IBL_X4(IBL_Q_, __VA_ARGS__)
 #define IBL_QC2(...) const uint32_t IBL_X2(IBL_QC_, __VA_ARGS__)
@@ -110,6 +135,14 @@
 #define IBL_LINK4(...) const uint32_t IBL_X4(IBL_LINK_, __VA_ARGS__)
 #define IBL_PK2(...) IBL_X2(IBL_PK_, __VA_ARGS__)
 #define IBL_PK4(...) IBL_X4(IBL_PK_, __VA_ARGS__)
+#define IBL_QK2(...) const uint32_t IBL_X2(IBL_QK_, __VA_ARGS__)
+#define IBL_QK4(...) const uint32_t IBL_X4(IBL_QK_, __VA_ARGS__)
+#define IBL_SH2(...) const uint32_t IBL_X2(IBL_SH_, __VA_ARGS__)
+#define IBL_SH4(...) const uint32_t IBL_X4(IBL_SH_, __VA_ARGS__)
+#define IBL_LUK2(...) const uint32_t IBL_X2(IBL_LUK_, __VA_ARGS__)
+#define IBL_LUK4(...) const uint32_t IBL_X4(IBL_LUK_, __VA_ARGS__)
+#define IBL_PKK2(...) IBL_X2(IBL_PKK_, __VA_ARGS__)
+#define IBL_PKK4(...) IBL_X4(IBL_PKK_, __VA_ARGS__)
 
 __device__ __forceinline__ uint32_t valid_nib8(int remaining) {
   return remaining >= 8 ? 0xFFFFFFFFu : (remaining <= 0 ? 0u : ((1u << (4 * remaining)) - 1u));
@@ -263,6 +296,7 @@
 #define IBL_UNROLLED_FILE "ib_unrolled.inc"
 #endif
 template <int D, int MAXD = 8> constexpr bool kWordCT = D <= 8 && MAXD <= 8;
+template <int D, int MAXD> constexpr bool kCompD = D >= 5 && D <= 8 && MAXD <= 8;
 #include IBL_UNROLLED_FILE
 template <int D, int K0, int ST>
 __device__ __forceinline__ void cn_group_ct(uint32_t lane4, const uint32_t (&in)[D], uint32_t fbase, uint32_t (&o)[D]) {
@@ -298,15 +332,16 @@
   }
 }
 
-template <int D, int FC, int GI = 0>
+template <int D, int FC, int GI = 0, bool CP = false, bool LS = false>
 __device__ __forceinline__ void cn_word_fold(uint32_t lane4, const uint32_t (&in)[D], uint32_t fbase,
                                              uint32_t lane4c, uint32_t ch0, uint32_t ch1, uint32_t (&outw)[D]) {
   constexpr int S = cn_sched_s(D);
   static_assert(S == 2 || S == 4, "parity groups of 2 or 4 codewords");
-  cn_group_fold_ct<D, FC, word_k0<S, 8>(GI), kWordST<8>>(lane4, in, fbase, lane4c, ch0, ch1, outw);
+  if constexpr (CP) cn_group_fold_cp<D, FC, word_k0<S, 8>(GI), kWordST<8>, LS>(lane4, in, fbase, lane4c, ch0, ch1, outw);
+  else cn_group_fold_ct<D, FC, word_k0<S, 8>(GI), kWordST<8>>(lane4, in, fbase, lane4c, ch0, ch1, outw);
   if constexpr ((GI + 1) * S < 8) {
     __builtin_amdgcn_sched_barrier(0);
-    cn_word_fold<D, FC, GI + 1>(lane4, in, fbase, lane4c, ch0, ch1, outw);
+    cn_word_fold<D, FC, GI + 1, CP, LS>(lane4, in, fbase, lane4c, ch0, ch1, outw);
   }
 }
 __device__ __forceinline__ uint32_t fold_word(uint32_t w, uint32_t ch, uint32_t lane4c) {
@@ -321,9 +356,10 @@
   return r;
 }
 
-template <int D, bool GATHER, class Buf, int FC = 0, bool KEEP = false>
+template <int D, bool GATHER, class Buf, int FC = 0, bool KEEP = false, bool CP = false>
 __device__ __forceinline__ void cn_compute(const IbFastArgs& a, uint32_t lane4, const Buf& b,
                                            int fslot, bool do_par, bool& unsat, uint8_t* fout = nullptr) {
+  static_assert(!CP || kCompD<D, Buf::kMax>, "composite bodies: degrees 5..8 of the degree <= 8 kernels");
   constexpr int W = Buf::W;
   uint32_t outw[D][W], trow[D];
   uint32_t chf[2][W] = {};
@@ -376,9 +412,10 @@
       }
     } else if constexpr (FC != 0 && !KEEP) {
       const uint32_t c0 = GATHER ? in[D - 2] : chf[0][i], c1 = GATHER ? in[D - 1] : chf[1][i];
-      cn_word_fold<D, FC>(lane4, in, fbase, lane4 + slot_off(a.fold_slot), c0, c1, o);
+      cn_word_fold<D, FC, 0, CP, GATHER>(lane4, in, fbase, lane4 + slot_off(a.fold_slot), c0, c1, o);
     } else {
-      cn_word<D, 8, kWordCT<D, Buf::kMax>>(lane4, in, fbase, o);
+      if constexpr (CP) cn_word_fold<D, 0, 0, true, GATHER>(lane4, in, fbase, 0u, 0u, 0u, o);
+      else cn_word<D, 8, kWordCT<D, Buf::kMax>>(lane4, in, fbase, o);
     }
 #pragma unroll
     for (int w = 0; w < D; ++w) outw[w][i] = o[w];
@@ -413,20 +450,25 @@
   }
 }
 
-template <int D, bool GATHER, bool KEEP, class Buf>
+template <int D, bool GATHER, bool KEEP, bool CP, class Buf>
 __device__ __forceinline__ void cn_compute_fold(const IbFastArgs& a, uint32_t lane4, const Buf& b,
                                                 int fslot, bool do_par, bool& unsat) {
   if constexpr (D >= 3 && D <= 8) {
     uint8_t* fout = a.fout;
     asm volatile("" : "+s"(fout));
     switch (b.fc) {
-      case 1: cn_compute<D, GATHER, Buf, 1, KEEP>(a, lane4, b, fslot, do_par, unsat, fout); return;
-      case 2: cn_compute<D, GATHER, Buf, 2, KEEP>(a, lane4, b, fslot, do_par, unsat, fout); return;
-      case 3: cn_compute<D, GATHER, Buf, 3, KEEP>(a, lane4, b, fslot, do_par, unsat, fout); return;
+      case 1: cn_compute<D, GATHER, Buf, 1, KEEP, CP>(a, lane4, b, fslot, do_par, unsat, fout); return;
+      case 2: cn_compute<D, GATHER, Buf, 2, KEEP, CP>(a, lane4, b, fslot, do_par, unsat, fout); return;
+      case 3: cn_compute<D, GATHER, Buf, 3, KEEP, CP>(a, lane4, b, fslot, do_par, unsat, fout); return;
       default: break;
     }
   }
-  cn_compute<D, GATHER>(a, lane4, b, fslot, do_par, unsat);
+  cn_compute<D, GATHER, Buf, 0, false, CP>(a, lane4, b, fslot, do_par, unsat);
+}
+template <int D, bool GATHER, int FOLD, bool CP, class Buf>
+__device__ __forceinline__ void cn_item(const IbFastArgs& a, uint32_t lane4, const Buf& b, bool do_par, bool& unsat) {
+  if constexpr (FOLD != 0) cn_compute_fold<D, GATHER, FOLD == 2, CP>(a, lane4, b, a.fslot[D], do_par, unsat);
+  else cn_compute<D, GATHER, Buf, 0, false, CP>(a, lane4, b, a.fslot[D], do_par, unsat);
 }
 
 template <int D, int GI, int NCW>
@@ -529,12 +571,38 @@
 #define IBL_DEG_CASES(X) X(2) X(3) X(4) X(5) X(6) X(7) X(8) X(9) X(10) X(11) X(12) X(13) X(14) X(15) X(16)
 #define IBL_DEG_CASES8(X) X(2) X(3) X(4) X(5) X(6) X(7) X(8)
 
-__device__ __forceinline__ int* lds_counters(const uint8_t* lds, const IbFastArgs& a) {
-  return reinterpret_cast<int*>(const_cast<uint8_t*>(lds) + lds_of_quads(a.nt));
+__device__ __forceinline__ int* lds_counters(const uint8_t* lds, const IbFastArgs& a, bool comp = false) {
+  return reinterpret_cast<int*>(const_cast<uint8_t*>(lds) + lds_of_quads(a.nt) + (comp ? (size_t)kSuper : 0));
 }
 __device__ __forceinline__ void stage_pass(uint8_t* lds, const IbFastArgs& a) {
   if (threadIdx.x < 2) lds_counters(lds, a)[threadIdx.x] = 0;
   stage_tables(lds, a.img, a.nt);
+}
+__device__ __forceinline__ void stage_pass_comp(uint8_t* lds, const IbFastArgs& a, const uint32_t* cimg) {
+  if (threadIdx.x < 2) lds_counters(lds, a, true)[threadIdx.x] = 0;
+  const int nraw = a.nt * 256, nall = nraw + 512, qc = 2 * ((a.nt + 1) >> 1), lane = threadIdx.x & 63;
+  const int wv = threadIdx.x >> 6, nwv = blockDim.x >> 6, nchunk = nall >> 6;
+  for (int c0 = 0; c0 < nchunk; c0 += kStageR * nwv) {
+    uint32_t v[kStageR];
+#pragma unroll
+    for (int k = 0; k < kStageR; ++k) {
+      const int r = (c0 + wv + k * nwv) * 64 + lane;
+      v[k] = r < nraw ? a.img[r] : (r < nall ? cimg[r - nraw] : 0u);
+    }
+#pragma unroll
+    for (int k = 0; k < kStageR; ++k) {
+      const int c = c0 + wv + k * nwv;
+      if (c >= nchunk) break;
+#pragma unroll
+      for (int p = 0; p < 8; ++p) {
+        const int src = 8 * p + (lane >> 3), r = c * 64 + src;
+        const uint32_t w = __shfl(v[k], src, 64);
+        const int q = r < nraw ? r >> 8 : qc + ((r - nraw) >> 8);
+        *reinterpret_cast<uint4*>(lds + quad_off(q) + (uint32_t)(r & 255) * 256u + 16u * (uint32_t)(lane & 7)) =
+            make_uint4(w, w, w, w);
+      }
+    }
+  }
 }
 
 #ifndef IBL_LIGHT_DEPTH
@@ -543,7 +611,7 @@
 template <class Buf, bool VN, bool GATHER, int DLO, int DEPTH = 2, int FOLD = 0>
 __device__ __forceinline__ void ib_phase(const IbFastArgs& a, uint32_t lane4, int lane, int first,
                                          int end, int nw, int wpb, int* ctr, bool do_par, bool& unsat,
-                                         uint64_t* trace_items, const PhaseItems pi) {
+                                         uint64_t* trace_items, const PhaseItems pi, int comp = 0) {
   auto compute = [&](const Buf& cur) __attribute__((always_inline)) {
     settle<VN>(cur);
     if constexpr (VN) {
@@ -557,8 +625,14 @@
     } else {
       switch (cur.d) {
 #define X(D) case D: if constexpr (D > DLO && D <= Buf::kMax) { \
-          if constexpr (FOLD != 0) cn_compute_fold<D, GATHER, FOLD == 2>(a, lane4, cur, a.fslot[D], do_par, unsat); \
-          else cn_compute<D, GATHER>(a, lane4, cur, a.fslot[D], do_par, unsat); } break;
+          if constexpr (kCompD<D, Buf::kMax>) { \
+            if (comp == D) { \
+              asm volatile("; composite item");    \
+              cn_item<D, GATHER, FOLD, true>(a, lane4, cur, do_par, unsat); \
+              break; \
+            } \
+          } \
+          cn_item<D, GATHER, FOLD, false>(a, lane4, cur, do_par, unsat); } break;
         IBL_DEG_CASES(X)
 #undef X
         default: break;
@@ -623,7 +697,7 @@
 }
 
 template <int MAXD, bool VN, bool GATHER, int FOLD = 0>
-__device__ __forceinline__ void ib_pass(const IbFastArgs& a, const uint8_t* lds) {
+__device__ __forceinline__ void ib_pass(const IbFastArgs& a, const uint8_t* lds, int comp = 0) {
   const int lane = threadIdx.x & 63;
   const uint32_t lane4 = (uint32_t)(lane & 31) << 2;
   const int wpb = blockDim.x >> 6;
@@ -639,7 +713,7 @@
     a.trace[3 * gw] = __builtin_readcyclecounter();
     *trace_items = (uint64_t)__smid() << 32;
   }
-  int* ctr = lds_counters(lds, a);
+  int* ctr = lds_counters(lds, a, comp != 0);
 #ifndef IBL_MIX16
 #define IBL_MIX16 6
 #endif
@@ -648,10 +722,10 @@
   for (int r = 0; r < 2; ++r) {
     if ((r == 0) != light_first)
       ib_phase<ItemBuf<MAXD, W>, VN, GATHER, kLightD, 2, FOLD>(a, lane4, lane, 0, heavy_end, nw, wpb, ctr, do_par, unsat,
-                                                      trace_items, PhaseItems{0, 0, a.nchunks});
+                                                      trace_items, PhaseItems{0, 0, a.nchunks}, comp);
     else
       ib_phase<ItemBuf<kLightD, LW>, VN, GATHER, 0, (VN ? IBL_LIGHT_DEPTH : 2), FOLD>(a, lane4, lane, heavy_end, nitems, nw, wpb, ctr + 1, do_par,
-                                                   unsat, trace_items, PhaseItems{heavy_end, a.n_heavy, nch_l});
+                                                   unsat, trace_items, PhaseItems{heavy_end, a.n_heavy, nch_l}, comp);
   }
   if (a.trace && lane == 0) {
     a.trace[3 * gw + 1] = __builtin_readcyclecounter();
@@ -675,14 +749,22 @@
 #define IBL_WPE8C IBL_WPE8
 #endif
 template <int MAXD, bool GATHER, int FOLD = 0>
-__global__ __launch_bounds__(MAXD <= 8 ? IBL_LB8C : IBL_LB16, MAXD <= 8 ? IBL_WPE8C : 1) void ib_cn_fast(IbFastArgs a) {
+__global__ __launch_bounds__(MAXD <= 8 ? IBL_LB8C : IBL_LB16, MAXD <= 8 ? IBL_WPE8C : 1) void ib_cn_fast(IbFastArgs a,
+    const uint32_t* cimg, int comp) {
   static_assert(FOLD == 0 || MAXD <= 8, "the max-degree-16 bodies do not fold");
   extern __shared__ __attribute__((aligned(16))) uint8_t lds[];
   if (!gate_open(a.gate, threadIdx.x & 63)) return;
   lds_at_zero(lds);
-  stage_pass(lds, a);
-  __syncthreads();
-  ib_pass<MAXD, false, GATHER, FOLD>(a, lds);
+  if constexpr (MAXD <= 8) {
+    if (comp != 0) stage_pass_comp(lds, a, cimg);
+    else stage_pass(lds, a);
+    __syncthreads();
+    ib_pass<MAXD, false, GATHER, FOLD>(a, lds, comp);
+  } else {
+    stage_pass(lds, a);
+    __syncthreads();
+    ib_pass<MAXD, false, GATHER, FOLD>(a, lds);
+  }
 }
 
 template <int MAXD>
@@ -1646,20 +1728,24 @@
   return maxd <= 8 && a.fold && a.fout && a.fold_slot >= 0 && a.fold_slot < 8 * (int)(kLdsBytes / kSuper) &&
          !(a.gather && a.fold_mode == 2);
 }
-hipError_t launch_ib_cn_fast(const IbFastArgs& a, int maxd, int grid, int block, size_t lds, hipStream_t s) {
+hipError_t launch_ib_cn_fast(const IbFastArgs& a, int maxd, int grid, int block, size_t lds, hipStream_t s,
+                             const uint32_t* cimg, int comp) {
+  if (comp != 0 && !(maxd <= 8 && comp >= 5 && comp <= 8 && cimg && lds_of_quads(a.nt) == (size_t)kSuper &&
+                     lds >= 2 * (size_t)kSuper + 8))
+    return hipErrorInvalidValue;
   if (a.fold_mode != 0) {
     if (!ib_fold_args_ok(a, maxd)) return hipErrorInvalidValue;
-    if (a.gather) hipLaunchKernelGGL((ib_cn_fast<8, true, 1>), dim3(grid), dim3(block), lds, s, a);
-    else if (a.fold_mode == 2) hipLaunchKernelGGL((ib_cn_fast<8, false, 2>), dim3(grid), dim3(block), lds, s, a);
-    else hipLaunchKernelGGL((ib_cn_fast<8, false, 1>), dim3(grid), dim3(block), lds, s, a);
+    if (a.gather) hipLaunchKernelGGL((ib_cn_fast<8, true, 1>), dim3(grid), dim3(block), lds, s, a, cimg, comp);
+    else if (a.fold_mode == 2) hipLaunchKernelGGL((ib_cn_fast<8, false, 2>), dim3(grid), dim3(block), lds, s, a, cimg, comp);
+    else hipLaunchKernelGGL((ib_cn_fast<8, false, 1>), dim3(grid), dim3(block), lds, s, a, cimg, comp);
     return hipGetLastError();
   }
   if (a.gather) {
-    if (maxd <= 8) hipLaunchKernelGGL((ib_cn_fast<8, true>), dim3(grid), dim3(block), lds, s, a);
-    else hipLaunchKernelGGL((ib_cn_fast<16, true>), dim3(grid), dim3(block), lds, s, a);
+    if (maxd <= 8) hipLaunchKernelGGL((ib_cn_fast<8, true>), dim3(grid), dim3(block), lds, s, a, cimg, comp);
+    else hipLaunchKernelGGL((ib_cn_fast<16, true>), dim3(grid), dim3(block), lds, s, a, cimg, comp);
   } else {
-    if (maxd <= 8) hipLaunchKernelGGL((ib_cn_fast<8, false>), dim3(grid), dim3(block), lds, s, a);
-    else hipLaunchKernelGGL((ib_cn_fast<16, false>), dim3(grid), dim3(block), lds, s, a);
+    if (maxd <= 8) hipLaunchKernelGGL((ib_cn_fast<8, false>), dim3(grid), dim3(block), lds, s, a, cimg, comp);
+    else hipLaunchKernelGGL((ib_cn_fast<16, false>), dim3(grid), dim3(block), lds, s, a, cimg, comp);
   }
   return hipGetLastError();
 }
diff --git a/informationbottleneckdecodingldpc_amd/csrc/ib_unrolled.inc b/informationbottleneckdecodingldpc_amd/csrc/ib_unrolled.inc
--- a/informationbottleneckdecodingldpc_amd/csrc/ib_unrolled.inc
+++ b/informationbottleneckdecodingldpc_amd/csrc/ib_unrolled.inc
@@ -276,6 +276,220 @@
     step_fence();
   }
 }
+template <int D, int FC, int K0, int ST, bool LS> __device__ __forceinline__ void cn_group_fold_cp(uint32_t lane4, const uint32_t (&in)[D], uint32_t fbase, uint32_t lane4c, uint32_t ch0, uint32_t ch1,
+    uint32_t (&o)[D]) {
+  static_assert(D >= 5 && D <= 8 && K0 >= 0 && (ST == 1 || ST == 2), "unrolled bodies: degrees 5..8");
+  if constexpr (D == 5) {
+    const uint32_t lane4f = lane4 + fbase;
+    const uint32_t lane4k = lane4 + kSuper;
+    IBL_E(E0_1, in[0], in[1]);
+    IBL_E(E0_2, in[0], in[2]);
+    IBL_E(E1_2, in[1], in[2]);
+    IBL_LU14(v_P_0, E0_1, lane4, 0u);
+    IBL_LU14(v_o0_0, E1_2, lane4, 0u);
+    step_fence();
+    IBL_Q4(q2, in[2], lane4);
+    IBL_QK4(qk, in[3], in[4], lane4k);
+    IBL_SH4(sh, in[4]);
+    IBL_LUC4(v_P_1, v_P_0, q2, 1u);
+    IBL_LUK4(v_o0_1, v_o0_0, qk);
+    step_fence();
+    IBL_Q4(q3, in[3], lane4f);
+    IBL_LUC4(v_P_2, v_P_1, q3, 0u);
+    IBL_LU14(v_c1_0, E0_2, lane4, 0u);
+    IBL_PKK4(o[0], v_o0_1, sh);
+    step_fence();
+    IBL_QC4(qc1, FC & 2, ch1);
+    IBL_LINK4(f_P, FC & 2, v_P_2, qc1);
+    IBL_LUK4(v_c1_1, v_c1_0, qk);
+    IBL_LUK4(v_c2_0, v_P_0, qk);
+    step_fence();
+    IBL_Q4(q4, in[4], lane4f);
+    IBL_LUC4(v_c3_0, v_P_1, q4, 0u);
+    IBL_PK4(o[4], f_P);
+    IBL_PKK4(o[1], v_c1_1, sh);
+    IBL_PKK4(o[2], v_c2_0, sh);
+    step_fence();
+    IBL_QC4(qc0, FC & 1, ch0);
+    IBL_LINK4(f_c3, FC & 1, v_c3_0, qc0);
+    step_fence();
+    IBL_PK4(o[3], f_c3);
+    step_fence();
+  }
+  if constexpr (D == 6) {
+    const uint32_t lane4f = lane4 + fbase;
+    const uint32_t lane4k = lane4 + kSuper;
+    IBL_E(E0_1, in[0], in[1]);
+    IBL_E(E0_2, in[0], in[2]);
+    IBL_E(E1_2, in[1], in[2]);
+    IBL_LU14(v_P_0, E0_1, lane4, 0u);
+    IBL_LU14(v_o0_0, E1_2, lane4, 0u);
+    step_fence();
+    IBL_Q4(q2, in[2], lane4);
+    IBL_Q4(q3, in[3], lane4);
+    IBL_LUC4(v_P_1, v_P_0, q2, 1u);
+    IBL_LUC4(v_o0_1, v_o0_0, q3, 1u);
+    step_fence();
+    IBL_QK4(qk, in[4], in[5], lane4k);
+    IBL_SH4(sh, in[5]);
+    IBL_LUC4(v_P_2, v_P_1, q3, 2u);
+    IBL_LUK4(v_o0_2, v_o0_1, qk);
+    step_fence();
+    IBL_Q4(q4, in[4], lane4f);
+    IBL_LUC4(v_P_3, v_P_2, q4, 0u);
+    IBL_LU14(v_c1_0, E0_2, lane4, 0u);
+    IBL_PKK4(o[0], v_o0_2, sh);
+    step_fence();
+    IBL_QC4(qc1, FC & 2, ch1);
+    IBL_LINK4(f_P, FC & 2, v_P_3, qc1);
+    IBL_LUC4(v_c1_1, v_c1_0, q3, 1u);
+    IBL_LUC4(v_c2_0, v_P_0, q3, 1u);
+    step_fence();
+    IBL_LUK4(v_c1_2, v_c1_1, qk);
+    IBL_LUK4(v_c2_1, v_c2_0, qk);
+    IBL_PK4(o[5], f_P);
+    step_fence();
+    IBL_Q4(q5, in[5], lane4f);
+    IBL_LUK4(v_c3_0, v_P_1, qk);
+    IBL_LUC4(v_c4_0, v_P_2, q5, 0u);
+    IBL_PKK4(o[1], v_c1_2, sh);
+    IBL_PKK4(o[2], v_c2_1, sh);
+    step_fence();
+    IBL_QC4(qc0, FC & 1, ch0);
+    IBL_LINK4(f_c4, FC & 1, v_c4_0, qc0);
+    IBL_PKK4(o[3], v_c3_0, sh);
+    step_fence();
+    IBL_PK4(o[4], f_c4);
+    step_fence();
+  }
+  if constexpr (D == 7) {
+    const uint32_t lane4f = lane4 + fbase;
+    const uint32_t lane4k = lane4 + kSuper;
+    IBL_E(E0_1, in[0], in[1]);
+    IBL_E(E0_2, in[0], in[2]);
+    IBL_E(E1_2, in[1], in[2]);
+    IBL_LU14(v_P_0, E0_1, lane4, 0u);
+    IBL_LU14(v_o0_0, E1_2, lane4, 0u);
+    step_fence();
+    IBL_Q4(q2, in[2], lane4);
+    IBL_Q4(q3, in[3], lane4);
+    IBL_LUC4(v_P_1, v_P_0, q2, 1u);
+    IBL_LUC4(v_o0_1, v_o0_0, q3, 1u);
+    step_fence();
+    IBL_Q4(q4, in[4], lane4);
+    IBL_LUC4(v_P_2, v_P_1, q3, 2u);
+    IBL_LUC4(v_o0_2, v_o0_1, q4, 2u);
+    step_fence();
+    IBL_QK4(qk, in[5], in[6], lane4k);
+    IBL_SH4(sh, in[6]);
+    IBL_LUC4(v_P_3, v_P_2, q4, 3u);
+    IBL_LUK4(v_o0_3, v_o0_2, qk);
+    step_fence();
+    IBL_Q4(q5, in[5], lane4f);
+    IBL_LUC4(v_P_4, v_P_3, q5, 0u);
+    IBL_LU14(v_c1_0, E0_2, lane4, 0u);
+    IBL_PKK4(o[0], v_o0_3, sh);
+    step_fence();
+    IBL_QC4(qc1, FC & 2, ch1);
+    IBL_LINK4(f_P, FC & 2, v_P_4, qc1);
+    IBL_LUC4(v_c1_1, v_c1_0, q3, 1u);
+    IBL_LUC4(v_c2_0, v_P_0, q3, 1u);
+    step_fence();
+    IBL_LUC4(v_c1_2, v_c1_1, q4, 2u);
+    IBL_LUC4(v_c2_1, v_c2_0, q4, 2u);
+    IBL_PK4(o[6], f_P);
+    step_fence();
+    IBL_LUK4(v_c1_3, v_c1_2, qk);
+    IBL_LUK4(v_c2_2, v_c2_1, qk);
+    step_fence();
+    IBL_LUC4(v_c3_0, v_P_1, q4, 2u);
+    IBL_LUK4(v_c4_0, v_P_2, qk);
+    IBL_PKK4(o[1], v_c1_3, sh);
+    IBL_PKK4(o[2], v_c2_2, sh);
+    step_fence();
+    IBL_Q4(q6, in[6], lane4f);
+    IBL_LUK4(v_c3_1, v_c3_0, qk);
+    IBL_LUC4(v_c5_0, v_P_3, q6, 0u);
+    IBL_PKK4(o[4], v_c4_0, sh);
+    step_fence();
+    IBL_QC4(qc0, FC & 1, ch0);
+    IBL_LINK4(f_c5, FC & 1, v_c5_0, qc0);
+    IBL_PKK4(o[3], v_c3_1, sh);
+    step_fence();
+    IBL_PK4(o[5], f_c5);
+    step_fence();
+  }
+  if constexpr (D == 8) {
+    const uint32_t lane4f = lane4 + fbase;
+    const uint32_t lane4k = lane4 + kSuper;
+    IBL_E(E0_1, in[0], in[1]);
+    IBL_E(E0_2, in[0], in[2]);
+    IBL_E(E1_2, in[1], in[2]);
+    IBL_LU14(v_P_0, E0_1, lane4, 0u);
+    IBL_LU14(v_o0_0, E1_2, lane4, 0u);
+    step_fence();
+    IBL_Q4(q2, in[2], lane4);
+    IBL_Q4(q3, in[3], lane4);
+    IBL_LUC4(v_P_1, v_P_0, q2, 1u);
+    IBL_LUC4(v_o0_1, v_o0_0, q3, 1u);
+    step_fence();
+    IBL_Q4(q4, in[4], lane4);
+    IBL_LUC4(v_P_2, v_P_1, q3, 2u);
+    IBL_LUC4(v_o0_2, v_o0_1, q4, 2u);
+    step_fence();
+    IBL_Q4(q5, in[5], lane4);
+    IBL_LUC4(v_P_3, v_P_2, q4, 3u);
+    IBL_LUC4(v_o0_3, v_o0_2, q5, 3u);
+    step_fence();
+    IBL_QK4(qk, in[6], in[7], lane4k);
+    IBL_SH4(sh, in[7]);
+    IBL_LUC4(v_P_4, v_P_3, q5, 128u);
+    IBL_LUK4(v_o0_4, v_o0_3, qk);
+    step_fence();
+    IBL_Q4(q6, in[6], lane4f);
+    IBL_LUC4(v_P_5, v_P_4, q6, 0u);
+    IBL_LU14(v_c1_0, E0_2, lane4, 0u);
+    IBL_PKK4(o[0], v_o0_4, sh);
+    step_fence();
+    IBL_QC4(qc1, FC & 2, ch1);
+    IBL_LINK4(f_P, FC & 2, v_P_5, qc1);
+    IBL_LUC4(v_c1_1, v_c1_0, q3, 1u);
+    IBL_LUC4(v_c2_0, v_P_0, q3, 1u);
+    step_fence();
+    IBL_LUC4(v_c1_2, v_c1_1, q4, 2u);
+    IBL_LUC4(v_c2_1, v_c2_0, q4, 2u);
+    IBL_PK4(o[7], f_P);
+    step_fence();
+    IBL_LUC4(v_c1_3, v_c1_2, q5, 3u);
+    IBL_LUC4(v_c2_2, v_c2_1, q5, 3u);
+    step_fence();
+    IBL_LUK4(v_c1_4, v_c1_3, qk);
+    IBL_LUK4(v_c2_3, v_c2_2, qk);
+    step_fence();
+    IBL_LUC4(v_c3_0, v_P_1, q4, 2u);
+    IBL_LUC4(v_c4_0, v_P_2, q5, 3u);
+    IBL_PKK4(o[1], v_c1_4, sh);
+    IBL_PKK4(o[2], v_c2_3, sh);
+    step_fence();
+    IBL_LUC4(v_c3_1, v_c3_0, q5, 3u);
+    IBL_LUK4(v_c4_1, v_c4_0, qk);
+    step_fence();
+    IBL_LUK4(v_c3_2, v_c3_1, qk);
+    IBL_LUK4(v_c5_0, v_P_3, qk);
+    IBL_PKK4(o[4], v_c4_1, sh);
+    step_fence();
+    IBL_Q4(q7, in[7], lane4f);
+    IBL_LUC4(v_c6_0, v_P_4, q7, 0u);
+    IBL_PKK4(o[3], v_c3_2, sh);
+    IBL_PKK4(o[5], v_c5_0, sh);
+    step_fence();
+    IBL_QC4(qc0, FC & 1, ch0);
+    IBL_LINK4(f_c6, FC & 1, v_c6_0, qc0);
+    step_fence();
+    IBL_PK4(o[6], f_c6);
+    step_fence();
+  }
+}
 template <int D, int K0, int ST> __device__ __forceinline__ void vn_group_ct(uint32_t lane4, const uint32_t (&in)[D], uint32_t fbase, uint32_t chw,
     uint32_t (&o)[D]) {
   static_assert(D >= 2 && D <= 4 && K0 >= 0 && (ST == 1 || ST == 2), "unrolled bodies: degrees 2..4");
diff --git a/informationbottleneckdecodingldpc_amd/csrc/plan.h b/informationbottleneckdecodingldpc_amd/csrc/plan.h
--- a/informationbottleneckdecodingldpc_amd/csrc/plan.h
+++ b/informationbottleneckdecodingldpc_amd/csrc/plan.h
@@ -182,6 +182,46 @@
     if (deg[v] > kLightD) ++*heavy;
   }
   return info;
+}
+
+constexpr size_t kIbCompBytes = 65536;
+constexpr size_t kIbLdsBytes = 160 * 1024;
+constexpr size_t ib_table_lds(int nt) { return (size_t)((((nt + 3) >> 2) + 1) >> 1) * 65536; }
+inline int32_t ib_composite_degree(const std::vector<int32_t>& cn_deg, int cm, int cn_tables) {
+  if (cm > 8 || ib_table_lds(cn_tables) + kIbCompBytes + 64 > kIbLdsBytes) return 0;
+  int64_t cnt[9] = {0};
+  for (int32_t d : cn_deg)
+    if (d >= 5 && d <= 8) ++cnt[d];
+  int32_t best = 0;
+  for (int32_t d = 5; d <= 8; ++d)
+    if (cnt[d] > 0 && (best == 0 || cnt[d] >= cnt[best])) best = d;
+  return best;
+}
+inline void ib_composite_image(const uint8_t* L, const uint8_t* F, uint32_t* img) {
+  for (int e = 0; e < 256; ++e)
+    for (int h = 0; h < 2; ++h) {
+      uint32_t w = 0;
+      for (int y = 0; y < 8; ++y) w |= (uint32_t)(F[16 * (L[e] & 15) + 8 * h + y] & 15) << (4 * y);
+      img[256 * h + e] = w;
+    }
+}
+
+inline int64_t ib_cn_raw_index(int Tc, int T, int CM, int p, int l, int t, int m) {
+  const int64_t T2 = (int64_t)T * T;
+  if (p == 0) return l == 0 ? (int64_t)t * Tc + m : (int64_t)Tc * Tc + (int64_t)(l - 1) * Tc * T + (int64_t)t * T + m;
+  return (int64_t)Tc * Tc + (int64_t)(CM - 3) * Tc * T + (int64_t)(p - 1) * (CM - 2) * T2 + l * T2 + (int64_t)t * T + m;
+}
+inline void ib_composite_pass(const int32_t* cn, const int32_t* mc, bool match, int T, int CM, int p, int D,
+                              uint32_t* img) {
+  uint8_t L[256] = {0}, F[256] = {0};
+  const int64_t mrow = (int64_t)p * T * CM + (int64_t)(D - 1) * T;
+  for (int t = 0; t < T; ++t)
+    for (int m = 0; m < T; ++m) {
+      const int32_t r = cn[ib_cn_raw_index(T, T, CM, p, D - 3, t, m)];
+      L[16 * t + m] = (uint8_t)cn[ib_cn_raw_index(T, T, CM, p, D - 4, t, m)];
+      F[16 * t + m] = (uint8_t)(match ? mc[mrow + r] : r);
+    }
+  ib_composite_image(L, F, img);
 }
 
 struct FusedTasks {
diff --git a/informationbottleneckdecodingldpc_amd/engine.py b/informationbottleneckdecodingldpc_amd/engine.py
--- a/informationbottleneckdecodingldpc_amd/engine.py
+++ b/informationbottleneckdecodingldpc_amd/engine.py
@@ -70,7 +70,7 @@
     _PATHS = {"auto": _lib.IBL_PATH_AUTO, "passes": _lib.IBL_PATH_PASSES, "fused": _lib.IBL_PATH_FUSED}
 
     def __init__(self, graph: Graph, tables: IBTables, match: bool, max_batch: int, force_generic: bool = False,
-                 path: str = "auto", fold: bool = True):
+                 path: str = "auto", fold: bool = True, composite: bool = True):
         self.graph = graph
         self.tables = tables
         self.match = bool(match)
@@ -94,6 +94,8 @@
         _lib.check(L.ibl_ib_set_path(h, self._PATHS[path]), "ibl_ib_set_path")
         if not fold:
             self.fold = False
+        if not composite:
+            self.composite = False
 
     @property
     def fused(self) -> bool:
@@ -125,6 +127,16 @@
     def fold(self, on: bool) -> None:
         _lib.check(_lib.load().ibl_ib_set_fold(self._h, int(bool(on))), "ibl_ib_set_fold")
         self._fold = bool(on)
+
+    @property
+    def composite(self) -> int:
+        d = ctypes.c_int32()
+        _lib.check(_lib.load().ibl_ib_composite(self._h, ctypes.byref(d)), "ibl_ib_composite")
+        return int(d.value)
+
+    @composite.setter
+    def composite(self, on: bool) -> None:
+        _lib.check(_lib.load().ibl_ib_set_composite(self._h, int(bool(on))), "ibl_ib_set_composite")
 
     def fused_ncw(self, B: int) -> int:
         n = ctypes.c_int32()
```

Result: faster. 204,400 (median of 6 runs) (+1.4%).
